# DeepRec-AI/DeepRec

Hardware: AMD Instinct MI355X
Metric: samples/sec (whole node) DLRM Criteo-TB-shaped synthetic (higher is better)
Workload: dtype bf16; 1 GPU; model=dlrm, global_batch=8192, seq_len=1, parallelism=single, hip_graph=True, optimizer=adamasync, embedding_dim=16, num_tables=26

## Files before the change

deeprec_amd/embedding/collection.py:

```python
from __future__ import annotations

from typing import List, Optional, Sequence

import torch

from deeprec_amd.embedding.options import EmbeddingVariableOption
from deeprec_amd.embedding.ragged import RaggedIds
from deeprec_amd.embedding.variable import get_global_step
from deeprec_amd.ops import functional as F
from deeprec_amd.ops.common import COMBINER_ID, KEY_BITS, DedupResult


def unique_and_probe(storage, keys, train: bool, graph_mode: bool = False,
                     allow_dedup: bool = True,
                     bump_step: bool = True) -> DedupResult:
    if graph_mode and train:
        return storage.dedup_lookup_capture(keys, bump_step=bump_step)
    prefers_dedup = getattr(storage, "prefers_dedup", None)
    if train and allow_dedup and prefers_dedup is not None \
            and prefers_dedup():
        return storage.dedup_lookup(keys, get_global_step())
    uniq, inverse, counts = torch.unique(
        keys, return_inverse=True, return_counts=True)
    slots = storage.lookup_or_create(uniq, counts, get_global_step(),
                                     train=train)
    if prefers_dedup is not None:
        storage.observe_uniq_ratio(uniq.numel(), keys.numel())
    return DedupResult(uniq, inverse.to(torch.int32), counts, slots, None,
                       None)


def prep_backward(storage, inverse, counts, rank=None):
    m = counts.numel()
    c32 = counts.to(torch.int32)
    bounds = torch.zeros(m + 1, dtype=torch.int32, device=inverse.device)
    bounds[1:] = c32.cumsum(0)
    if inverse.device.type != "cuda":
        order = torch.argsort(inverse.long()).to(torch.int32)
    elif rank is not None:
        order = storage.ext.csr_scatter(inverse, rank, bounds,
                                        storage.error_flag)
    else:
        order = storage.ext.csr_order(inverse, bounds, m)
    return order, bounds


def row_coeffs(comb, offsets, row_ids, weights):
    lengths = (offsets[1:] - offsets[:-1]).float()
    if weights is None:
        wsum = lengths
        wsq = lengths
    else:
        wsum = torch.zeros_like(lengths)
        wsum.index_add_(0, row_ids.long(), weights)
        wsq = torch.zeros_like(lengths)
        wsq.index_add_(0, row_ids.long(), weights * weights)
    denom = torch.where(comb == 2, wsq.sqrt(), wsum)
    coeff = torch.where(comb == 0, torch.ones_like(denom),
                        1.0 / denom.clamp(min=1e-12))
    return torch.where(lengths > 0, coeff, torch.zeros_like(coeff))


class EmbeddingCollection:
    def __init__(self, name: str, table_names: Sequence[str],
                 embedding_dim: int,
                 ev_option: Optional[EmbeddingVariableOption] = None,
                 combiners=None, device=None, value_dtype=torch.float32,
                 generator=None, trainable: bool = True):
        self.name = name
        self.table_names = list(table_names)
        self.n_tables = len(self.table_names)
        assert 0 < self.n_tables < (1 << (63 - KEY_BITS))
        self.dim = embedding_dim
        self.device = torch.device(device or "cpu")
        self.trainable = trainable
        self.ev_option = ev_option or EmbeddingVariableOption()
        self.combiners = list(combiners or ["mean"] * self.n_tables)
        assert len(self.combiners) == self.n_tables

        import copy
        opt = copy.deepcopy(self.ev_option)
        dvd = max(1, opt.init_option.default_value_dim)
        opt.init_option.default_value_dim = dvd * self.n_tables
        from deeprec_amd.embedding.options import StorageType
        fp8 = opt.storage_option.storage_type == StorageType.HBM_FP8
        if fp8:
            from deeprec_amd.ops.quant_backend import (QuantizedHbmStorage,
                                                       require_cuda_for_fp8)
            require_cuda_for_fp8(self.device, f"EmbeddingCollection {name!r}")
            self.trainable = trainable = False
            self.storage = QuantizedHbmStorage(embedding_dim, opt,
                                               value_dtype, self.device,
                                               generator)
        elif self.device.type == "cuda":
            from deeprec_amd.ops.hip_backend import HbmStorage
            self.storage = HbmStorage(embedding_dim, opt, value_dtype,
                                      self.device, generator)
        else:
            from deeprec_amd.ops.cpu_backend import CpuStorage
            self.storage = CpuStorage(embedding_dim, opt, value_dtype,
                                      self.device, generator)
        self.storage.key_bits = KEY_BITS
        self.storage.dvd_per_table = dvd
        self._combiner_ids = torch.tensor(
            [COMBINER_ID[c] for c in self.combiners], dtype=torch.int32,
            device=self.device)
        self._anchor = torch.zeros((), device=self.device,
                                   requires_grad=trainable)
        self._matrix_cache = {}
        self.graph_mode = False
        self._pending_grads: List = []
        self._recorded_ids: List[torch.Tensor] = []
        self._record_sparse_ids = False

    def composite(self, table: int, ids: torch.Tensor) -> torch.Tensor:
        return ids + (table << KEY_BITS)

    def decompose(self, keys: torch.Tensor):
        return keys >> KEY_BITS, keys & ((1 << KEY_BITS) - 1)

    def accumulate_grad(self, slots, keys, grad_unique):
        self._pending_grads.append((slots, keys, grad_unique))

    def consume_grads(self):
        out = self._pending_grads
        self._pending_grads = []
        return out

    def get_slab(self, name, width=None, init_value=0.0, dtype=torch.float32):
        return self.storage.get_slab(name, width or self.dim, init_value,
                                     dtype)

    def size(self):
        return self.storage.size()

    def total_count(self):
        return self.storage.total_count()

    def _concat_inputs(self, sp_list: Sequence[RaggedIds]):
        batch = sp_list[0].batch_size
        dev = self.device
        vals, offs, rows, weights = [], [], [], []
        base = 0
        any_weights = any(sp.weights is not None for sp in sp_list)
        for t, sp in enumerate(sp_list):
            assert sp.batch_size == batch, "collection: batch mismatch"
            vals.append(sp.values + (t << KEY_BITS))
            o = sp.offsets.to(torch.int64)
            offs.append((o[:-1] if t + 1 < len(sp_list) else o) + base)
            base += int(sp.values.numel())
            rows.append(sp.row_ids().to(torch.int64) + t * batch)
            if any_weights:
                weights.append(sp.weights.float() if sp.weights is not None
                               else torch.ones(sp.values.numel(), device=dev))
        values_cat = torch.cat(vals)
        offsets_cat = torch.cat(offs).to(torch.int32)
        row_ids_cat = torch.cat(rows).to(torch.int32)
        weights_cat = torch.cat(weights) if any_weights else None
        return batch, values_cat, offsets_cat, row_ids_cat, weights_cat

    def _row_coeffs(self, offsets_cat, row_ids_cat, weights_cat, batch):
        return row_coeffs(self._combiner_ids.repeat_interleave(batch),
                          offsets_cat, row_ids_cat, weights_cat)

    def lookup(self, sp_list: Sequence[RaggedIds], out_dtype=None,
               train: bool = True) -> torch.Tensor:
        assert len(sp_list) == self.n_tables
        batch, values_cat, offsets_cat, row_ids_cat, weights_cat = \
            self._concat_inputs(sp_list)
        train = train and self.trainable
        d = self._dedup_and_probe(values_cat, train)
        if not train:
            return self._forward(d.uniq, d.slots, d.inverse, offsets_cat,
                                 weights_cat, batch, out_dtype)
        order, bounds = self._prep_backward(d.inverse, d.counts, d.rank)
        row_coeff = self._row_coeffs(offsets_cat, row_ids_cat, weights_cat,
                                     batch)
        return _CollectionLookup.apply(
            self._anchor, self, d.uniq, d.slots, d.inverse, offsets_cat,
            row_ids_cat, order, bounds, row_coeff, weights_cat, batch,
            out_dtype, False)

    def _dedup_and_probe(self, values_cat, train) -> DedupResult:
        d = unique_and_probe(self.storage, values_cat, train,
                             self.graph_mode)
        if train and self._record_sparse_ids:
            self._recorded_ids.append(d.uniq.detach())
        return d

    def _prep_backward(self, inverse, counts, rank=None):
        return prep_backward(self.storage, inverse, counts, rank)

    def matrix_inputs(self, ids: torch.Tensor):
        batch, n = ids.shape
        assert n == self.n_tables
        cache = self._matrix_cache.get(batch)
        if cache is None:
            dev = self.device
            nb = n * batch
            cache = (
                torch.arange(nb + 1, dtype=torch.int32, device=dev),
                torch.arange(nb, dtype=torch.int32, device=dev),
                torch.ones(nb, device=dev),
                (torch.arange(n, dtype=torch.int64, device=dev)
                 << KEY_BITS).repeat_interleave(batch))
            self._matrix_cache[batch] = cache
        offsets, row_ids, row_coeff, tags = cache
        return ids.t().reshape(-1) + tags, offsets, row_ids, row_coeff

    def lookup_matrix(self, ids: torch.Tensor, out_dtype=None,
                      train: bool = True) -> torch.Tensor:
        batch = ids.shape[0]
        values_cat, offsets, row_ids, row_coeff = self.matrix_inputs(ids)
        train = train and self.trainable
        d = self._dedup_and_probe(values_cat, train)
        if not train:
            return self._forward(d.uniq, d.slots, d.inverse, offsets, None,
                                 batch, out_dtype)
        order, bounds = self._prep_backward(d.inverse, d.counts, d.rank)
        return _CollectionLookup.apply(
            self._anchor, self, d.uniq, d.slots, d.inverse, offsets,
            row_ids, order, bounds, row_coeff, None, batch, out_dtype, True)

    def _forward(self, uniq, slots, inverse, offsets_cat, weights_cat, batch,
                 out_dtype, emb_override=None):
        if self.device.type == "cuda" and hasattr(self.storage, "ext"):
            if emb_override is not None:
                return self.storage.ext.group_pooled_fwd_direct(
                    emb_override.contiguous(), uniq, inverse, offsets_cat,
                    weights_cat if weights_cat is not None
                    else torch.Tensor(),
                    self._combiner_ids, batch, self.n_tables,
                    out_dtype or torch.float32)
            return self.storage.group_pooled_lookup(
                uniq, slots, inverse, offsets_cat, weights_cat,
                self._combiner_ids, batch, self.n_tables, out_dtype)
        emb = (emb_override if emb_override is not None
               else self.storage.gather(uniq, slots))
        outs = []
        row_ids_all = None
        nb = offsets_cat.numel() - 1
        lengths = (offsets_cat[1:] - offsets_cat[:-1]).long()
        row_ids_cat = torch.repeat_interleave(
            torch.arange(nb, dtype=torch.int64,
                         device=offsets_cat.device), lengths)
        for t in range(self.n_tables):
            lo, hi = t * batch, (t + 1) * batch
            jmask = (row_ids_cat >= lo) & (row_ids_cat < hi)
            sub_off = (offsets_cat[lo:hi + 1] - offsets_cat[lo]).to(
                torch.int32)
            out_t = F.pooled_forward(
                emb, inverse[jmask], sub_off,
                (row_ids_cat[jmask] - lo).to(torch.int32),
                self.combiners[t],
                weights_cat[jmask] if weights_cat is not None else None,
                out_dtype)
            outs.append(out_t)
        return torch.cat(outs, dim=1)

    def _backward(self, grad_out, order, bounds, inverse, row_ids_cat,
                  weights_cat, row_coeff, m, batch, identity_rows=False):
        if self.device.type == "cuda":
            return self.storage.ext.group_pooled_bwd_seg(
                grad_out.contiguous(), order, inverse, row_ids_cat,
                weights_cat if weights_cat is not None else torch.Tensor(),
                row_coeff, m, batch, self.n_tables, self.dim,
                identity_rows, 0)
        g = grad_out.float().reshape(batch, self.n_tables, self.dim)
        grad_unique = torch.zeros(m, self.dim)
        order_l = order.long()
        j_sorted = order_l
        counts = (bounds[1:] - bounds[:-1]).long()
        u_of_k = torch.repeat_interleave(
            torch.arange(m, dtype=torch.int64), counts)
        rid = row_ids_cat.long()[j_sorted]
        t_idx = rid // batch
        b_idx = rid % batch
        contrib = g[b_idx, t_idx, :] * row_coeff[rid].unsqueeze(1)
        if weights_cat is not None:
            contrib = contrib * weights_cat[j_sorted].unsqueeze(1)
        grad_unique.index_add_(0, u_of_k, contrib)
        return grad_unique

    def export(self, include_filtered: bool = False):
        return self.storage.export(include_filtered)

    def restore(self, keys, values, freqs=None, versions=None):
        self.storage.import_(keys.to(self.device), values, freqs, versions)

    def export_tables(self, include_filtered: bool = False):
        keys, values, freqs, versions = self.storage.export()
        tid, raw = self.decompose(keys)
        out = {}
        for t, name in enumerate(self.table_names):
            mask = tid == t
            out[name] = (raw[mask], values[mask], freqs[mask],
                         versions[mask])
        return out

    def restore_table(self, table: int, keys, values, freqs=None,
                      versions=None):
        self.storage.import_(self.composite(table, keys.to(self.device)),
                             values, freqs, versions)

    def shrink(self, step: Optional[int] = None) -> int:
        return self.storage.shrink(
            step if step is not None else get_global_step())

    def start_sparse_recording(self):
        self._record_sparse_ids = True

    def consume_recorded_ids(self) -> torch.Tensor:
        if not self._recorded_ids:
            return torch.empty(0, dtype=torch.int64, device=self.device)
        ids = torch.unique(torch.cat(self._recorded_ids))
        self._recorded_ids = []
        return ids

    def get_frequency(self, table: int, keys):
        return self.storage.frequencies(
            self.composite(table, keys.to(self.device)))

    def get_version(self, table: int, keys):
        return self.storage.versions(
            self.composite(table, keys.to(self.device)))

    def __repr__(self):
        return (f"EmbeddingCollection(name={self.name!r}, "
                f"tables={self.n_tables}, dim={self.dim}, "
                f"device={self.device})")


class _CollectionLookup(torch.autograd.Function):
    @staticmethod
    def forward(ctx, anchor, coll, uniq, slots, inverse, offsets_cat,
                row_ids_cat, order, bounds, row_coeff, weights_cat, batch,
                out_dtype, identity_rows=False):
        out = coll._forward(uniq, slots, inverse, offsets_cat, weights_cat,
                            batch, out_dtype)
        ctx.coll = coll
        ctx.batch = batch
        ctx.identity_rows = identity_rows
        ctx.save_for_backward(uniq, slots, order, bounds, inverse,
                              row_ids_cat, row_coeff)
        ctx.weights_cat = weights_cat
        return out

    @staticmethod
    def backward(ctx, grad_out):
        uniq, slots, order, bounds, inverse, row_ids_cat, row_coeff = \
            ctx.saved_tensors
        coll = ctx.coll
        grad_unique = coll._backward(grad_out, order, bounds, inverse,
                                     row_ids_cat, ctx.weights_cat,
                                     row_coeff, uniq.numel(), ctx.batch,
                                     ctx.identity_rows)
        coll.accumulate_grad(slots, uniq, grad_unique)
        return (torch.zeros_like(coll._anchor),) + (None,) * 13
```

deeprec_amd/embedding/lookup.py:

```python
from __future__ import annotations

import os
from typing import List, Sequence

import torch

from deeprec_amd.embedding.collection import (prep_backward, row_coeffs,
                                              unique_and_probe)
from deeprec_amd.embedding.ragged import RaggedIds
from deeprec_amd.embedding.variable import (EmbeddingVariable,
                                            get_global_step)
from deeprec_amd.ops import functional as F
from deeprec_amd.ops.common import COMBINER_ID, PAD_KEY


class _PooledLookup(torch.autograd.Function):
    @staticmethod
    def forward(ctx, anchor, ev, uniq, slots, inverse, offsets, row_ids,
                counts, combiner, weights, out_dtype):
        out = ev.storage.pooled_lookup(
            uniq, slots, inverse, offsets, row_ids, combiner, weights,
            out_dtype) if hasattr(ev.storage, "pooled_lookup") else None
        if out is None:
            emb = ev.storage.gather(uniq, slots)
            out = F.pooled_forward(emb, inverse, offsets, row_ids, combiner,
                                   weights, out_dtype)
        ctx.ev = ev
        ctx.combiner = combiner
        ctx.save_for_backward(uniq, slots, inverse, offsets, row_ids, counts)
        ctx.weights = weights
        return out

    @staticmethod
    def backward(ctx, grad_out):
        uniq, slots, inverse, offsets, row_ids, counts = ctx.saved_tensors
        ev = ctx.ev
        if (grad_out.device.type == "cuda"
                and hasattr(ev.storage, "ext") and counts.numel()):
            grad_unique = _chunked_ev_backward(
                ev, grad_out, inverse, offsets, row_ids, counts,
                ctx.combiner, ctx.weights)
        elif hasattr(ev.storage, "pooled_grad"):
            grad_unique = ev.storage.pooled_grad(
                grad_out, inverse, offsets, row_ids, uniq.numel(),
                ctx.combiner, ctx.weights)
        else:
            grad_unique = F.pooled_backward(
                grad_out, inverse, offsets, row_ids, uniq.numel(),
                ctx.combiner, ctx.weights)
        ev.accumulate_grad(slots, uniq, grad_unique)
        return (torch.zeros_like(ctx.ev._anchor),) + (None,) * 10


def _chunked_ev_backward(ev, grad_out, inverse, offsets, row_ids, counts,
                         combiner, weights):
    st = ev.storage
    m = counts.numel()
    weights = weights.float() if weights is not None else None
    order, _ = prep_backward(st, inverse, counts)
    comb = torch.full((1,), COMBINER_ID[combiner], dtype=torch.int32,
                      device=grad_out.device)
    row_coeff = row_coeffs(comb, offsets, row_ids, weights)
    return st.ext.group_pooled_bwd_seg(
        grad_out.contiguous(), order, inverse.to(torch.int32),
        row_ids.to(torch.int32),
        weights if weights is not None else torch.Tensor(),
        row_coeff, m, offsets.numel() - 1, 1, ev.dim, False, 0)


def _drop_positions(sp_ids: RaggedIds, keep: torch.Tensor) -> RaggedIds:
    row_ids = sp_ids.row_ids()[keep]
    values = sp_ids.values[keep]
    weights = sp_ids.weights[keep] if sp_ids.weights is not None else None
    lengths = torch.zeros(sp_ids.batch_size, dtype=torch.int64,
                          device=values.device)
    lengths.index_add_(0, row_ids.long(),
                       torch.ones_like(row_ids, dtype=torch.int64))
    offsets = torch.zeros(sp_ids.batch_size + 1, dtype=sp_ids.offsets.dtype,
                          device=values.device)
    offsets[1:] = lengths.cumsum(0)
    return RaggedIds(values, offsets, weights)


def embedding_lookup_sparse(ev: EmbeddingVariable, sp_ids: RaggedIds,
                            combiner: str = "mean",
                            out_dtype=None,
                            train: bool = True) -> torch.Tensor:
    from deeprec_amd.parallel.sharded_embedding import (
        ShardedEmbeddingVariable, sharded_embedding_lookup_sparse)
    if isinstance(ev, ShardedEmbeddingVariable):
        return sharded_embedding_lookup_sparse(ev, sp_ids, combiner,
                                               out_dtype, train)
    inv = getattr(ev, "invalid_key", None)
    if inv is not None and bool((sp_ids.values == inv).any()):
        sp_ids = _drop_positions(sp_ids, sp_ids.values != inv)
    graph_mode = bool(getattr(ev, "graph_mode", False)) and ev.trainable
    uniq, inverse, counts, slots, _rank, _m = unique_and_probe(
        ev.storage, sp_ids.values, train, graph_mode,
        allow_dedup=ev.trainable
        and not os.environ.get("DEEPREC_AMD_DISABLE_DEDUP"),
        bump_step=not (graph_mode and train)
        or ev.first_lookup_of_step())
    if train and ev._record_sparse_ids:
        ev._recorded_ids.append(uniq.detach())
    row_ids = sp_ids.row_ids()
    if not (train and ev.trainable):
        emb = ev.storage.gather(uniq, slots)
        return F.pooled_forward(emb, inverse, offsets=sp_ids.offsets,
                                row_ids=row_ids, combiner=combiner,
                                weights=sp_ids.weights, out_dtype=out_dtype)
    return _PooledLookup.apply(ev._anchor, ev, uniq, slots,
                               inverse.to(torch.int32),
                               sp_ids.offsets.to(torch.int32),
                               row_ids, counts, combiner, sp_ids.weights,
                               out_dtype)


def safe_embedding_lookup_sparse(ev, sp_ids: RaggedIds, combiner="mean",
                                 out_dtype=None, train=True):
    if bool((sp_ids.values < 0).any()):
        sp_ids = _drop_positions(sp_ids, sp_ids.values >= 0)
    return embedding_lookup_sparse(ev, sp_ids, combiner, out_dtype, train)


class _PaddedSeqLookup(torch.autograd.Function):

    @staticmethod
    def forward(ctx, anchor, ev, uniq, slots, inverse, order, out_dtype):
        out = ev.storage.seq_gather_pad(uniq, slots, inverse, out_dtype)
        ctx.ev = ev
        ctx.save_for_backward(uniq, slots, inverse, order)
        return out

    @staticmethod
    def backward(ctx, grad_out):
        uniq, slots, inverse, order = ctx.saved_tensors
        ev = ctx.ev
        if grad_out.dtype not in (torch.float32, torch.bfloat16):
            grad_out = grad_out.float()
        none = torch.Tensor()
        grad_unique = ev.storage.ext.group_pooled_bwd_seg(
            grad_out.contiguous(), order, inverse, none, none, none,
            uniq.numel(), inverse.numel(), 1, ev.dim, True, 0)
        ev.accumulate_grad(slots, uniq, grad_unique)
        return (torch.zeros_like(ev._anchor),) + (None,) * 6


def masked_padded_lookup(ev, ids: torch.Tensor, pad_id: int, out_dtype=None,
                         train: bool = True) -> torch.Tensor:
    flat = ids.reshape(-1)
    mask = flat != pad_id
    rows = embedding_lookup(ev, flat[mask], out_dtype=out_dtype, train=train)
    emb = torch.zeros(flat.numel(), ev.dim, device=flat.device,
                      dtype=rows.dtype)
    emb = emb.index_put((mask.nonzero().squeeze(1),), rows)
    return emb.reshape(*ids.shape, ev.dim)


def _static_padded_lookup(ev, ids, pad_id, out_dtype, train):
    st = ev.storage
    flat = ids.reshape(-1).to(torch.int64)
    n = flat.numel()
    is_pad = flat == pad_id
    keys = torch.where(is_pad, torch.full_like(flat, PAD_KEY), flat)
    if not (train and ev.trainable):
        slots = st.lookup(keys)
        inverse = torch.where(
            is_pad, torch.full((n,), -1, dtype=torch.int32,
                               device=flat.device),
            torch.arange(n, dtype=torch.int32, device=flat.device))
        out = st.seq_gather_pad(keys, slots, inverse, out_dtype)
        return out.reshape(*ids.shape, ev.dim)
    if ev.graph_mode:
        d = st.dedup_lookup_capture(
            keys, pad=True, bump_step=ev.first_lookup_of_step())
    else:
        d = st.dedup_lookup(keys, get_global_step(), pad=True)
    if ev._record_sparse_ids:
        if d.m_dev is not None:
            raise RuntimeError(
                "sparse-id recording needs the exact unique keys; "
                "graph_mode pads them")
        ev._recorded_ids.append(d.uniq.detach())
    m = d.counts.numel()
    bounds = torch.zeros(m + 1, dtype=torch.int32, device=flat.device)
    bounds[1:] = d.counts.cumsum(0)
    order = st.ext.csr_scatter_pad(d.inverse, d.rank, bounds, st.error_flag)
    out = _PaddedSeqLookup.apply(ev._anchor, ev, d.uniq, d.slots, d.inverse,
                                 order, out_dtype)
    return out.reshape(*ids.shape, ev.dim)


def embedding_lookup(ev: EmbeddingVariable, ids: torch.Tensor,
                     out_dtype=None, train: bool = True,
                     pad_id=None) -> torch.Tensor:
    if pad_id is not None:
        st = getattr(ev, "storage", None)
        if (isinstance(ev, EmbeddingVariable) and ev.device.type == "cuda"
                and hasattr(st, "ext") and not hasattr(st, "apply_split")):
            return _static_padded_lookup(ev, ids, pad_id, out_dtype, train)
        return masked_padded_lookup(ev, ids, pad_id, out_dtype, train)
    flat = ids.reshape(-1)
    n = flat.numel()
    offsets = torch.arange(n + 1, dtype=torch.int32, device=flat.device)
    out = embedding_lookup_sparse(
        ev, RaggedIds(flat, offsets), combiner="sum",
        out_dtype=out_dtype, train=train)
    return out.reshape(*ids.shape, ev.dim)


def group_embedding_lookup_sparse(evs: Sequence[EmbeddingVariable],
                                  sp_ids_list: Sequence[RaggedIds],
                                  combiners=None, out_dtype=None,
                                  train: bool = True) -> List[torch.Tensor]:
    if combiners is None:
        combiners = ["mean"] * len(evs)
    if len(evs) != len(sp_ids_list) or len(evs) != len(combiners):
        raise ValueError("group_embedding_lookup_sparse: length mismatch")
    return [embedding_lookup_sparse(ev, sp, c, out_dtype, train)
            for ev, sp, c in zip(evs, sp_ids_list, combiners)]
```

deeprec_amd/models/common.py:

```python
from __future__ import annotations

from typing import List, Optional, Sequence

import torch
import torch.nn as nn

from deeprec_amd.data.synthetic import NUM_SPARSE
from deeprec_amd.embedding import EmbeddingVariableOption
from deeprec_amd.embedding.collection import EmbeddingCollection


def make_mlp(sizes: Sequence[int], in_dim: int, device,
             bf16: bool, final_activation: bool = True) -> nn.Sequential:
    if bf16 and torch.device(device).type == "cuda":
        from deeprec_amd.ops.fused_mlp import fused_mlp
        return fused_mlp(list(sizes), in_dim, final_activation)
    layers: List[nn.Module] = []
    d = in_dim
    for i, h in enumerate(sizes):
        layers.append(nn.Linear(d, h))
        if final_activation or i + 1 < len(sizes):
            layers.append(nn.ReLU(inplace=True))
        d = h
    return nn.Sequential(*layers)


class Dice(nn.Module):

    def __init__(self, dim: int, eps: float = 1e-8):
        super().__init__()
        self.bn = nn.BatchNorm1d(dim, eps=eps, affine=False)
        self.alpha = nn.Parameter(torch.zeros(dim))

    def forward(self, x):
        shape = x.shape
        p = torch.sigmoid(self.bn(x.reshape(-1, shape[-1]).float()))
        p = p.reshape(shape).to(x.dtype)
        return x * p + self.alpha.to(x.dtype) * x * (1 - p)


class RecModelBase(nn.Module):

    def __init__(self, embedding_dim: int = 16, device="cpu",
                 bf16: bool = True, num_sparse: int = NUM_SPARSE,
                 ev_option: Optional[EmbeddingVariableOption] = None,
                 name: str = "model", sharded: bool = False,
                 combiners: Optional[List[str]] = None):
        super().__init__()
        self.device_ = torch.device(device)
        self.embedding_dim = embedding_dim
        self.num_sparse = num_sparse
        self.bf16 = bf16 and self.device_.type == "cuda"
        cls = EmbeddingCollection
        if sharded:
            from deeprec_amd.parallel.sharded_collection import (
                ShardedEmbeddingCollection)
            cls = ShardedEmbeddingCollection
        self.collection = cls(
            f"{name}/sparse", [f"C{i + 1}" for i in range(num_sparse)],
            embedding_dim, ev_option=ev_option,
            combiners=combiners or ["mean"] * num_sparse,
            device=self.device_)

    @property
    def compute_dtype(self):
        return torch.bfloat16 if self.bf16 else torch.float32

    def embedding_variables(self):
        return [self.collection]

    def sparse_feats(self, sparse_ids, train=True) -> torch.Tensor:
        if isinstance(sparse_ids, torch.Tensor):
            cat = self.collection.lookup_matrix(
                sparse_ids, out_dtype=self.compute_dtype, train=train)
        else:
            cat = self.collection.lookup(
                sparse_ids, out_dtype=self.compute_dtype, train=train)
        return cat.view(-1, self.num_sparse, self.embedding_dim)

    def amp(self):
        import contextlib
        if self.bf16:
            return torch.autocast(device_type="cuda", dtype=torch.bfloat16)
        return contextlib.nullcontext()

    def loss_fn(self, logits: torch.Tensor, labels: torch.Tensor):
        return nn.functional.binary_cross_entropy_with_logits(
            logits.float(), labels.float())
```

deeprec_amd/models/dlrm.py:

```python
from __future__ import annotations

from typing import List, Optional

import torch
import torch.nn as nn

from deeprec_amd.data.synthetic import NUM_SPARSE
from deeprec_amd.embedding import (
    EmbeddingVariable, EmbeddingVariableOption,
    group_embedding_lookup_sparse,
)


def _mlp(sizes, in_dim, final_activation=True):
    layers: List[nn.Module] = []
    d = in_dim
    for i, h in enumerate(sizes):
        layers.append(nn.Linear(d, h))
        if final_activation or i + 1 < len(sizes):
            layers.append(nn.ReLU(inplace=True))
        d = h
    return nn.Sequential(*layers)


class DLRM(nn.Module):
    def __init__(self, embedding_dim: int = 16,
                 mlp_bot=(512, 256, 64, 16), mlp_top=(512, 256),
                 interaction_op: str = "dot", bf16: bool = True,
                 device="cpu", ev_option: Optional[EmbeddingVariableOption] = None,
                 num_sparse: int = NUM_SPARSE, name_prefix: str = "dlrm",
                 sharded: bool = False, use_collection: bool = True):
        super().__init__()
        assert mlp_bot[-1] == embedding_dim, \
            "bottom MLP output must match embedding dim (dot interaction)"
        self.embedding_dim = embedding_dim
        self.interaction_op = interaction_op
        self.bf16 = bf16
        self.device_ = torch.device(device)
        self.num_sparse = num_sparse

        self.dense_in = 16
        use_fused = bf16 and torch.device(device).type == "cuda"
        self._fused = use_fused
        n_f = num_sparse + 1
        n_pairs = n_f * (n_f - 1) // 2
        self.n_pairs_pad = (n_pairs + 15) & ~15
        top_in = (embedding_dim + self.n_pairs_pad
                  if interaction_op == "dot" else n_f * embedding_dim)
        if use_fused:
            from deeprec_amd.ops.fused_mlp import fused_mlp
            self.mlp_bot = fused_mlp(mlp_bot, self.dense_in)
            self.mlp_top = fused_mlp(list(mlp_top) + [1], top_in,
                                     final_activation=False)
        else:
            self.mlp_bot = _mlp(mlp_bot, self.dense_in)
            self.mlp_top = _mlp(list(mlp_top) + [1], top_in,
                                final_activation=False)
        self.to(self.device_)

        self.collection = None
        if sharded:
            from deeprec_amd.parallel.sharded_collection import (
                ShardedEmbeddingCollection)
            self.collection = ShardedEmbeddingCollection(
                f"{name_prefix}/sparse",
                [f"C{i+1}" for i in range(num_sparse)], embedding_dim,
                ev_option=ev_option, combiners=["mean"] * num_sparse,
                device=self.device_,
                comm_dtype=torch.bfloat16 if self.bf16 else None)
            self.evs = []
        elif use_collection:
            from deeprec_amd.embedding.collection import EmbeddingCollection
            self.collection = EmbeddingCollection(
                f"{name_prefix}/sparse",
                [f"C{i+1}" for i in range(num_sparse)], embedding_dim,
                ev_option=ev_option, combiners=["mean"] * num_sparse,
                device=self.device_)
            self.evs = []
        else:
            self.evs = [
                EmbeddingVariable(f"{name_prefix}/C{i+1}", embedding_dim,
                                  ev_option=ev_option, device=self.device_)
                for i in range(num_sparse)]

    def embedding_variables(self):
        return [self.collection] if self.collection is not None else self.evs

    def _interact(self, feats: torch.Tensor) -> torch.Tensor:
        from deeprec_amd.ops.fused_mlp import dot_interaction
        return dot_interaction(feats, self.n_pairs_pad)

    def forward(self, dense: torch.Tensor, sparse_ids,
                train: bool = True) -> torch.Tensor:
        compute_dtype = torch.bfloat16 if (
            self.bf16 and dense.device.type == "cuda") else torch.float32
        if self.collection is not None:
            if isinstance(sparse_ids, torch.Tensor):
                emb_cat = self.collection.lookup_matrix(
                    sparse_ids, out_dtype=compute_dtype, train=train)
            else:
                emb_cat = self.collection.lookup(sparse_ids,
                                                 out_dtype=compute_dtype,
                                                 train=train)
            emb_feats = emb_cat.view(-1, self.num_sparse, self.embedding_dim)
        else:
            emb_list = group_embedding_lookup_sparse(
                self.evs, sparse_ids, combiners=["mean"] * len(self.evs),
                out_dtype=compute_dtype, train=train)
            emb_feats = torch.stack(list(emb_list), dim=1)
        import contextlib
        amp = (torch.autocast(device_type="cuda", dtype=torch.bfloat16)
               if compute_dtype == torch.bfloat16 else contextlib.nullcontext())
        from deeprec_amd.ops.fused_mlp import prep_dense
        dense = prep_dense(dense, self.dense_in, fused=self._fused)
        with amp:
            bot = self.mlp_bot(dense)
            if self.interaction_op == "dot":
                from deeprec_amd.ops.fused_mlp import dot_interaction_cat
                top_in = dot_interaction_cat(bot, emb_feats,
                                             self.n_pairs_pad)
            else:
                feats = torch.cat(
                    [bot.unsqueeze(1), emb_feats.to(bot.dtype)], dim=1)
                top_in = feats.flatten(1)
            logits = self.mlp_top(top_in)
        return logits.squeeze(1).float()

    def loss_fn(self, logits: torch.Tensor, labels: torch.Tensor):
        return nn.functional.binary_cross_entropy_with_logits(logits, labels)
```

deeprec_amd/ops/build_ext.py:

```python
from __future__ import annotations

import hashlib
import importlib.machinery
import importlib.util
import os
import subprocess
import sys
import sysconfig

_EXT_NAME = "deeprec_amd_hip"
_HERE = os.path.dirname(os.path.abspath(__file__))
_EXT_DIR = os.path.normpath(os.path.join(_HERE, "..", "_ext"))
_SOURCES = [os.path.join(_HERE, "hip", "ev_kernels.hip"),
            os.path.join(_HERE, "hip", "dense_kernels.hip"),
            os.path.join(_HERE, "hip", "gru_kernels.hip"),
            os.path.join(_HERE, "hip", "attention_kernels.hip"),
            os.path.join(_HERE, "hip", "fp8_kernels.hip"),
            os.path.join(_HERE, "hip", "quant_ev_kernels.hip")]
_HIPCC = os.environ.get("HIPCC", "/opt/rocm/bin/hipcc")
_ARCH = os.environ.get("PYTORCH_ROCM_ARCH", "gfx950")

_cached = None


def _torch_paths():
    import torch
    root = os.path.dirname(torch.__file__)
    return (
        [os.path.join(root, "include"),
         os.path.join(root, "include", "torch", "csrc", "api", "include"),
         "/opt/rocm/include",
         sysconfig.get_paths()["include"]],
        os.path.join(root, "lib"),
    )


def _so_path() -> str:
    return os.path.join(_EXT_DIR, f"{_EXT_NAME}.so")


def _headers():
    hip_dir = os.path.join(_HERE, "hip")
    return sorted(os.path.join(hip_dir, f) for f in os.listdir(hip_dir)
                  if f.endswith((".h", ".hpp")))


def _sources_digest() -> str:
    h = hashlib.sha256()
    for s in _SOURCES + _headers():
        with open(s, "rb") as f:
            h.update(f.read())
    return h.hexdigest()[:16]


def build_extension(verbose: bool = False, force: bool = False):
    global _cached
    os.makedirs(_EXT_DIR, exist_ok=True)
    so = _so_path()
    stamp = os.path.join(_EXT_DIR, "source.sha")
    digest = _sources_digest()
    if (not force and os.path.exists(so) and os.path.exists(stamp)
            and open(stamp).read().strip() == digest):
        return load_extension()

    includes, libdir = _torch_paths()
    objs = []
    common_defs = [
        f"-DTORCH_EXTENSION_NAME={_EXT_NAME}",
        "-DTORCH_API_INCLUDE_EXTENSION_H",
        "-D__HIP_PLATFORM_AMD__=1", "-DUSE_ROCM=1", "-DHIPBLAS_V2",
        "-DCUDA_HAS_FP16=1", "-D__HIP_NO_HALF_OPERATORS__=1",
        "-D__HIP_NO_HALF_CONVERSIONS__=1",
        "-DHIP_ENABLE_WARP_SYNC_BUILTINS=1",
    ]
    for src in _SOURCES:
        obj = os.path.join(
            _EXT_DIR, os.path.basename(src).replace(".hip", ".o"))
        cmd = ([_HIPCC, "-c", src, "-o", obj, "-O3", "-std=c++17", "-fPIC",
                f"--offload-arch={_ARCH}", "-fno-gpu-rdc"]
               + common_defs + [f"-isystem{p}" for p in includes])
        if verbose:
            print(" ".join(cmd))
        subprocess.run(cmd, check=True)
        objs.append(obj)
    link = ([_HIPCC, "-shared", "-o", so] + objs +
            [f"-L{libdir}", "-lc10", "-lc10_hip", "-ltorch_cpu",
             "-ltorch_hip", "-ltorch", "-ltorch_python",
             "-L/opt/rocm/lib", "-lamdhip64",
             f"-Wl,-rpath,{libdir}"])
    if verbose:
        print(" ".join(link))
    subprocess.run(link, check=True)
    with open(stamp, "w") as f:
        f.write(digest)
    _cached = None
    return load_extension()


def load_extension():
    global _cached
    if _cached is not None:
        return _cached
    import torch
    so = _so_path()
    if not os.path.exists(so):
        return build_extension()
    loader = importlib.machinery.ExtensionFileLoader(_EXT_NAME, so)
    spec = importlib.util.spec_from_loader(_EXT_NAME, loader)
    mod = importlib.util.module_from_spec(spec)
    loader.exec_module(mod)
    sys.modules[_EXT_NAME] = mod
    _cached = mod
    return mod


def require_extension():
    try:
        return load_extension()
    except Exception as e:
        raise RuntimeError(
            "deeprec_amd HIP extension is not built/loadable. Run "
            "`python __graft_entry__.py` (build) first. Native kernels are "
            f"required on GPU — no eager fallback. Cause: {e}") from e
```

deeprec_amd/ops/hip/ev_kernels.hip:

```cpp

#include "hip_common.h"

#define DEV_INLINE __device__ __forceinline__

static constexpr int64_t EMPTY_KEY = INT64_MIN;
static constexpr int64_t PAD_KEY = INT64_MAX;
static constexpr int kBlock = 256;

namespace {

DEV_INLINE uint64_t mix_hash(uint64_t k) {
  k += 0x9E3779B97F4A7C15ull;
  k = (k ^ (k >> 30)) * 0xBF58476D1CE4E5B9ull;
  k = (k ^ (k >> 27)) * 0x94D049BB133111EBull;
  return k ^ (k >> 31);
}

DEV_INLINE float bf2f(__hip_bfloat16 v) { return __bfloat162float(v); }
DEV_INLINE __hip_bfloat16 f2bf(float v) { return __float2bfloat16(v); }


DEV_INLINE int64_t ht_find(const int64_t* __restrict__ ht_keys,
                           int64_t cap_mask, int64_t key) {
  uint64_t h = mix_hash((uint64_t)key) & (uint64_t)cap_mask;
  for (int64_t probe = 0; probe <= cap_mask; ++probe) {
    int64_t idx = (int64_t)((h + probe) & (uint64_t)cap_mask);
    int64_t cur = ht_keys[idx];
    if (cur == key) return idx;
    if (cur == EMPTY_KEY) return -1;
  }
  return -1;
}

DEV_INLINE int64_t ht_find_or_claim(int64_t* __restrict__ ht_keys,
                                    int64_t cap_mask, int64_t key,
                                    int32_t* __restrict__ entry_counter) {
  uint64_t h = mix_hash((uint64_t)key) & (uint64_t)cap_mask;
  for (int64_t probe = 0; probe <= cap_mask; ++probe) {
    int64_t idx = (int64_t)((h + probe) & (uint64_t)cap_mask);
    int64_t cur = ht_keys[idx];
    if (cur != key) {
      if (cur != EMPTY_KEY) continue;
      int64_t prev = (int64_t)atomicCAS(
          (unsigned long long*)&ht_keys[idx],
          (unsigned long long)EMPTY_KEY, (unsigned long long)key);
      if (prev != EMPTY_KEY && prev != key) continue;
      if (prev == EMPTY_KEY) atomicAdd(entry_counter, 1);
    }
    return idx;
  }
  return -1;
}

DEV_INLINE int64_t default_row(int64_t key, int key_bits,
                               int default_value_dim) {
  if (key_bits > 0) {
    int64_t mask = ((int64_t)1 << key_bits) - 1;
    return (key >> key_bits) * default_value_dim +
           (int64_t)((uint64_t)(key & mask) % (uint64_t)default_value_dim);
  }
  return (int64_t)((uint64_t)key % (uint64_t)default_value_dim);
}

DEV_INLINE int32_t ht_admit(
    int64_t key, int64_t idx, int32_t* __restrict__ ht_slot,
    int32_t* __restrict__ slot_counter, int max_slots,
    float* __restrict__ values, const float* __restrict__ default_values,
    int dim, int default_value_dim, int key_bits, int init_limit,
    int32_t* __restrict__ error_flag) {
  int32_t slot = atomicAdd(slot_counter, 1);
  if (slot >= max_slots) {
    atomicExch(error_flag, 1);
    return -1;
  }
  ht_slot[idx] = slot;
  if (slot < init_limit) {
    const float* src =
        default_values + default_row(key, key_bits, default_value_dim) * dim;
    float* dst = values + (int64_t)slot * dim;
    for (int d = 0; d < dim; ++d) dst[d] = src[d];
  }
  return slot;
}

__global__ void k_lookup_insert(
    const int64_t* __restrict__ keys, const int32_t* __restrict__ counts,
    int n, int64_t* __restrict__ ht_keys, int32_t* __restrict__ ht_slot,
    int32_t* __restrict__ ht_freq, int64_t* __restrict__ ht_version,
    int64_t cap_mask, int32_t* __restrict__ slot_counter,
    int32_t* __restrict__ entry_counter, int max_slots,
    float* __restrict__ values, const float* __restrict__ default_values,
    int dim, int default_value_dim, int key_bits, int init_limit,
    int filter_freq, int64_t step, int train,
    int32_t* __restrict__ out_slots, int32_t* __restrict__ error_flag) {
  int64_t i = blockIdx.x * (int64_t)blockDim.x + threadIdx.x;
  int64_t gstride = gridDim.x * (int64_t)blockDim.x;
  for (; i < n; i += gstride) {
    const int64_t key = keys[i];
    int32_t slot = -1;
    if (!train) {
      int64_t idx = ht_find(ht_keys, cap_mask, key);
      if (idx >= 0) slot = ht_slot[idx];
    } else {
      int64_t idx = ht_find_or_claim(ht_keys, cap_mask, key, entry_counter);
      if (idx < 0) {
        atomicExch(error_flag, 2);
      } else {
        int32_t freq = ht_freq[idx] + (counts ? counts[i] : 1);
        ht_freq[idx] = freq;
        ht_version[idx] = step;
        slot = ht_slot[idx];
        if (slot < 0 && freq >= filter_freq)
          slot = ht_admit(key, idx, ht_slot, slot_counter, max_slots, values,
                          default_values, dim, default_value_dim, key_bits,
                          init_limit, error_flag);
      }
    }
    out_slots[i] = slot;
  }
}

__global__ void k_insert_bulk(
    const int64_t* __restrict__ keys, const int32_t* __restrict__ slots,
    const int32_t* __restrict__ freqs, const int64_t* __restrict__ versions,
    int n, int64_t* __restrict__ ht_keys, int32_t* __restrict__ ht_slot,
    int32_t* __restrict__ ht_freq, int64_t* __restrict__ ht_version,
    int64_t cap_mask, int32_t* __restrict__ entry_counter,
    int32_t* __restrict__ error_flag) {
  int64_t i = blockIdx.x * (int64_t)blockDim.x + threadIdx.x;
  int64_t gstride = gridDim.x * (int64_t)blockDim.x;
  for (; i < n; i += gstride) {
    int64_t idx = ht_find_or_claim(ht_keys, cap_mask, keys[i], entry_counter);
    if (idx < 0) {
      atomicExch(error_flag, 2);
      continue;
    }
    ht_slot[idx] = slots[i];
    if (freqs) ht_freq[idx] = freqs[i];
    if (versions) ht_version[idx] = versions[i];
  }
}


template <bool SKIP_PAD>
__global__ void k_dedup_pass_a(
    const int64_t* __restrict__ keys, int nnz, int64_t* __restrict__ ht_keys,
    int32_t* __restrict__ ht_epoch, int32_t* __restrict__ ht_compact,
    int64_t cap_mask, const int32_t* __restrict__ epoch_dev, int epoch_val,
    int32_t* __restrict__ entry_counter, int32_t* __restrict__ m_counter,
    int64_t* __restrict__ uniq_keys, int64_t* __restrict__ compact_entry,
    int64_t* __restrict__ occ_entry, int32_t* __restrict__ error_flag) {
  const int epoch = epoch_dev ? *epoch_dev : epoch_val;
  int64_t j = blockIdx.x * (int64_t)blockDim.x + threadIdx.x;
  int64_t stride = gridDim.x * (int64_t)blockDim.x;
  for (; j < nnz; j += stride) {
    const int64_t key = keys[j];
    if constexpr (SKIP_PAD) {
      if (key == PAD_KEY) {
        occ_entry[j] = -1;
        continue;
      }
    }
    int64_t idx = ht_find_or_claim(ht_keys, cap_mask, key, entry_counter);
    if (idx < 0) {
      atomicExch(error_flag, 2);
      continue;
    }
    if (ht_epoch[idx] != epoch) {
      int old = atomicExch(&ht_epoch[idx], epoch);
      if (old != epoch) {
        int c = atomicAdd(m_counter, 1);
        ht_compact[idx] = c;
        uniq_keys[c] = key;
        compact_entry[c] = idx;
      }
    }
    occ_entry[j] = idx;
  }
}

__global__ void k_bump_epoch(int32_t* __restrict__ epoch_dev,
                             int64_t* __restrict__ step_dev) {
  if (threadIdx.x == 0 && blockIdx.x == 0) {
    epoch_dev[0] += 1;
    step_dev[0] += 1;
  }
}

__global__ void k_dedup_pass_b(
    const int64_t* __restrict__ compact_entry,
    const int64_t* __restrict__ uniq_keys, int n,
    const int32_t* __restrict__ m_dev, int32_t* __restrict__ ht_slot,
    int32_t* __restrict__ ht_freq, int64_t* __restrict__ ht_version,
    const int32_t* __restrict__ batch_counts,
    const int64_t* __restrict__ step_dev, int64_t step_val,
    int32_t* __restrict__ slot_counter, int max_slots,
    float* __restrict__ values, const float* __restrict__ default_values,
    int dim, int default_value_dim, int key_bits, int init_limit,
    int filter_freq, int32_t* __restrict__ out_slots,
    int32_t* __restrict__ error_flag) {
  const int m = m_dev ? *m_dev : n;
  const int64_t step = step_dev ? *step_dev : step_val;
  int64_t c = blockIdx.x * (int64_t)blockDim.x + threadIdx.x;
  int64_t gstride = gridDim.x * (int64_t)blockDim.x;
  for (; c < n; c += gstride) {
    if (m_dev && (c >= m || uniq_keys[c] == PAD_KEY)) {
      out_slots[c] = -1;
      continue;
    }
    int64_t idx = compact_entry[c];
    int32_t freq = ht_freq[idx] + batch_counts[c];
    ht_freq[idx] = freq;
    ht_version[idx] = step;
    int32_t slot = ht_slot[idx];
    if (slot < 0 && freq >= filter_freq)
      slot = ht_admit(uniq_keys[c], idx, ht_slot, slot_counter, max_slots,
                      values, default_values, dim, default_value_dim,
                      key_bits, init_limit, error_flag);
    out_slots[c] = slot;
  }
}

__global__ void k_zero_f32(float* __restrict__ p, int64_t n) {
  int64_t i = (blockIdx.x * (int64_t)blockDim.x + threadIdx.x) * 4;
  int64_t stride = gridDim.x * (int64_t)blockDim.x * 4;
  for (; i + 3 < n; i += stride)
    *reinterpret_cast<float4*>(p + i) = make_float4(0.f, 0.f, 0.f, 0.f);
  if (blockIdx.x == 0 && threadIdx.x == 0)
    for (int64_t j = n & ~3LL; j < n; ++j) p[j] = 0.0f;
}


__global__ void k_bump_epoch_only(int32_t* __restrict__ epoch_dev) {
  if (threadIdx.x == 0 && blockIdx.x == 0) epoch_dev[0] += 1;
}

__global__ void k_route_fill(int64_t* __restrict__ send_keys,
                             int32_t* __restrict__ send_cnt,
                             int32_t* __restrict__ peer_cursor, int total,
                             int world) {
  int64_t i = blockIdx.x * (int64_t)blockDim.x + threadIdx.x;
  int64_t stride = gridDim.x * (int64_t)blockDim.x;
  for (; i < total; i += stride) {
    send_keys[i] = PAD_KEY;
    send_cnt[i] = 0;
    if (i < world) peer_cursor[i] = 0;
  }
}

static constexpr int kMaxWorld = 64;

__global__ void k_route_pad(
    const int64_t* __restrict__ uniq_keys, const int32_t* __restrict__ counts,
    const int32_t* __restrict__ m_dev, int n_cap, int world, int cap,
    int key_bits, int64_t* __restrict__ send_keys,
    int32_t* __restrict__ send_cnt, int32_t* __restrict__ route_pos,
    int32_t* __restrict__ peer_cursor, int32_t* __restrict__ error_flag) {
  const int m = min(*m_dev, n_cap);
  const int64_t key_mask =
      key_bits > 0 ? (((int64_t)1 << key_bits) - 1) : ~(int64_t)0;
  __shared__ int32_t lcnt[kMaxWorld];
  __shared__ int32_t lbase[kMaxWorld];
  for (int64_t base = (int64_t)blockIdx.x * blockDim.x; base < m;
       base += (int64_t)gridDim.x * blockDim.x) {
    int64_t u = base + threadIdx.x;
    for (int o = threadIdx.x; o < world; o += blockDim.x) lcnt[o] = 0;
    __syncthreads();
    int owner = -1, my = 0;
    int64_t key = 0;
    if (u < m) {
      key = uniq_keys[u];
      owner = (int)((uint64_t)(key & key_mask) % (uint64_t)world);
      my = atomicAdd(&lcnt[owner], 1);
    }
    __syncthreads();
    for (int o = threadIdx.x; o < world; o += blockDim.x)
      lbase[o] = lcnt[o] ? atomicAdd(&peer_cursor[o], lcnt[o]) : 0;
    __syncthreads();
    if (u < m) {
      int pos = lbase[owner] + my;
      if (pos >= cap) {
        atomicExch(error_flag, 4);
        route_pos[u] = owner * cap;
      } else {
        int64_t o = (int64_t)owner * cap + pos;
        send_keys[o] = key;
        send_cnt[o] = counts[u];
        route_pos[u] = (int32_t)o;
      }
    }
    __syncthreads();
  }
}


__global__ void k_slots_gather_pad(const int32_t* __restrict__ inverse,
                                   const int32_t* __restrict__ slots,
                                   int nnz, int32_t* __restrict__ out) {
  int64_t j = blockIdx.x * (int64_t)blockDim.x + threadIdx.x;
  int64_t stride = gridDim.x * (int64_t)blockDim.x;
  for (; j < nnz; j += stride) {
    int c = inverse[j];
    out[j] = c < 0 ? -1 : slots[c];
  }
}

__global__ void k_cnt_sum_pad(const int32_t* __restrict__ inverse,
                              const int32_t* __restrict__ cnt, int nnz,
                              int32_t* __restrict__ cnt_sum) {
  int64_t j = blockIdx.x * (int64_t)blockDim.x + threadIdx.x;
  int64_t stride = gridDim.x * (int64_t)blockDim.x;
  for (; j < nnz; j += stride) {
    int c = inverse[j];
    if (c >= 0) atomicAdd(&cnt_sum[c], cnt[j]);
  }
}

__global__ void k_rows_segsum_pad(const float* __restrict__ grad,
                                  const int32_t* __restrict__ inverse,
                                  int nnz, int dim,
                                  float* __restrict__ grad2) {
  int64_t t = blockIdx.x * (int64_t)blockDim.x + threadIdx.x;
  int64_t total = (int64_t)nnz * dim;
  int64_t stride = gridDim.x * (int64_t)blockDim.x;
  for (; t < total; t += stride) {
    int j = (int)(t / dim);
    int c = inverse[j];
    if (c < 0) continue;
    int d = (int)(t % dim);
    atomicAdd(&grad2[(int64_t)c * dim + d], grad[t]);
  }
}

__global__ void k_compose_i32(const int32_t* __restrict__ inv_in,
                              const int32_t* __restrict__ lut, int nnz,
                              int32_t* __restrict__ inv_out) {
  int64_t j = blockIdx.x * (int64_t)blockDim.x + threadIdx.x;
  int64_t stride = gridDim.x * (int64_t)blockDim.x;
  for (; j < nnz; j += stride) inv_out[j] = lut[inv_in[j]];
}

__global__ void k_rows_to_padded(const float* __restrict__ src,
                                 const int32_t* __restrict__ route_pos,
                                 const int32_t* __restrict__ m_dev,
                                 int n_cap, int dim,
                                 float* __restrict__ dst) {
  const int m = min(*m_dev, n_cap);
  int64_t t = blockIdx.x * (int64_t)blockDim.x + threadIdx.x;
  int64_t total = (int64_t)m * dim;
  int64_t stride = gridDim.x * (int64_t)blockDim.x;
  for (; t < total; t += stride) {
    int u = (int)(t / dim);
    int d = (int)(t % dim);
    dst[(int64_t)route_pos[u] * dim + d] = src[t];
  }
}

struct WaveGroup {
  uint64_t mask;
  int leader;
  int pos;
};

DEV_INLINE WaveGroup wave_group_by(uint64_t v, bool valid) {
  WaveGroup g{0ull, 0, 0};
  const int lane = __lane_id();
  uint64_t mask = __ballot(valid);
  int leader = lane;
  for (int b = 0; b < 64; b += 8) {
#pragma unroll
    for (int i = 0; i < 8; ++i) {
      const bool bit = (v >> (b + i)) & 1ull;
      const uint64_t with = __ballot(bit);
      mask &= bit ? with : ~with;
    }
    leader = valid ? __ffsll((unsigned long long)mask) - 1 : lane;
    const uint64_t lv = __shfl(v, leader);
    if (!__ballot(valid && lv != v)) break;
  }
  if (valid) {
    g.mask = mask;
    g.leader = leader;
    g.pos = __popcll(mask & ((1ull << lane) - 1ull));
  }
  return g;
}

DEV_INLINE int64_t wave_slice_begin() {
  const int wave = __builtin_amdgcn_readfirstlane((int)(threadIdx.x >> 6));
  return (blockIdx.x * (int64_t)(blockDim.x >> 6) + wave) * 64;
}
DEV_INLINE int64_t wave_slice_stride() {
  return gridDim.x * (int64_t)(blockDim.x >> 6) * 64;
}

__global__ void k_dedup_pass_c(
    const int64_t* __restrict__ keys, const int64_t* __restrict__ occ_entry,
    int nnz, const int32_t* __restrict__ ht_compact,
    int32_t* __restrict__ inverse, int32_t* __restrict__ counts,
    int32_t* __restrict__ rank) {
  const int lane = __lane_id();
  const int64_t stride = wave_slice_stride();
  for (int64_t j0 = wave_slice_begin(); j0 < nnz; j0 += stride) {
    const int64_t j = j0 + lane;
    const bool in_range = j < nnz;
    const bool valid = in_range && !(keys && keys[j] == PAD_KEY);
    const int64_t entry = valid ? occ_entry[j] : 0;
    const WaveGroup g = wave_group_by((uint64_t)entry, valid);
    int c = -1, base = 0;
    if (valid && lane == g.leader) {
      c = ht_compact[entry];
      base = atomicAdd(&counts[c], __popcll(g.mask));
    }
    c = __shfl(c, g.leader);
    base = __shfl(base, g.leader);
    if (in_range) {
      inverse[j] = valid ? c : -1;
      rank[j] = valid ? base + g.pos : 0;
    }
  }
}

__global__ void k_csr_scatter(const int32_t* __restrict__ inverse,
                              const int32_t* __restrict__ rank, int nnz,
                              const int32_t* __restrict__ bounds,
                              int32_t* __restrict__ order,
                              int32_t* __restrict__ error_flag) {
  int64_t j = blockIdx.x * (int64_t)blockDim.x + threadIdx.x;
  int64_t stride = gridDim.x * (int64_t)blockDim.x;
  for (; j < nnz; j += stride) {
    int64_t o = (int64_t)bounds[inverse[j]] + rank[j];
    if (o < 0 || o >= nnz) {
      atomicExch(error_flag, 3);
      continue;
    }
    order[o] = (int32_t)j;
  }
}

__global__ void k_fill_i32(int32_t* __restrict__ p, int64_t n, int32_t v) {
  int64_t i = blockIdx.x * (int64_t)blockDim.x + threadIdx.x;
  int64_t stride = gridDim.x * (int64_t)blockDim.x;
  for (; i < n; i += stride) p[i] = v;
}

__global__ void k_csr_scatter_pad(const int32_t* __restrict__ inverse,
                                  const int32_t* __restrict__ rank, int nnz,
                                  const int32_t* __restrict__ bounds, int m,
                                  int32_t* __restrict__ order,
                                  int32_t* __restrict__ error_flag) {
  int64_t j = blockIdx.x * (int64_t)blockDim.x + threadIdx.x;
  int64_t stride = gridDim.x * (int64_t)blockDim.x;
  for (; j < nnz; j += stride) {
    const int c = inverse[j];
    if (c < 0) continue;
    if (c >= m) {
      atomicExch(error_flag, 3);
      continue;
    }
    int64_t o = (int64_t)bounds[c] + rank[j];
    if (o < 0 || o >= nnz) {
      atomicExch(error_flag, 3);
      continue;
    }
    order[o] = (int32_t)j;
  }
}

__global__ void k_csr_order(const int32_t* __restrict__ inverse, int nnz,
                            const int32_t* __restrict__ bounds,
                            int32_t* __restrict__ cursor,
                            int32_t* __restrict__ order) {
  int64_t j = blockIdx.x * (int64_t)blockDim.x + threadIdx.x;
  int64_t stride = gridDim.x * (int64_t)blockDim.x;
  for (; j < nnz; j += stride) {
    int c = inverse[j];
    int pos = atomicAdd(&cursor[c], 1);
    order[bounds[c] + pos] = (int32_t)j;
  }
}

__global__ void k_gather_host_rows(const float* __restrict__ host_src,
                                   const int64_t* __restrict__ rows,
                                   int64_t m, int dim,
                                   float* __restrict__ out) {
  int64_t t = blockIdx.x * (int64_t)blockDim.x + threadIdx.x;
  int64_t total = m * dim;
  int64_t stride = gridDim.x * (int64_t)blockDim.x;
  for (; t < total; t += stride)
    out[t] = host_src[rows[t / dim] * dim + t % dim];
}

__global__ void k_scatter_host_rows(const float* __restrict__ src,
                                    const int64_t* __restrict__ rows,
                                    int64_t m, int dim,
                                    float* __restrict__ host_dst) {
  int64_t t = blockIdx.x * (int64_t)blockDim.x + threadIdx.x;
  int64_t total = m * dim;
  int64_t stride = gridDim.x * (int64_t)blockDim.x;
  for (; t < total; t += stride)
    host_dst[rows[t / dim] * dim + t % dim] = src[t];
}

__global__ void k_lookup(
    const int64_t* __restrict__ keys, int n,
    const int64_t* __restrict__ ht_keys, const int32_t* __restrict__ ht_slot,
    int64_t cap_mask, int32_t* __restrict__ out_slots,
    int64_t* __restrict__ out_entry) {
  int64_t i = blockIdx.x * (int64_t)blockDim.x + threadIdx.x;
  int64_t gstride = gridDim.x * (int64_t)blockDim.x;
  for (; i < n; i += gstride) {
    int64_t idx = ht_find(ht_keys, cap_mask, keys[i]);
    out_slots[i] = idx >= 0 ? ht_slot[idx] : -1;
    if (out_entry) out_entry[i] = idx;
  }
}

__global__ void k_export_scan(
    const int64_t* __restrict__ ht_keys, const int32_t* __restrict__ ht_slot,
    const int32_t* __restrict__ ht_freq,
    const int64_t* __restrict__ ht_version, int64_t capacity,
    int32_t* __restrict__ cursor, int64_t* __restrict__ out_keys,
    int32_t* __restrict__ out_slots, int32_t* __restrict__ out_freqs,
    int64_t* __restrict__ out_versions, int out_cap) {
  int64_t i = blockIdx.x * (int64_t)blockDim.x + threadIdx.x;
  int64_t stride = gridDim.x * (int64_t)blockDim.x;
  for (; i < capacity; i += stride) {
    int64_t k = ht_keys[i];
    if (k == EMPTY_KEY) continue;
    int32_t pos = atomicAdd(cursor, 1);
    if (pos >= out_cap) continue;
    out_keys[pos] = k;
    out_slots[pos] = ht_slot[i];
    out_freqs[pos] = ht_freq[i];
    out_versions[pos] = ht_version[i];
  }
}


template <typename OutT>
__global__ void k_gather(
    const float* __restrict__ values, const float* __restrict__ default_values,
    const int64_t* __restrict__ keys, const int32_t* __restrict__ slots,
    int m, int dim, int default_value_dim, float no_permission_value,
    int use_no_permission, OutT* __restrict__ out) {
  int64_t t = blockIdx.x * (int64_t)blockDim.x + threadIdx.x;
  int64_t total = (int64_t)m * dim;
  int64_t stride = gridDim.x * (int64_t)blockDim.x;
  for (; t < total; t += stride) {
    int i = (int)(t / dim);
    int d = (int)(t % dim);
    int32_t s = slots[i];
    float v;
    if (s >= 0) {
      v = values[(int64_t)s * dim + d];
    } else if (use_no_permission) {
      v = no_permission_value;
    } else {
      int64_t row = (int64_t)((uint64_t)keys[i] % (uint64_t)default_value_dim);
      v = default_values[row * dim + d];
    }
    if constexpr (std::is_same_v<OutT, __hip_bfloat16>) out[t] = f2bf(v);
    else out[t] = v;
  }
}

template <typename OutT, int VEC>
__global__ void k_seq_gather_pad(
    const float* __restrict__ values, const float* __restrict__ default_values,
    const int64_t* __restrict__ keys, const int32_t* __restrict__ slots,
    const int32_t* __restrict__ inverse, int nnz, int n_uniq, int dim,
    int default_value_dim, float no_permission_value, int use_no_permission,
    OutT* __restrict__ out) {
  const int cpr = dim / VEC;
  int64_t t = blockIdx.x * (int64_t)blockDim.x + threadIdx.x;
  const int64_t total = (int64_t)nnz * cpr;
  const int64_t stride = gridDim.x * (int64_t)blockDim.x;
  for (; t < total; t += stride) {
    const int j = (int)(t / cpr);
    const int d0 = (int)(t % cpr) * VEC;
    const int u = inverse[j];
    float v[VEC];
#pragma unroll
    for (int i = 0; i < VEC; ++i) v[i] = 0.0f;
    if ((unsigned)u < (unsigned)n_uniq) {
      const int32_t s = slots[u];
      const float* src = nullptr;
      if (s >= 0) {
        src = values + (int64_t)s * dim + d0;
      } else if (!use_no_permission) {
        int64_t row =
            (int64_t)((uint64_t)keys[u] % (uint64_t)default_value_dim);
        src = default_values + row * dim + d0;
      }
      if (src) {
        if constexpr (VEC % 4 == 0) {
#pragma unroll
          for (int i = 0; i < VEC; i += 4) {
            const float4 q = *reinterpret_cast<const float4*>(src + i);
            v[i] = q.x; v[i + 1] = q.y; v[i + 2] = q.z; v[i + 3] = q.w;
          }
        } else {
#pragma unroll
          for (int i = 0; i < VEC; ++i) v[i] = src[i];
        }
      } else {
#pragma unroll
        for (int i = 0; i < VEC; ++i) v[i] = no_permission_value;
      }
    }
    OutT* dst = out + (int64_t)j * dim + d0;
    if constexpr (std::is_same_v<OutT, __hip_bfloat16>) {
      if constexpr (VEC == 1) {
        dst[0] = f2bf(v[0]);
      } else {
        uint32_t w[VEC / 2];
#pragma unroll
        for (int i = 0; i < VEC / 2; ++i) {
          const __hip_bfloat16 lo = f2bf(v[2 * i]), hi = f2bf(v[2 * i + 1]);
          w[i] = (uint32_t)(*reinterpret_cast<const uint16_t*>(&lo)) |
                 ((uint32_t)(*reinterpret_cast<const uint16_t*>(&hi)) << 16);
        }
        if constexpr (VEC == 8)
          *reinterpret_cast<uint4*>(dst) = make_uint4(w[0], w[1], w[2], w[3]);
        else
          *reinterpret_cast<uint2*>(dst) = make_uint2(w[0], w[1]);
      }
    } else {
      if constexpr (VEC == 4)
        *reinterpret_cast<float4*>(dst) = make_float4(v[0], v[1], v[2], v[3]);
      else
        dst[0] = v[0];
    }
  }
}

DEV_INLINE float row_coeff(int combiner, int len, const float* wsum) {
  if (combiner == 0 || len == 0) return 1.0f;
  float denom = wsum ? *wsum : (float)len;
  if (combiner == 2) denom = sqrtf(wsum ? *wsum : (float)len);
  return denom > 1e-12f ? 1.0f / denom : 0.0f;
}

template <typename OutT>
__global__ void k_pooled_fwd(
    const float* __restrict__ values, const float* __restrict__ default_values,
    const int64_t* __restrict__ keys, const int32_t* __restrict__ slots,
    const int32_t* __restrict__ inverse, const int32_t* __restrict__ offsets,
    const float* __restrict__ weights, int batch, int dim,
    int default_value_dim, float no_permission_value, int use_no_permission,
    int combiner, OutT* __restrict__ out) {
  int64_t t = blockIdx.x * (int64_t)blockDim.x + threadIdx.x;
  int64_t total = (int64_t)batch * dim;
  int64_t stride = gridDim.x * (int64_t)blockDim.x;
  for (; t < total; t += stride) {
    int b = (int)(t / dim);
    int d = (int)(t % dim);
    int beg = offsets[b], end = offsets[b + 1];
    float acc = 0.0f, wacc = 0.0f;
    for (int j = beg; j < end; ++j) {
      int u = inverse[j];
      int32_t s = slots[u];
      float v;
      if (s >= 0) {
        v = values[(int64_t)s * dim + d];
      } else if (use_no_permission) {
        v = no_permission_value;
      } else {
        int64_t row =
            (int64_t)((uint64_t)keys[u] % (uint64_t)default_value_dim);
        v = default_values[row * dim + d];
      }
      float w = weights ? weights[j] : 1.0f;
      acc += w * v;
      wacc += (combiner == 2) ? w * w : w;
    }
    float coeff = 1.0f;
    int len = end - beg;
    if (combiner != 0 && len > 0) {
      float denom = (combiner == 2) ? sqrtf(wacc) : wacc;
      coeff = denom > 1e-12f ? 1.0f / denom : 0.0f;
    }
    float r = acc * coeff;
    if constexpr (std::is_same_v<OutT, __hip_bfloat16>) out[t] = f2bf(r);
    else out[t] = r;
  }
}

template <typename GradT>
__global__ void k_pooled_bwd(
    const GradT* __restrict__ grad_out, const int32_t* __restrict__ inverse,
    const int32_t* __restrict__ offsets, const float* __restrict__ weights,
    int batch, int dim, int combiner, float* __restrict__ grad_unique) {
  int64_t t = blockIdx.x * (int64_t)blockDim.x + threadIdx.x;
  int64_t total = (int64_t)batch * dim;
  int64_t stride = gridDim.x * (int64_t)blockDim.x;
  for (; t < total; t += stride) {
    int b = (int)(t / dim);
    int d = (int)(t % dim);
    int beg = offsets[b], end = offsets[b + 1];
    int len = end - beg;
    if (len == 0) continue;
    float g;
    if constexpr (std::is_same_v<GradT, __hip_bfloat16>) g = bf2f(grad_out[t]);
    else g = grad_out[t];
    float coeff = 1.0f;
    if (combiner != 0) {
      float wacc = 0.0f;
      if (weights) {
        for (int j = beg; j < end; ++j)
          wacc += (combiner == 2) ? weights[j] * weights[j] : weights[j];
      } else {
        wacc = (float)len;
      }
      float denom = (combiner == 2) ? sqrtf(wacc) : wacc;
      coeff = denom > 1e-12f ? 1.0f / denom : 0.0f;
    }
    float gc = g * coeff;
    for (int j = beg; j < end; ++j) {
      float w = weights ? weights[j] : 1.0f;
      atomicAdd(&grad_unique[(int64_t)inverse[j] * dim + d], w * gc);
    }
  }
}


template <typename OutT>
__global__ void k_group_pooled_fwd(
    const float* __restrict__ values, const float* __restrict__ default_values,
    const int64_t* __restrict__ keys, const int32_t* __restrict__ slots,
    const int32_t* __restrict__ inverse, const int32_t* __restrict__ offsets,
    const float* __restrict__ weights,
    const int32_t* __restrict__ combiner_ids, int batch, int n_tables,
    int dim, int default_value_dim, int key_bits, float no_permission_value,
    int use_no_permission, const float* __restrict__ direct,
    OutT* __restrict__ out) {
  int64_t t = blockIdx.x * (int64_t)blockDim.x + threadIdx.x;
  int64_t total = (int64_t)batch * n_tables * dim;
  int64_t stride = gridDim.x * (int64_t)blockDim.x;
  const int64_t key_mask = ((int64_t)1 << key_bits) - 1;
  for (; t < total; t += stride) {
    int d = (int)(t % dim);
    int64_t rid = t / dim;
    int table = (int)(rid / batch);
    int b = (int)(rid % batch);
    int beg = offsets[rid], end = offsets[rid + 1];
    int combiner = combiner_ids[table];
    float acc = 0.0f, wacc = 0.0f;
    for (int j = beg; j < end; ++j) {
      int u = inverse[j];
      float v;
      if (direct) {
        v = direct[(int64_t)u * dim + d];
      } else {
        int32_t s = slots[u];
        if (s >= 0) {
          v = values[(int64_t)s * dim + d];
        } else if (use_no_permission) {
          v = no_permission_value;
        } else {
          int64_t k = keys[u];
          int64_t row = (int64_t)(table)*default_value_dim +
                        (int64_t)((uint64_t)(k & key_mask) %
                                  (uint64_t)default_value_dim);
          v = default_values[row * dim + d];
        }
      }
      float w = weights ? weights[j] : 1.0f;
      acc += w * v;
      wacc += (combiner == 2) ? w * w : w;
    }
    float coeff = 1.0f;
    if (combiner != 0 && end > beg) {
      float denom = (combiner == 2) ? sqrtf(wacc) : wacc;
      coeff = denom > 1e-12f ? 1.0f / denom : 0.0f;
    }
    float r = acc * coeff;
    int64_t oidx = ((int64_t)b * n_tables + table) * dim + d;
    if constexpr (std::is_same_v<OutT, __hip_bfloat16>) out[oidx] = f2bf(r);
    else out[oidx] = r;
  }
}

template <typename GradT, int LANES, int R, bool IDENTITY>
__global__ void k_group_pooled_bwd_seg(
    const GradT* __restrict__ grad_out, const int32_t* __restrict__ order,
    const int32_t* __restrict__ inverse, const int32_t* __restrict__ row_ids,
    const float* __restrict__ weights, const float* __restrict__ row_coeff,
    int nnz, int m_rows, int batch, int n_tables, int dim,
    float* __restrict__ grad_unique) {
  constexpr int kGroups = kBlock / LANES;
  const int l = threadIdx.x % LANES;
  const int64_t step = gridDim.x * (int64_t)kGroups * R;
  const int n_rows = batch * n_tables;
  auto u_at = [&](int64_t k) -> int {
    if (k < 0 || k >= nnz) return -2;
    int j = order[k];
    if ((unsigned)j >= (unsigned)nnz) return -1;
    int u = inverse[j];
    return (unsigned)u < (unsigned)m_rows ? u : -1;
  };
  for (int64_t k0 = (blockIdx.x * (int64_t)kGroups + threadIdx.x / LANES) * R;
       k0 < nnz; k0 += step) {
    int u[R], grow[R];
    float cf[R];
#pragma unroll
    for (int r = 0; r < R; ++r) {
      u[r] = -2;
      grow[r] = 0;
      cf[r] = 1.0f;
      const int64_t k = k0 + r;
      if (k < nnz) {
        const int j = order[k];
        if ((unsigned)j >= (unsigned)nnz) { u[r] = -1; continue; }
        const int rid = IDENTITY ? j : row_ids[j];
        const int uu = inverse[j];
        if ((unsigned)uu >= (unsigned)m_rows ||
            (unsigned)rid >= (unsigned)n_rows) { u[r] = -1; continue; }
        u[r] = uu;
        grow[r] = (rid % batch) * n_tables + rid / batch;
        if constexpr (!IDENTITY)
          cf[r] = (weights ? weights[j] : 1.0f) * row_coeff[rid];
      }
    }
    const int u_prev = u_at(k0 - 1);
    const int u_next = u_at(k0 + R);
    for (int d = l; d < dim; d += LANES) {
      float g[R];
#pragma unroll
      for (int r = 0; r < R; ++r) {
        g[r] = 0.0f;
        if (u[r] >= 0) {
          const int64_t gidx = (int64_t)grow[r] * dim + d;
          if constexpr (std::is_same_v<GradT, __hip_bfloat16>)
            g[r] = bf2f(grad_out[gidx]);
          else
            g[r] = grad_out[gidx];
        }
      }
      float acc = 0.0f;
      bool cut = u[0] >= 0 && u_prev == u[0];
#pragma unroll
      for (int r = 0; r < R; ++r) {
        if (u[r] < 0) continue;
        if constexpr (IDENTITY) acc += g[r];
        else acc += cf[r] * g[r];
        const int un = (r + 1 < R) ? u[r + 1] : u_next;
        if (un == u[r] && r + 1 < R) continue;
        float* dst = &grad_unique[(int64_t)u[r] * dim + d];
        if (cut || un == u[r]) atomicAdd(dst, acc);
        else *dst = acc;
        acc = 0.0f;
        cut = false;
      }
    }
  }
}


#define APPLY_PROLOG                                              \
  int64_t t = blockIdx.x * (int64_t)blockDim.x + threadIdx.x;     \
  int64_t total = (int64_t)m * dim;                               \
  int64_t stride = gridDim.x * (int64_t)blockDim.x;               \
  for (; t < total; t += stride) {                                \
    int i = (int)(t / dim);                                       \
    int d = (int)(t % dim);                                       \
    int32_t s = slots[i];                                         \
    if (s < 0) continue;                                          \
    int64_t o = (int64_t)s * dim + d;                             \
    float g = grad[t];

#define APPLY_EPILOG }

__global__ void k_apply_sgd(float* __restrict__ w,
                            const int32_t* __restrict__ slots,
                            const float* __restrict__ grad, int m, int dim,
                            float lr) {
  APPLY_PROLOG
  w[o] -= lr * g;
  APPLY_EPILOG
}

__global__ void k_apply_adagrad(float* __restrict__ w,
                                float* __restrict__ accum,
                                const int32_t* __restrict__ slots,
                                const float* __restrict__ grad, int m,
                                int dim, float lr, float epsilon) {
  APPLY_PROLOG
  float a = accum[o] + g * g;
  accum[o] = a;
  w[o] -= lr * g / (sqrtf(a) + epsilon);
  APPLY_EPILOG
}

__global__ void k_apply_adagrad_decay(
    float* __restrict__ w, float* __restrict__ accum,
    float* __restrict__ period_slab, const int32_t* __restrict__ slots,
    const float* __restrict__ grad, int m, int dim, float lr, float epsilon,
    float cur_period, float decay_rate, float baseline) {
  APPLY_PROLOG
  float prev_period = period_slab[s];
  float dp = cur_period - prev_period;
  if (dp < 0.0f) dp = 0.0f;
  float decay = powf(decay_rate, dp);
  float a = accum[o] * decay;
  if (a < baseline) a = baseline;
  a += g * g;
  accum[o] = a;
  w[o] -= lr * g / (sqrtf(a) + epsilon);
  APPLY_EPILOG
}

__global__ void k_commit_period(float* __restrict__ period_slab,
                                const int32_t* __restrict__ slots, int m,
                                float cur_period) {
  int64_t i = blockIdx.x * (int64_t)blockDim.x + threadIdx.x;
  int64_t gstride = gridDim.x * (int64_t)blockDim.x;
  for (; i < m; i += gstride) {
    int32_t sl = slots[i];
    if (sl >= 0) period_slab[sl] = cur_period;
  }
}

__global__ void k_apply_adam(float* __restrict__ w, float* __restrict__ mom,
                             float* __restrict__ vel,
                             const int32_t* __restrict__ slots,
                             const float* __restrict__ grad, int m, int dim,
                             float lr_t, float beta1, float beta2,
                             float epsilon) {
  APPLY_PROLOG
  float mn = beta1 * mom[o] + (1.0f - beta1) * g;
  float vn = beta2 * vel[o] + (1.0f - beta2) * g * g;
  mom[o] = mn;
  vel[o] = vn;
  w[o] -= lr_t * mn / (sqrtf(vn) + epsilon);
  APPLY_EPILOG
}

__global__ void k_apply_adam_dev(float* __restrict__ w,
                                 float* __restrict__ mom,
                                 float* __restrict__ vel,
                                 const int32_t* __restrict__ slots,
                                 const float* __restrict__ grad, int m,
                                 int dim, float lr, float beta1, float beta2,
                                 float epsilon,
                                 const float* __restrict__ powers) {
  const float lr_t =
      lr * sqrtf(1.0f - powers[1]) / (1.0f - powers[0]);
  APPLY_PROLOG
  float mn = beta1 * mom[o] + (1.0f - beta1) * g;
  float vn = beta2 * vel[o] + (1.0f - beta2) * g * g;
  mom[o] = mn;
  vel[o] = vn;
  w[o] -= lr_t * mn / (sqrtf(vn) + epsilon);
  APPLY_EPILOG
}

__global__ void k_update_powers(float* __restrict__ powers, float beta1,
                                float beta2) {
  if (threadIdx.x == 0 && blockIdx.x == 0) {
    powers[0] *= beta1;
    powers[1] *= beta2;
  }
}

__global__ void k_apply_adamw(float* __restrict__ w, float* __restrict__ mom,
                              float* __restrict__ vel,
                              const int32_t* __restrict__ slots,
                              const float* __restrict__ grad, int m, int dim,
                              float lr_t, float lr, float beta1, float beta2,
                              float epsilon, float weight_decay) {
  APPLY_PROLOG
  float mn = beta1 * mom[o] + (1.0f - beta1) * g;
  float vn = beta2 * vel[o] + (1.0f - beta2) * g * g;
  mom[o] = mn;
  vel[o] = vn;
  float wv = w[o];
  w[o] = wv - lr_t * mn / (sqrtf(vn) + epsilon) - lr * weight_decay * wv;
  APPLY_EPILOG
}

__global__ void k_apply_rmsprop(float* __restrict__ w, float* __restrict__ vel,
                                const int32_t* __restrict__ slots,
                                const float* __restrict__ grad, int m,
                                int dim, float lr, float beta2,
                                float epsilon) {
  APPLY_PROLOG
  float vn = beta2 * vel[o] + (1.0f - beta2) * g * g;
  vel[o] = vn;
  w[o] -= lr * g / (sqrtf(vn) + epsilon);
  APPLY_EPILOG
}

__global__ void k_apply_ftrl(float* __restrict__ w, float* __restrict__ n,
                             float* __restrict__ z,
                             const int32_t* __restrict__ slots,
                             const float* __restrict__ grad, int m, int dim,
                             float lr, float l1, float l2, float lr_power,
                             float l2_shrinkage) {
  APPLY_PROLOG
  float wv = w[o];
  float n_old = n[o];
  float n_new = n_old + g * g;
  float sigma = (powf(n_new, -lr_power) - powf(n_old, -lr_power)) / lr;
  float gs = g + 2.0f * l2_shrinkage * wv;
  float z_new = z[o] + gs - sigma * wv;
  n[o] = n_new;
  z[o] = z_new;
  float quad = powf(n_new, -lr_power) / lr + 2.0f * l2;
  float w_new = 0.0f;
  if (fabsf(z_new) > l1)
    w_new = ((z_new > 0.0f ? l1 : -l1) - z_new) / quad;
  w[o] = w_new;
  APPLY_EPILOG
}

}


#define CHECK_DEV(t) TORCH_CHECK((t).is_cuda(), #t " must be on GPU")

static inline void zero_fill(void* p, int64_t n, hipStream_t stream) {
  if (n <= 0) return;
  k_zero_f32<<<n_blocks((n + 3) / 4), kBlock, 0, stream>>>(
      static_cast<float*>(p), n);
}

torch::Tensor ht_lookup_insert(
    torch::Tensor keys, torch::Tensor counts, torch::Tensor ht_keys,
    torch::Tensor ht_slot, torch::Tensor ht_freq, torch::Tensor ht_version,
    torch::Tensor slot_counter, torch::Tensor entry_counter,
    torch::Tensor values, torch::Tensor default_values, int64_t max_slots,
    int64_t dvd_per_table, int64_t key_bits, int64_t init_limit,
    int64_t filter_freq, int64_t step, bool train,
    torch::Tensor error_flag) {
  CHECK_DEV(keys);
  int n = keys.numel();
  auto out = torch::empty({n}, keys.options().dtype(torch::kInt32));
  if (n == 0) return out;
  auto stream = current_hip_stream();
  int dim = values.size(1);
  k_lookup_insert<<<n_blocks(n), kBlock, 0, stream>>>(
      keys.data_ptr<int64_t>(),
      counts.defined() && counts.numel() ? counts.data_ptr<int32_t>()
                                         : nullptr,
      n, ht_keys.data_ptr<int64_t>(), ht_slot.data_ptr<int32_t>(),
      ht_freq.data_ptr<int32_t>(), ht_version.data_ptr<int64_t>(),
      ht_keys.numel() - 1, slot_counter.data_ptr<int32_t>(),
      entry_counter.data_ptr<int32_t>(), (int)max_slots,
      values.data_ptr<float>(), default_values.data_ptr<float>(), dim,
      (int)dvd_per_table, (int)key_bits, (int)init_limit, (int)filter_freq,
      step, train ? 1 : 0, out.data_ptr<int32_t>(),
      error_flag.data_ptr<int32_t>());
  return out;
}

template <typename T>
static inline const T* opt_ptr(const c10::optional<torch::Tensor>& t) {
  return t.has_value() ? t->data_ptr<T>() : nullptr;
}

template <bool SKIP_PAD>
static torch::Tensor dedup_a_impl(
    torch::Tensor keys, torch::Tensor ht_keys, torch::Tensor ht_epoch,
    torch::Tensor ht_compact, c10::optional<torch::Tensor> epoch_dev,
    int64_t epoch, torch::Tensor entry_counter, torch::Tensor m_counter,
    torch::Tensor uniq_keys, torch::Tensor compact_entry,
    torch::Tensor occ_entry, torch::Tensor error_flag) {
  int64_t nnz = keys.numel();
  if (nnz == 0) return m_counter;
  auto stream = current_hip_stream();
  k_dedup_pass_a<SKIP_PAD><<<n_blocks(nnz), kBlock, 0, stream>>>(
      keys.data_ptr<int64_t>(), (int)nnz, ht_keys.data_ptr<int64_t>(),
      ht_epoch.data_ptr<int32_t>(), ht_compact.data_ptr<int32_t>(),
      ht_keys.numel() - 1, opt_ptr<int32_t>(epoch_dev), (int)epoch,
      entry_counter.data_ptr<int32_t>(), m_counter.data_ptr<int32_t>(),
      uniq_keys.data_ptr<int64_t>(), compact_entry.data_ptr<int64_t>(),
      occ_entry.data_ptr<int64_t>(), error_flag.data_ptr<int32_t>());
  return m_counter;
}

torch::Tensor ht_dedup_a(torch::Tensor keys, torch::Tensor ht_keys,
                         torch::Tensor ht_epoch, torch::Tensor ht_compact,
                         c10::optional<torch::Tensor> epoch_dev,
                         int64_t epoch, torch::Tensor entry_counter,
                         torch::Tensor m_counter, torch::Tensor uniq_keys,
                         torch::Tensor compact_entry,
                         torch::Tensor occ_entry, torch::Tensor error_flag) {
  return dedup_a_impl<false>(keys, ht_keys, ht_epoch, ht_compact, epoch_dev,
                             epoch, entry_counter, m_counter, uniq_keys,
                             compact_entry, occ_entry, error_flag);
}

torch::Tensor ht_dedup_a_pad(torch::Tensor keys, torch::Tensor ht_keys,
                             torch::Tensor ht_epoch, torch::Tensor ht_compact,
                             c10::optional<torch::Tensor> epoch_dev,
                             int64_t epoch, torch::Tensor entry_counter,
                             torch::Tensor m_counter, torch::Tensor uniq_keys,
                             torch::Tensor compact_entry,
                             torch::Tensor occ_entry,
                             torch::Tensor error_flag) {
  return dedup_a_impl<true>(keys, ht_keys, ht_epoch, ht_compact, epoch_dev,
                            epoch, entry_counter, m_counter, uniq_keys,
                            compact_entry, occ_entry, error_flag);
}

torch::Tensor ht_dedup_b(torch::Tensor compact_entry, torch::Tensor uniq_keys,
                         c10::optional<torch::Tensor> m_dev,
                         torch::Tensor ht_slot, torch::Tensor ht_freq,
                         torch::Tensor ht_version,
                         torch::Tensor batch_counts,
                         c10::optional<torch::Tensor> step_dev, int64_t step,
                         torch::Tensor slot_counter, int64_t max_slots,
                         torch::Tensor values, torch::Tensor default_values,
                         int64_t dvd_per_table, int64_t key_bits,
                         int64_t init_limit, int64_t filter_freq,
                         torch::Tensor error_flag) {
  int n = uniq_keys.numel();
  auto slots = torch::empty({n}, ht_slot.options());
  if (n == 0) return slots;
  auto stream = current_hip_stream();
  k_dedup_pass_b<<<n_blocks(n), kBlock, 0, stream>>>(
      compact_entry.data_ptr<int64_t>(), uniq_keys.data_ptr<int64_t>(), n,
      opt_ptr<int32_t>(m_dev), ht_slot.data_ptr<int32_t>(),
      ht_freq.data_ptr<int32_t>(), ht_version.data_ptr<int64_t>(),
      batch_counts.data_ptr<int32_t>(), opt_ptr<int64_t>(step_dev), step,
      slot_counter.data_ptr<int32_t>(), (int)max_slots,
      values.data_ptr<float>(), default_values.data_ptr<float>(),
      values.size(1), (int)dvd_per_table, (int)key_bits, (int)init_limit,
      (int)filter_freq, slots.data_ptr<int32_t>(),
      error_flag.data_ptr<int32_t>());
  return slots;
}

void bump_epoch(torch::Tensor epoch_dev, torch::Tensor step_dev) {
  k_bump_epoch<<<1, 64, 0, current_hip_stream()>>>(
      epoch_dev.data_ptr<int32_t>(), step_dev.data_ptr<int64_t>());
}

void bump_epoch_only(torch::Tensor epoch_dev) {
  k_bump_epoch_only<<<1, 64, 0, current_hip_stream()>>>(
      epoch_dev.data_ptr<int32_t>());
}

std::tuple<torch::Tensor, torch::Tensor, torch::Tensor> route_pad(
    torch::Tensor uniq_keys, torch::Tensor counts, torch::Tensor m_dev,
    int64_t world, int64_t cap, int64_t key_bits,
    torch::Tensor error_flag) {
  int n_cap = uniq_keys.numel();
  int total = (int)(world * cap);
  auto opts_i32 = counts.options();
  auto send_keys = torch::empty({(int64_t)total}, uniq_keys.options());
  auto send_cnt = torch::empty({(int64_t)total}, opts_i32);
  auto route_pos = torch::empty({(int64_t)n_cap}, opts_i32);
  auto cursor = torch::empty({world}, opts_i32);
  auto stream = current_hip_stream();
  k_route_fill<<<n_blocks(total), kBlock, 0, stream>>>(
      send_keys.data_ptr<int64_t>(), send_cnt.data_ptr<int32_t>(),
      cursor.data_ptr<int32_t>(), total, (int)world);
  k_route_pad<<<n_blocks(n_cap), kBlock, 0, stream>>>(
      uniq_keys.data_ptr<int64_t>(), counts.data_ptr<int32_t>(),
      m_dev.data_ptr<int32_t>(), n_cap, (int)world, (int)cap, (int)key_bits,
      send_keys.data_ptr<int64_t>(), send_cnt.data_ptr<int32_t>(),
      route_pos.data_ptr<int32_t>(), cursor.data_ptr<int32_t>(),
      error_flag.data_ptr<int32_t>());
  return {send_keys, send_cnt, route_pos};
}

torch::Tensor slots_gather_pad(torch::Tensor inverse, torch::Tensor slots) {
  int64_t nnz = inverse.numel();
  auto out = torch::empty({nnz}, slots.options());
  if (nnz == 0) return out;
  k_slots_gather_pad<<<n_blocks(nnz), kBlock, 0, current_hip_stream()>>>(
      inverse.data_ptr<int32_t>(), slots.data_ptr<int32_t>(), (int)nnz,
      out.data_ptr<int32_t>());
  return out;
}

torch::Tensor cnt_sum_pad(torch::Tensor inverse, torch::Tensor cnt,
                          int64_t m_cap) {
  int64_t nnz = inverse.numel();
  auto out = torch::empty({m_cap}, cnt.options());
  auto stream = current_hip_stream();
  zero_fill(out.data_ptr<int32_t>(), m_cap, stream);
  if (nnz)
    k_cnt_sum_pad<<<n_blocks(nnz), kBlock, 0, stream>>>(
        inverse.data_ptr<int32_t>(), cnt.data_ptr<int32_t>(), (int)nnz,
        out.data_ptr<int32_t>());
  return out;
}

torch::Tensor rows_segsum_pad(torch::Tensor grad, torch::Tensor inverse,
                              int64_t m_cap) {
  int64_t nnz = inverse.numel();
  int dim = grad.size(1);
  auto out = torch::empty({m_cap, (int64_t)dim}, grad.options());
  auto stream = current_hip_stream();
  zero_fill(out.data_ptr<float>(), m_cap * dim, stream);
  if (nnz)
    k_rows_segsum_pad<<<n_blocks(nnz * dim), kBlock, 0, stream>>>(
        grad.data_ptr<float>(), inverse.data_ptr<int32_t>(), (int)nnz, dim,
        out.data_ptr<float>());
  return out;
}

torch::Tensor gather_host_rows(torch::Tensor host_src, torch::Tensor rows) {
  TORCH_CHECK(host_src.is_pinned(), "cold slab must be pinned host memory");
  TORCH_CHECK(rows.is_cuda() && rows.scalar_type() == torch::kInt64);
  int64_t m = rows.numel();
  int dim = host_src.size(1);
  auto out = torch::empty({m, (int64_t)dim},
                          rows.options().dtype(torch::kFloat32));
  if (m == 0) return out;
  k_gather_host_rows<<<n_blocks(m * dim), kBlock, 0, current_hip_stream()>>>(
      host_src.data_ptr<float>(), rows.data_ptr<int64_t>(), m, dim,
      out.data_ptr<float>());
  return out;
}

void scatter_host_rows(torch::Tensor src, torch::Tensor rows,
                       torch::Tensor host_dst) {
  TORCH_CHECK(host_dst.is_pinned(), "cold slab must be pinned host memory");
  TORCH_CHECK(rows.is_cuda() && src.is_cuda());
  int64_t m = rows.numel();
  int dim = host_dst.size(1);
  if (m == 0) return;
  k_scatter_host_rows<<<n_blocks(m * dim), kBlock, 0, current_hip_stream()>>>(
      src.data_ptr<float>(), rows.data_ptr<int64_t>(), m, dim,
      host_dst.data_ptr<float>());
}

torch::Tensor compose_i32(torch::Tensor inv_in, torch::Tensor lut) {
  int64_t nnz = inv_in.numel();
  auto out = torch::empty({nnz}, inv_in.options());
  if (nnz == 0) return out;
  k_compose_i32<<<n_blocks(nnz), kBlock, 0, current_hip_stream()>>>(
      inv_in.data_ptr<int32_t>(), lut.data_ptr<int32_t>(), (int)nnz,
      out.data_ptr<int32_t>());
  return out;
}

torch::Tensor rows_to_padded(torch::Tensor src, torch::Tensor route_pos,
                             torch::Tensor m_dev, int64_t out_rows) {
  int n_cap = route_pos.numel();
  int dim = src.size(1);
  auto dst = torch::empty({out_rows, (int64_t)dim}, src.options());
  auto stream = current_hip_stream();
  zero_fill(dst.data_ptr<float>(), out_rows * dim, stream);
  k_rows_to_padded<<<n_blocks((int64_t)n_cap * dim), kBlock, 0, stream>>>(
      src.data_ptr<float>(), route_pos.data_ptr<int32_t>(),
      m_dev.data_ptr<int32_t>(), n_cap, dim, dst.data_ptr<float>());
  return dst;
}

std::tuple<torch::Tensor, torch::Tensor, torch::Tensor> ht_dedup_c(
    c10::optional<torch::Tensor> keys, torch::Tensor occ_entry,
    torch::Tensor ht_compact, int64_t m) {
  int64_t nnz = occ_entry.numel();
  auto inverse = torch::empty({nnz}, ht_compact.options());
  auto rank = torch::empty({nnz}, ht_compact.options());
  auto counts = torch::empty({m}, ht_compact.options());
  if (nnz == 0) return {inverse, counts, rank};
  auto stream = current_hip_stream();
  zero_fill(counts.data_ptr<int32_t>(), m, stream);
  k_dedup_pass_c<<<n_blocks(nnz), kBlock, 0, stream>>>(
      opt_ptr<int64_t>(keys), occ_entry.data_ptr<int64_t>(), (int)nnz,
      ht_compact.data_ptr<int32_t>(), inverse.data_ptr<int32_t>(),
      counts.data_ptr<int32_t>(), rank.data_ptr<int32_t>());
  return {inverse, counts, rank};
}

torch::Tensor csr_scatter(torch::Tensor inverse, torch::Tensor rank,
                          torch::Tensor bounds, torch::Tensor error_flag) {
  int64_t nnz = inverse.numel();
  auto order = torch::empty({nnz}, inverse.options());
  if (nnz == 0) return order;
  k_csr_scatter<<<n_blocks(nnz), kBlock, 0, current_hip_stream()>>>(
      inverse.data_ptr<int32_t>(), rank.data_ptr<int32_t>(), (int)nnz,
      bounds.data_ptr<int32_t>(), order.data_ptr<int32_t>(),
      error_flag.data_ptr<int32_t>());
  return order;
}

torch::Tensor csr_scatter_pad(torch::Tensor inverse, torch::Tensor rank,
                              torch::Tensor bounds,
                              torch::Tensor error_flag) {
  int64_t nnz = inverse.numel();
  auto order = torch::empty({nnz}, inverse.options());
  if (nnz == 0) return order;
  TORCH_CHECK(rank.numel() == nnz, "csr_scatter_pad: rank size mismatch");
  TORCH_CHECK(bounds.numel() >= 1, "csr_scatter_pad: bounds is empty");
  auto stream = current_hip_stream();
  k_fill_i32<<<n_blocks(nnz), kBlock, 0, stream>>>(
      order.data_ptr<int32_t>(), nnz, -1);
  k_csr_scatter_pad<<<n_blocks(nnz), kBlock, 0, stream>>>(
      inverse.data_ptr<int32_t>(), rank.data_ptr<int32_t>(), (int)nnz,
      bounds.data_ptr<int32_t>(), (int)(bounds.numel() - 1),
      order.data_ptr<int32_t>(), error_flag.data_ptr<int32_t>());
  return order;
}

template <typename OutT, int VEC>
static void launch_seq_gather_pad(
    torch::Tensor& values, torch::Tensor& default_values, torch::Tensor& keys,
    torch::Tensor& slots, torch::Tensor& inverse, int dim,
    double no_permission_value, bool use_no_permission, OutT* out,
    hipStream_t stream) {
  int64_t nnz = inverse.numel();
  k_seq_gather_pad<OutT, VEC>
      <<<n_blocks(nnz * (dim / VEC)), kBlock, 0, stream>>>(
          values.data_ptr<float>(), default_values.data_ptr<float>(),
          keys.data_ptr<int64_t>(), slots.data_ptr<int32_t>(),
          inverse.data_ptr<int32_t>(), (int)nnz, (int)slots.numel(), dim,
          (int)default_values.size(0), (float)no_permission_value,
          use_no_permission ? 1 : 0, out);
}

torch::Tensor seq_gather_pad(torch::Tensor values,
                             torch::Tensor default_values, torch::Tensor keys,
                             torch::Tensor slots, torch::Tensor inverse,
                             double no_permission_value,
                             bool use_no_permission,
                             torch::ScalarType out_dtype) {
  CHECK_DEV(inverse);
  TORCH_CHECK(keys.numel() == slots.numel(),
              "seq_gather_pad: keys/slots size mismatch");
  TORCH_CHECK(out_dtype == torch::kFloat32 || out_dtype == torch::kBFloat16,
              "seq_gather_pad: out dtype must be float32 or bfloat16");
  int64_t nnz = inverse.numel();
  int dim = values.size(1);
  auto out = torch::empty({nnz, dim}, values.options().dtype(out_dtype));
  if (nnz * dim == 0) return out;
  auto stream = current_hip_stream();
  if (out_dtype == torch::kBFloat16) {
    auto* op = reinterpret_cast<__hip_bfloat16*>(out.data_ptr<at::BFloat16>());
    if (dim % 8 == 0)
      launch_seq_gather_pad<__hip_bfloat16, 8>(
          values, default_values, keys, slots, inverse, dim,
          no_permission_value, use_no_permission, op, stream);
    else if (dim % 4 == 0)
      launch_seq_gather_pad<__hip_bfloat16, 4>(
          values, default_values, keys, slots, inverse, dim,
          no_permission_value, use_no_permission, op, stream);
    else
      launch_seq_gather_pad<__hip_bfloat16, 1>(
          values, default_values, keys, slots, inverse, dim,
          no_permission_value, use_no_permission, op, stream);
  } else {
    auto* op = out.data_ptr<float>();
    if (dim % 4 == 0)
      launch_seq_gather_pad<float, 4>(
          values, default_values, keys, slots, inverse, dim,
          no_permission_value, use_no_permission, op, stream);
    else
      launch_seq_gather_pad<float, 1>(
          values, default_values, keys, slots, inverse, dim,
          no_permission_value, use_no_permission, op, stream);
  }
  return out;
}

torch::Tensor csr_order(torch::Tensor inverse, torch::Tensor bounds,
                        int64_t m) {
  int64_t nnz = inverse.numel();
  auto order = torch::empty({nnz}, inverse.options());
  auto cursor = torch::zeros({m}, inverse.options());
  if (nnz == 0) return order;
  auto stream = current_hip_stream();
  k_csr_order<<<n_blocks(nnz), kBlock, 0, stream>>>(
      inverse.data_ptr<int32_t>(), (int)nnz, bounds.data_ptr<int32_t>(),
      cursor.data_ptr<int32_t>(), order.data_ptr<int32_t>());
  return order;
}

void ht_insert_bulk(torch::Tensor keys, torch::Tensor slots,
                    torch::Tensor freqs, torch::Tensor versions,
                    torch::Tensor ht_keys, torch::Tensor ht_slot,
                    torch::Tensor ht_freq, torch::Tensor ht_version,
                    torch::Tensor entry_counter, torch::Tensor error_flag) {
  int n = keys.numel();
  if (n == 0) return;
  auto stream = current_hip_stream();
  k_insert_bulk<<<n_blocks(n), kBlock, 0, stream>>>(
      keys.data_ptr<int64_t>(), slots.data_ptr<int32_t>(),
      freqs.defined() && freqs.numel() ? freqs.data_ptr<int32_t>() : nullptr,
      versions.defined() && versions.numel() ? versions.data_ptr<int64_t>()
                                             : nullptr,
      n, ht_keys.data_ptr<int64_t>(), ht_slot.data_ptr<int32_t>(),
      ht_freq.data_ptr<int32_t>(), ht_version.data_ptr<int64_t>(),
      ht_keys.numel() - 1, entry_counter.data_ptr<int32_t>(),
      error_flag.data_ptr<int32_t>());
}

std::tuple<torch::Tensor, torch::Tensor> ht_lookup(torch::Tensor keys,
                                                   torch::Tensor ht_keys,
                                                   torch::Tensor ht_slot,
                                                   bool want_entry) {
  int n = keys.numel();
  auto slots = torch::empty({n}, keys.options().dtype(torch::kInt32));
  auto entry = want_entry
                   ? torch::empty({n}, keys.options().dtype(torch::kInt64))
                   : torch::Tensor();
  if (n == 0) return {slots, entry};
  auto stream = current_hip_stream();
  k_lookup<<<n_blocks(n), kBlock, 0, stream>>>(
      keys.data_ptr<int64_t>(), n, ht_keys.data_ptr<int64_t>(),
      ht_slot.data_ptr<int32_t>(), ht_keys.numel() - 1,
      slots.data_ptr<int32_t>(),
      want_entry ? entry.data_ptr<int64_t>() : nullptr);
  return {slots, entry};
}

std::tuple<torch::Tensor, torch::Tensor, torch::Tensor, torch::Tensor>
ht_export(torch::Tensor ht_keys, torch::Tensor ht_slot, torch::Tensor ht_freq,
          torch::Tensor ht_version, int64_t n_entries) {
  auto opts_i64 = ht_keys.options();
  auto opts_i32 = ht_slot.options();
  auto out_keys = torch::empty({n_entries}, opts_i64);
  auto out_slots = torch::empty({n_entries}, opts_i32);
  auto out_freqs = torch::empty({n_entries}, opts_i32);
  auto out_versions = torch::empty({n_entries}, opts_i64);
  auto cursor = torch::zeros({1}, opts_i32);
  if (n_entries > 0) {
    auto stream = current_hip_stream();
    k_export_scan<<<n_blocks(ht_keys.numel()), kBlock, 0, stream>>>(
        ht_keys.data_ptr<int64_t>(), ht_slot.data_ptr<int32_t>(),
        ht_freq.data_ptr<int32_t>(), ht_version.data_ptr<int64_t>(),
        ht_keys.numel(), cursor.data_ptr<int32_t>(),
        out_keys.data_ptr<int64_t>(), out_slots.data_ptr<int32_t>(),
        out_freqs.data_ptr<int32_t>(), out_versions.data_ptr<int64_t>(),
        (int)n_entries);
  }
  return {out_keys, out_slots, out_freqs, out_versions};
}

torch::Tensor ev_gather(torch::Tensor values, torch::Tensor default_values,
                        torch::Tensor keys, torch::Tensor slots,
                        double no_permission_value, bool use_no_permission,
                        torch::ScalarType out_dtype) {
  int m = keys.numel();
  int dim = values.size(1);
  auto out = torch::empty({m, dim}, values.options().dtype(out_dtype));
  if (m == 0) return out;
  auto stream = current_hip_stream();
  int64_t total = (int64_t)m * dim;
  if (out_dtype == torch::kBFloat16) {
    k_gather<__hip_bfloat16><<<n_blocks(total), kBlock, 0, stream>>>(
        values.data_ptr<float>(), default_values.data_ptr<float>(),
        keys.data_ptr<int64_t>(), slots.data_ptr<int32_t>(), m, dim,
        default_values.size(0), (float)no_permission_value,
        use_no_permission ? 1 : 0,
        reinterpret_cast<__hip_bfloat16*>(out.data_ptr<at::BFloat16>()));
  } else {
    k_gather<float><<<n_blocks(total), kBlock, 0, stream>>>(
        values.data_ptr<float>(), default_values.data_ptr<float>(),
        keys.data_ptr<int64_t>(), slots.data_ptr<int32_t>(), m, dim,
        default_values.size(0), (float)no_permission_value,
        use_no_permission ? 1 : 0, out.data_ptr<float>());
  }
  return out;
}

torch::Tensor pooled_fwd(torch::Tensor values, torch::Tensor default_values,
                         torch::Tensor keys, torch::Tensor slots,
                         torch::Tensor inverse, torch::Tensor offsets,
                         torch::Tensor weights, int64_t combiner,
                         double no_permission_value, bool use_no_permission,
                         torch::ScalarType out_dtype) {
  int batch = offsets.numel() - 1;
  int dim = values.size(1);
  auto out = torch::empty({batch, dim}, values.options().dtype(out_dtype));
  if (batch == 0) return out;
  auto stream = current_hip_stream();
  int64_t total = (int64_t)batch * dim;
  const float* wptr =
      weights.defined() && weights.numel() ? weights.data_ptr<float>()
                                           : nullptr;
  if (out_dtype == torch::kBFloat16) {
    k_pooled_fwd<__hip_bfloat16><<<n_blocks(total), kBlock, 0, stream>>>(
        values.data_ptr<float>(), default_values.data_ptr<float>(),
        keys.data_ptr<int64_t>(), slots.data_ptr<int32_t>(),
        inverse.data_ptr<int32_t>(), offsets.data_ptr<int32_t>(), wptr, batch,
        dim, default_values.size(0), (float)no_permission_value,
        use_no_permission ? 1 : 0, (int)combiner,
        reinterpret_cast<__hip_bfloat16*>(out.data_ptr<at::BFloat16>()));
  } else {
    k_pooled_fwd<float><<<n_blocks(total), kBlock, 0, stream>>>(
        values.data_ptr<float>(), default_values.data_ptr<float>(),
        keys.data_ptr<int64_t>(), slots.data_ptr<int32_t>(),
        inverse.data_ptr<int32_t>(), offsets.data_ptr<int32_t>(), wptr, batch,
        dim, default_values.size(0), (float)no_permission_value,
        use_no_permission ? 1 : 0, (int)combiner, out.data_ptr<float>());
  }
  return out;
}

torch::Tensor pooled_bwd(torch::Tensor grad_out, torch::Tensor inverse,
                         torch::Tensor offsets, torch::Tensor weights,
                         int64_t m, int64_t combiner) {
  int batch = offsets.numel() - 1;
  int dim = grad_out.size(1);
  auto grad_unique = torch::zeros(
      {m, dim}, grad_out.options().dtype(torch::kFloat32));
  if (batch == 0 || m == 0) return grad_unique;
  auto stream = current_hip_stream();
  int64_t total = (int64_t)batch * dim;
  const float* wptr =
      weights.defined() && weights.numel() ? weights.data_ptr<float>()
                                           : nullptr;
  if (grad_out.scalar_type() == torch::kBFloat16) {
    k_pooled_bwd<__hip_bfloat16><<<n_blocks(total), kBlock, 0, stream>>>(
        reinterpret_cast<const __hip_bfloat16*>(
            grad_out.data_ptr<at::BFloat16>()),
        inverse.data_ptr<int32_t>(), offsets.data_ptr<int32_t>(), wptr, batch,
        dim, (int)combiner, grad_unique.data_ptr<float>());
  } else {
    k_pooled_bwd<float><<<n_blocks(total), kBlock, 0, stream>>>(
        grad_out.data_ptr<float>(), inverse.data_ptr<int32_t>(),
        offsets.data_ptr<int32_t>(), wptr, batch, dim, (int)combiner,
        grad_unique.data_ptr<float>());
  }
  return grad_unique;
}

torch::Tensor group_pooled_fwd(
    torch::Tensor values, torch::Tensor default_values, torch::Tensor keys,
    torch::Tensor slots, torch::Tensor inverse, torch::Tensor offsets,
    torch::Tensor weights, torch::Tensor combiner_ids, int64_t batch,
    int64_t n_tables, int64_t key_bits, double no_permission_value,
    bool use_no_permission, torch::ScalarType out_dtype) {
  int dim = values.size(1);
  auto out = torch::empty({batch, n_tables * dim},
                          values.options().dtype(out_dtype));
  int64_t total = batch * n_tables * dim;
  if (total == 0) return out;
  auto stream = current_hip_stream();
  const float* wptr =
      weights.defined() && weights.numel() ? weights.data_ptr<float>()
                                           : nullptr;
  if (out_dtype == torch::kBFloat16) {
    k_group_pooled_fwd<__hip_bfloat16>
        <<<n_blocks(total), kBlock, 0, stream>>>(
            values.data_ptr<float>(), default_values.data_ptr<float>(),
            keys.data_ptr<int64_t>(), slots.data_ptr<int32_t>(),
            inverse.data_ptr<int32_t>(), offsets.data_ptr<int32_t>(), wptr,
            combiner_ids.data_ptr<int32_t>(), (int)batch, (int)n_tables, dim,
            default_values.size(0) / (int)n_tables, (int)key_bits,
            (float)no_permission_value, use_no_permission ? 1 : 0, nullptr,
            reinterpret_cast<__hip_bfloat16*>(out.data_ptr<at::BFloat16>()));
  } else {
    k_group_pooled_fwd<float><<<n_blocks(total), kBlock, 0, stream>>>(
        values.data_ptr<float>(), default_values.data_ptr<float>(),
        keys.data_ptr<int64_t>(), slots.data_ptr<int32_t>(),
        inverse.data_ptr<int32_t>(), offsets.data_ptr<int32_t>(), wptr,
        combiner_ids.data_ptr<int32_t>(), (int)batch, (int)n_tables, dim,
        default_values.size(0) / (int)n_tables, (int)key_bits,
        (float)no_permission_value, use_no_permission ? 1 : 0, nullptr,
        out.data_ptr<float>());
  }
  return out;
}

torch::Tensor group_pooled_fwd_direct(
    torch::Tensor emb_rows, torch::Tensor keys, torch::Tensor inverse,
    torch::Tensor offsets, torch::Tensor weights, torch::Tensor combiner_ids,
    int64_t batch, int64_t n_tables, torch::ScalarType out_dtype) {
  int dim = emb_rows.size(1);
  auto out = torch::empty({batch, n_tables * dim},
                          emb_rows.options().dtype(out_dtype));
  int64_t total = batch * n_tables * dim;
  if (total == 0) return out;
  auto stream = current_hip_stream();
  const float* wptr =
      weights.defined() && weights.numel() ? weights.data_ptr<float>()
                                           : nullptr;
  if (out_dtype == torch::kBFloat16) {
    k_group_pooled_fwd<__hip_bfloat16>
        <<<n_blocks(total), kBlock, 0, stream>>>(
            nullptr, nullptr, keys.data_ptr<int64_t>(), nullptr,
            inverse.data_ptr<int32_t>(), offsets.data_ptr<int32_t>(), wptr,
            combiner_ids.data_ptr<int32_t>(), (int)batch, (int)n_tables, dim,
            1, 0, 0.0f, 0, emb_rows.data_ptr<float>(),
            reinterpret_cast<__hip_bfloat16*>(out.data_ptr<at::BFloat16>()));
  } else {
    k_group_pooled_fwd<float><<<n_blocks(total), kBlock, 0, stream>>>(
        nullptr, nullptr, keys.data_ptr<int64_t>(), nullptr,
        inverse.data_ptr<int32_t>(), offsets.data_ptr<int32_t>(), wptr,
        combiner_ids.data_ptr<int32_t>(), (int)batch, (int)n_tables, dim, 1,
        0, 0.0f, 0, emb_rows.data_ptr<float>(), out.data_ptr<float>());
  }
  return out;
}

static constexpr int kSegR = 8;

template <typename T, int LANES, int R>
static void launch_bwd_seg(const T* gp, torch::Tensor& order,
                           torch::Tensor& inverse, torch::Tensor& row_ids,
                           const float* wptr, torch::Tensor& row_coeff,
                           int64_t m, int64_t batch, int64_t n_tables,
                           int64_t dim, bool identity_rows,
                           torch::Tensor& out, hipStream_t stream) {
  int64_t nnz = order.numel();
  int64_t groups = (nnz + R - 1) / R;
  int grid = n_blocks(groups * LANES);
  if (identity_rows) {
    k_group_pooled_bwd_seg<T, LANES, R, true><<<grid, kBlock, 0, stream>>>(
        gp, order.data_ptr<int32_t>(), inverse.data_ptr<int32_t>(), nullptr,
        nullptr, nullptr, (int)nnz, (int)m, (int)batch, (int)n_tables,
        (int)dim, out.data_ptr<float>());
  } else {
    k_group_pooled_bwd_seg<T, LANES, R, false><<<grid, kBlock, 0, stream>>>(
        gp, order.data_ptr<int32_t>(), inverse.data_ptr<int32_t>(),
        row_ids.data_ptr<int32_t>(), wptr, row_coeff.data_ptr<float>(),
        (int)nnz, (int)m, (int)batch, (int)n_tables, (int)dim,
        out.data_ptr<float>());
  }
}

template <typename T, int LANES>
static void launch_bwd_seg_r(int64_t r, const T* gp, torch::Tensor& order,
                             torch::Tensor& inverse, torch::Tensor& row_ids,
                             const float* wptr, torch::Tensor& row_coeff,
                             int64_t m, int64_t batch, int64_t n_tables,
                             int64_t dim, bool identity_rows,
                             torch::Tensor& out, hipStream_t stream) {
#define SEG_CASE(RR)                                                       \
  case RR:                                                                 \
    launch_bwd_seg<T, LANES, RR>(gp, order, inverse, row_ids, wptr,        \
                                 row_coeff, m, batch, n_tables, dim,       \
                                 identity_rows, out, stream);              \
    break;
  switch (r) {
    SEG_CASE(4)
    SEG_CASE(8)
    SEG_CASE(16)
    SEG_CASE(32)
    default:
      TORCH_CHECK(false, "group_pooled_bwd_seg: r must be 4, 8, 16 or 32");
  }
#undef SEG_CASE
}

torch::Tensor group_pooled_bwd_seg(
    torch::Tensor grad_out, torch::Tensor order, torch::Tensor inverse,
    torch::Tensor row_ids, torch::Tensor weights, torch::Tensor row_coeff,
    int64_t m, int64_t batch, int64_t n_tables, int64_t dim,
    bool identity_rows, int64_t r) {
  auto grad_unique = torch::empty(
      {m, dim}, grad_out.options().dtype(torch::kFloat32));
  if (m * dim == 0) return grad_unique;
  TORCH_CHECK(inverse.numel() == order.numel(),
              "group_pooled_bwd_seg: inverse/order size mismatch");
  TORCH_CHECK(grad_out.numel() == batch * n_tables * dim,
              "group_pooled_bwd_seg: grad_out is not [batch, n_tables*dim]");
  if (!identity_rows)
    TORCH_CHECK(row_ids.numel() == order.numel() &&
                    row_coeff.numel() == batch * n_tables,
                "group_pooled_bwd_seg: row_ids/row_coeff size mismatch");
  auto stream = current_hip_stream();
  zero_fill(grad_unique.data_ptr<float>(), m * dim, stream);
  if (order.numel() == 0) return grad_unique;
  const float* wptr =
      weights.defined() && weights.numel() ? weights.data_ptr<float>()
                                           : nullptr;
  if (wptr)
    TORCH_CHECK(weights.numel() == order.numel(),
                "group_pooled_bwd_seg: weights size mismatch");
  if (r <= 0) r = kSegR;
  if (grad_out.scalar_type() == torch::kBFloat16) {
    auto* gp = reinterpret_cast<const __hip_bfloat16*>(
        grad_out.data_ptr<at::BFloat16>());
    if (dim >= 16)
      launch_bwd_seg_r<__hip_bfloat16, 16>(
          r, gp, order, inverse, row_ids, wptr, row_coeff, m, batch,
          n_tables, dim, identity_rows, grad_unique, stream);
    else
      launch_bwd_seg_r<__hip_bfloat16, 8>(
          r, gp, order, inverse, row_ids, wptr, row_coeff, m, batch,
          n_tables, dim, identity_rows, grad_unique, stream);
  } else {
    auto* gp = grad_out.data_ptr<float>();
    if (dim >= 16)
      launch_bwd_seg_r<float, 16>(
          r, gp, order, inverse, row_ids, wptr, row_coeff, m, batch,
          n_tables, dim, identity_rows, grad_unique, stream);
    else
      launch_bwd_seg_r<float, 8>(
          r, gp, order, inverse, row_ids, wptr, row_coeff, m, batch,
          n_tables, dim, identity_rows, grad_unique, stream);
  }
  return grad_unique;
}


void apply_sgd(torch::Tensor w, torch::Tensor slots, torch::Tensor grad,
               double lr) {
  int m = slots.numel();
  if (m == 0) return;
  int dim = w.size(1);
  auto stream = current_hip_stream();
  k_apply_sgd<<<n_blocks((int64_t)m * dim), kBlock, 0, stream>>>(
      w.data_ptr<float>(), slots.data_ptr<int32_t>(), grad.data_ptr<float>(),
      m, dim, (float)lr);
}

void apply_adagrad(torch::Tensor w, torch::Tensor accum, torch::Tensor slots,
                   torch::Tensor grad, double lr, double epsilon) {
  int m = slots.numel();
  if (m == 0) return;
  int dim = w.size(1);
  auto stream = current_hip_stream();
  k_apply_adagrad<<<n_blocks((int64_t)m * dim), kBlock, 0, stream>>>(
      w.data_ptr<float>(), accum.data_ptr<float>(), slots.data_ptr<int32_t>(),
      grad.data_ptr<float>(), m, dim, (float)lr, (float)epsilon);
}

void apply_adagrad_decay(torch::Tensor w, torch::Tensor accum,
                         torch::Tensor period_slab, torch::Tensor slots,
                         torch::Tensor grad, double lr, double epsilon,
                         double cur_period, double decay_rate,
                         double baseline) {
  int m = slots.numel();
  if (m == 0) return;
  int dim = w.size(1);
  auto stream = current_hip_stream();
  k_apply_adagrad_decay<<<n_blocks((int64_t)m * dim), kBlock, 0, stream>>>(
      w.data_ptr<float>(), accum.data_ptr<float>(),
      period_slab.data_ptr<float>(), slots.data_ptr<int32_t>(),
      grad.data_ptr<float>(), m, dim, (float)lr, (float)epsilon,
      (float)cur_period, (float)decay_rate, (float)baseline);
  k_commit_period<<<n_blocks(m), kBlock, 0, stream>>>(
      period_slab.data_ptr<float>(), slots.data_ptr<int32_t>(), m,
      (float)cur_period);
}

void apply_adam(torch::Tensor w, torch::Tensor mom, torch::Tensor vel,
                torch::Tensor slots, torch::Tensor grad, double lr_t,
                double beta1, double beta2, double epsilon) {
  int m = slots.numel();
  if (m == 0) return;
  int dim = w.size(1);
  auto stream = current_hip_stream();
  k_apply_adam<<<n_blocks((int64_t)m * dim), kBlock, 0, stream>>>(
      w.data_ptr<float>(), mom.data_ptr<float>(), vel.data_ptr<float>(),
      slots.data_ptr<int32_t>(), grad.data_ptr<float>(), m, dim, (float)lr_t,
      (float)beta1, (float)beta2, (float)epsilon);
}

void apply_adam_dev(torch::Tensor w, torch::Tensor mom, torch::Tensor vel,
                    torch::Tensor slots, torch::Tensor grad, double lr,
                    double beta1, double beta2, double epsilon,
                    torch::Tensor powers) {
  int m = slots.numel();
  if (m == 0) return;
  int dim = w.size(1);
  auto stream = current_hip_stream();
  k_apply_adam_dev<<<n_blocks((int64_t)m * dim), kBlock, 0, stream>>>(
      w.data_ptr<float>(), mom.data_ptr<float>(), vel.data_ptr<float>(),
      slots.data_ptr<int32_t>(), grad.data_ptr<float>(), m, dim, (float)lr,
      (float)beta1, (float)beta2, (float)epsilon,
      powers.data_ptr<float>());
}

void update_powers(torch::Tensor powers, double beta1, double beta2) {
  auto stream = current_hip_stream();
  k_update_powers<<<1, 64, 0, stream>>>(powers.data_ptr<float>(),
                                        (float)beta1, (float)beta2);
}

void apply_adamw(torch::Tensor w, torch::Tensor mom, torch::Tensor vel,
                 torch::Tensor slots, torch::Tensor grad, double lr_t,
                 double lr, double beta1, double beta2, double epsilon,
                 double weight_decay) {
  int m = slots.numel();
  if (m == 0) return;
  int dim = w.size(1);
  auto stream = current_hip_stream();
  k_apply_adamw<<<n_blocks((int64_t)m * dim), kBlock, 0, stream>>>(
      w.data_ptr<float>(), mom.data_ptr<float>(), vel.data_ptr<float>(),
      slots.data_ptr<int32_t>(), grad.data_ptr<float>(), m, dim, (float)lr_t,
      (float)lr, (float)beta1, (float)beta2, (float)epsilon,
      (float)weight_decay);
}

void apply_rmsprop(torch::Tensor w, torch::Tensor vel, torch::Tensor slots,
                   torch::Tensor grad, double lr, double beta2,
                   double epsilon) {
  int m = slots.numel();
  if (m == 0) return;
  int dim = w.size(1);
  auto stream = current_hip_stream();
  k_apply_rmsprop<<<n_blocks((int64_t)m * dim), kBlock, 0, stream>>>(
      w.data_ptr<float>(), vel.data_ptr<float>(), slots.data_ptr<int32_t>(),
      grad.data_ptr<float>(), m, dim, (float)lr, (float)beta2,
      (float)epsilon);
}

void apply_ftrl(torch::Tensor w, torch::Tensor n, torch::Tensor z,
                torch::Tensor slots, torch::Tensor grad, double lr, double l1,
                double l2, double lr_power, double l2_shrinkage) {
  int m = slots.numel();
  if (m == 0) return;
  int dim = w.size(1);
  auto stream = current_hip_stream();
  k_apply_ftrl<<<n_blocks((int64_t)m * dim), kBlock, 0, stream>>>(
      w.data_ptr<float>(), n.data_ptr<float>(), z.data_ptr<float>(),
      slots.data_ptr<int32_t>(), grad.data_ptr<float>(), m, dim, (float)lr,
      (float)l1, (float)l2, (float)lr_power, (float)l2_shrinkage);
}

void register_dense(pybind11::module_& mod);
void register_gru(pybind11::module_& mod);
void register_attention(pybind11::module_& mod);
void register_fp8(pybind11::module_& mod);
void register_quant_ev(pybind11::module_& mod);

PYBIND11_MODULE(TORCH_EXTENSION_NAME, mod) {
  register_dense(mod);
  register_gru(mod);
  register_attention(mod);
  register_fp8(mod);
  register_quant_ev(mod);
  mod.def("ht_lookup_insert", &ht_lookup_insert);
  mod.def("ht_dedup_a", &ht_dedup_a);
  mod.def("ht_dedup_a_pad", &ht_dedup_a_pad);
  mod.def("ht_dedup_b", &ht_dedup_b);
  mod.def("bump_epoch", &bump_epoch);
  mod.def("bump_epoch_only", &bump_epoch_only);
  mod.def("route_pad", &route_pad);
  mod.def("rows_to_padded", &rows_to_padded);
  mod.def("slots_gather_pad", &slots_gather_pad);
  mod.def("cnt_sum_pad", &cnt_sum_pad);
  mod.def("rows_segsum_pad", &rows_segsum_pad);
  mod.def("compose_i32", &compose_i32);
  mod.def("gather_host_rows", &gather_host_rows);
  mod.def("scatter_host_rows", &scatter_host_rows);
  mod.def("ht_dedup_c", &ht_dedup_c);
  mod.def("csr_order", &csr_order);
  mod.def("csr_scatter", &csr_scatter);
  mod.def("csr_scatter_pad", &csr_scatter_pad);
  mod.def("seq_gather_pad", &seq_gather_pad);
  mod.def("ht_insert_bulk", &ht_insert_bulk);
  mod.def("ht_lookup", &ht_lookup);
  mod.def("ht_export", &ht_export);
  mod.def("ev_gather", &ev_gather);
  mod.def("pooled_fwd", &pooled_fwd);
  mod.def("pooled_bwd", &pooled_bwd);
  mod.def("group_pooled_fwd", &group_pooled_fwd);
  mod.def("group_pooled_fwd_direct", &group_pooled_fwd_direct);
  mod.def("group_pooled_bwd_seg", &group_pooled_bwd_seg);
  mod.attr("BWD_SEG_R") = (int64_t)kSegR;
  mod.def("apply_sgd", &apply_sgd);
  mod.def("apply_adagrad", &apply_adagrad);
  mod.def("apply_adagrad_decay", &apply_adagrad_decay);
  mod.def("apply_adam", &apply_adam);
  mod.def("apply_adamw", &apply_adamw);
  mod.def("apply_adam_dev", &apply_adam_dev);
  mod.def("update_powers", &update_powers);
  mod.def("apply_rmsprop", &apply_rmsprop);
  mod.def("apply_ftrl", &apply_ftrl);
  mod.attr("EMPTY_KEY") = EMPTY_KEY;
  mod.attr("PAD_KEY") = INT64_MAX;
}
```

deeprec_amd/ops/hip_backend.py:

```python
from __future__ import annotations

import math
import torch

from deeprec_amd.embedding.options import (
    CBFFilter,
    CounterFilter,
    EmbeddingVariableOption,
    GlobalStepEvict,
    L2WeightEvict,
)
from deeprec_amd.ops.build_ext import require_extension
from deeprec_amd.ops.common import COMBINER_ID, KEY_BITS, DedupResult

_LOAD_FACTOR = 0.6


def _pow2(n: int) -> int:
    return 1 << max(10, (n - 1).bit_length())


class HbmStorage:

    def __init__(self, dim: int, ev_option: EmbeddingVariableOption,
                 value_dtype=torch.float32, device=None, generator=None):
        assert value_dtype == torch.float32, \
            "master values are fp32; bf16 is produced by the fused gather"
        self.ext = require_extension()
        self.dim = dim
        self.device = torch.device(device or "cuda")
        self.value_dtype = value_dtype
        self.ev_option = ev_option

        io = ev_option.init_option
        self.default_value_dim = max(1, io.default_value_dim)
        dv = torch.empty(self.default_value_dim, dim, dtype=torch.float32)
        if io.initializer is None:
            dv.normal_(0.0, 1.0 / math.sqrt(dim), generator=generator)
        elif callable(io.initializer):
            io.initializer(dv)
        else:
            dv.fill_(float(io.initializer))
        self.default_values = dv.to(self.device)

        fo = ev_option.filter_option
        self.filter_freq = 0
        if isinstance(fo, (CounterFilter, CBFFilter)):
            self.filter_freq = fo.filter_freq

        self.key_bits = 0
        self.dvd_per_table = self.default_value_dim

        cap = _pow2(ev_option.init_capacity)
        self._alloc_table(cap)
        self._alloc_slabs(max(1024, cap // 2))
        self.slabs = {}
        self._slab_init = {}
        self.slot_counter = torch.zeros(1, dtype=torch.int32,
                                        device=self.device)
        self.entry_counter = torch.zeros(1, dtype=torch.int32,
                                         device=self.device)
        self.error_flag = torch.zeros(1, dtype=torch.int32,
                                      device=self.device)
        self._entries_hint = 0
        self._slots_hint = 0
        self._uniq_ratio = None

    def _alloc_table(self, capacity: int):
        self.capacity = capacity
        self.ht_keys = torch.full((capacity,), -(2 ** 63), dtype=torch.int64,
                                  device=self.device)
        self.ht_slot = torch.full((capacity,), -1, dtype=torch.int32,
                                  device=self.device)
        self.ht_freq = torch.zeros(capacity, dtype=torch.int32,
                                   device=self.device)
        self.ht_version = torch.full((capacity,), -1, dtype=torch.int64,
                                     device=self.device)
        self.ht_epoch = torch.zeros(capacity, dtype=torch.int32,
                                    device=self.device)
        self.ht_compact = torch.zeros(capacity, dtype=torch.int32,
                                      device=self.device)
        self._epoch = getattr(self, "_epoch", 0)

    def _alloc_slabs(self, max_slots: int):
        self.values = torch.empty(max_slots, self.dim, dtype=torch.float32,
                                  device=self.device)

    @property
    def max_slots(self) -> int:
        return self.values.shape[0]

    def _init_limit(self) -> int:
        return self.max_slots

    def _sync_counters(self):
        c = torch.stack([self.slot_counter, self.entry_counter]).cpu()
        self._slots_hint = int(c[0])
        self._entries_hint = int(c[1])

    def _ensure_capacity(self, incoming: int):
        if (self._entries_hint + incoming > self.capacity * _LOAD_FACTOR or
                self._slots_hint + incoming > self.max_slots):
            self._sync_counters()
            if self._entries_hint + incoming > self.capacity * _LOAD_FACTOR:
                self._rehash(_pow2(
                    int((self._entries_hint + incoming) / _LOAD_FACTOR) + 1))
            if self._slots_hint + incoming > self.max_slots:
                self._grow_slots(self._slots_hint + incoming)
        self._entries_hint += incoming
        self._slots_hint += incoming

    def _grow_slots(self, need: int):
        new_cap = self.max_slots
        while new_cap < need:
            new_cap *= 2
        nv = torch.empty(new_cap, self.dim, dtype=torch.float32,
                         device=self.device)
        nv[: self.max_slots] = self.values
        for name, t in list(self.slabs.items()):
            nt = torch.full((new_cap, t.shape[1]), self._slab_init[name],
                            dtype=t.dtype, device=self.device)
            nt[: t.shape[0]] = t
            self.slabs[name] = nt
        self.values = nv

    def _rehash(self, new_capacity: int):
        keys, slots, freqs, versions = self._export_entries()
        self._alloc_table(new_capacity)
        self.entry_counter.zero_()
        self.ext.ht_insert_bulk(keys, slots, freqs, versions, self.ht_keys,
                                self.ht_slot, self.ht_freq, self.ht_version,
                                self.entry_counter, self.error_flag)
        self._check_error()

    def _export_entries(self):
        n = int(self.entry_counter.cpu())
        keys, slots, freqs, versions = self.ext.ht_export(
            self.ht_keys, self.ht_slot, self.ht_freq, self.ht_version, n)
        if n and bool((keys == self.ext.PAD_KEY).any()):
            keep = keys != self.ext.PAD_KEY
            keys, slots = keys[keep], slots[keep]
            freqs, versions = freqs[keep], versions[keep]
        if n:
            order = torch.argsort(keys)
            keys, slots = keys[order], slots[order]
            freqs, versions = freqs[order], versions[order]
        return keys, slots, freqs, versions

    def _check_error(self):
        err = int(self.error_flag.cpu())
        if err != 0:
            raise RuntimeError(
                f"HBM hash table error {err} (1=slab overflow, "
                "2=table full, 3=CSR scatter out of bounds, "
                "4=padded all-to-all peer cap overflow — re-capture with "
                "a larger pad_cap) — engine invariant violated")

    def get_slab(self, name, width, init_value, dtype=torch.float32):
        if name not in self.slabs:
            self.slabs[name] = torch.full(
                (self.max_slots, width), init_value, dtype=dtype,
                device=self.device)
            self._slab_init[name] = init_value
        return self.slabs[name]

    def lookup_or_create(self, keys, counts, step, train=True):
        if train:
            self._ensure_capacity(keys.numel())
        counts_i32 = (counts.to(torch.int32)
                      if counts is not None else torch.Tensor())
        return self.ext.ht_lookup_insert(
            keys, counts_i32, self.ht_keys, self.ht_slot, self.ht_freq,
            self.ht_version, self.slot_counter, self.entry_counter,
            self.values, self.default_values, self.max_slots,
            self.dvd_per_table, self.key_bits, self._init_limit(),
            self.filter_freq, step, train, self.error_flag)

    def lookup(self, keys):
        slots, _ = self.ext.ht_lookup(keys, self.ht_keys, self.ht_slot, False)
        return slots

    def lookup_tier(self, keys) -> torch.Tensor:
        slots = self.lookup(keys).long()
        hot = getattr(self, "hot_rows", None)
        tier = torch.where(slots >= 0,
                           torch.zeros_like(slots),
                           torch.full_like(slots, -1))
        if hot is not None:
            tier = torch.where(slots >= hot, torch.ones_like(slots), tier)
            ssd_base = getattr(self, "ssd_base", None)
            if ssd_base is not None:
                tier = torch.where(slots >= ssd_base,
                                   torch.full_like(slots, 2), tier)
        return tier

    def enable_graph_mode(self, expected_entries: int, expected_slots: int):
        if self.capacity < _pow2(int(expected_entries / _LOAD_FACTOR) + 1):
            self._rehash(_pow2(int(expected_entries / _LOAD_FACTOR) + 1))
        if self.max_slots < expected_slots:
            self._grow_slots(expected_slots)
        self.graph_mode = True
        self._epoch_dev = torch.tensor([self._epoch], dtype=torch.int32,
                                       device=self.device)
        from deeprec_amd.embedding.variable import get_global_step
        self._step_dev = torch.tensor([get_global_step()],
                                      dtype=torch.int64, device=self.device)

    def _dedup_claim(self, keys: torch.Tensor, epoch_dev=None, pad=False):
        nnz = keys.numel()
        uniq_buf = torch.empty(nnz, dtype=torch.int64, device=self.device)
        centry_buf = torch.empty(nnz, dtype=torch.int64, device=self.device)
        occ_entry = torch.empty(nnz, dtype=torch.int64, device=self.device)
        m_counter = torch.zeros(1, dtype=torch.int32, device=self.device)
        pass_a = self.ext.ht_dedup_a_pad if pad else self.ext.ht_dedup_a
        pass_a(keys, self.ht_keys, self.ht_epoch, self.ht_compact,
               epoch_dev, self._epoch, self.entry_counter, m_counter,
               uniq_buf, centry_buf, occ_entry, self.error_flag)
        return uniq_buf, centry_buf, occ_entry, m_counter

    def _dedup_count(self, occ_entry: torch.Tensor, m: int, pad_keys=None):
        return self.ext.ht_dedup_c(pad_keys, occ_entry, self.ht_compact, m)

    def _dedup_admit(self, centry, uniq, counts, step=0, m_dev=None):
        return self.ext.ht_dedup_b(
            centry, uniq, m_dev, self.ht_slot, self.ht_freq,
            self.ht_version, counts,
            self._step_dev if m_dev is not None else None, step,
            self.slot_counter, self.max_slots, self.values,
            self.default_values, self.dvd_per_table, self.key_bits,
            self._init_limit(), self.filter_freq, self.error_flag)

    def dedup_lookup_capture(self, values_cat: torch.Tensor, pad=False,
                             bump_step=True) -> DedupResult:
        if bump_step:
            self.ext.bump_epoch(self._epoch_dev, self._step_dev)
        else:
            self.ext.bump_epoch_only(self._epoch_dev)
        uniq_buf, centry_buf, occ_entry, m_counter = self._dedup_claim(
            values_cat, self._epoch_dev, pad)
        inverse, counts, rank = self._dedup_count(
            occ_entry, values_cat.numel(),
            pad_keys=values_cat if pad else None)
        slots = self._dedup_admit(centry_buf, uniq_buf, counts,
                                  m_dev=m_counter)
        return DedupResult(uniq_buf, inverse, counts, slots, rank, m_counter)

    def dedup_only_capture(self, values_cat: torch.Tensor) -> DedupResult:
        self.ext.bump_epoch(self._epoch_dev, self._step_dev)
        uniq_buf, _centry, occ_entry, m_counter = self._dedup_claim(
            values_cat, self._epoch_dev)
        inverse, counts, rank = self._dedup_count(occ_entry,
                                                  values_cat.numel())
        return DedupResult(uniq_buf, inverse, counts, None, rank, m_counter)

    def dedup_lookup_capture_owner(self, recv_keys: torch.Tensor,
                                   recv_cnt: torch.Tensor) -> DedupResult:
        nnz = recv_keys.numel()
        self.ext.bump_epoch_only(self._epoch_dev)
        uniq_buf, centry_buf, occ_entry, m_counter = self._dedup_claim(
            recv_keys, self._epoch_dev)
        inverse, _counts_c, _rank = self._dedup_count(occ_entry, nnz,
                                                      pad_keys=recv_keys)
        cnt_sum = self.ext.cnt_sum_pad(inverse, recv_cnt, nnz)
        slots = self._dedup_admit(centry_buf, uniq_buf, cnt_sum,
                                  m_dev=m_counter)
        return DedupResult(uniq_buf, inverse, cnt_sum, slots, None,
                           m_counter)

    def prefers_dedup(self) -> bool:
        return self._uniq_ratio is None or self._uniq_ratio < 0.95

    def observe_uniq_ratio(self, m: int, nnz: int):
        r = m / max(nnz, 1)
        self._uniq_ratio = (r if self._uniq_ratio is None
                            else 0.7 * self._uniq_ratio + 0.3 * r)

    def dedup_lookup(self, values_cat: torch.Tensor, step: int,
                     pad=False) -> DedupResult:
        nnz = values_cat.numel()
        self._ensure_capacity(nnz)
        self._epoch += 1
        uniq_buf, centry_buf, occ_entry, m_counter = self._dedup_claim(
            values_cat, pad=pad)
        c = torch.cat([m_counter, self.entry_counter,
                       self.slot_counter]).cpu()
        m = int(c[0])
        self._entries_hint = int(c[1])
        self._slots_hint = int(c[2]) + m
        if not pad:
            self.observe_uniq_ratio(m, nnz)
        uniq = uniq_buf[:m]
        inverse, counts, rank = self._dedup_count(
            occ_entry, m, pad_keys=values_cat if pad else None)
        slots = self._dedup_admit(centry_buf[:m], uniq, counts, step=step)
        return DedupResult(uniq, inverse, counts, slots, rank, None)

    def _use_no_permission(self) -> bool:
        return (self.filter_freq > 0 and
                self.ev_option.init_option.default_value_no_permission
                is not None)

    def _no_permission_value(self) -> float:
        v = self.ev_option.init_option.default_value_no_permission
        return float(v) if v is not None else 0.0

    def gather(self, keys, slots, out_dtype=None):
        return self.ext.ev_gather(
            self.values, self.default_values, keys, slots,
            self._no_permission_value(), self._use_no_permission(),
            out_dtype or torch.float32)

    def seq_gather_pad(self, keys, slots, inverse, out_dtype=None):
        return self.ext.seq_gather_pad(
            self.values, self.default_values, keys, slots, inverse,
            self._no_permission_value(), self._use_no_permission(),
            out_dtype or torch.float32)

    def pooled_lookup(self, keys, slots, inverse, offsets, row_ids, combiner,
                      weights, out_dtype):
        return self.ext.pooled_fwd(
            self.values, self.default_values, keys, slots,
            inverse.to(torch.int32), offsets.to(torch.int32),
            weights.float() if weights is not None else torch.Tensor(),
            COMBINER_ID[combiner], self._no_permission_value(),
            self._use_no_permission(), out_dtype or torch.float32)

    def group_pooled_lookup(self, keys, slots, inverse, offsets, weights,
                            combiner_ids, batch, n_tables, out_dtype):
        return self.ext.group_pooled_fwd(
            self.values, self.default_values, keys, slots,
            inverse, offsets,
            weights if weights is not None else torch.Tensor(),
            combiner_ids, batch, n_tables, KEY_BITS,
            self._no_permission_value(),
            self._use_no_permission(),
            out_dtype or torch.float32)

    def pooled_grad(self, grad_out, inverse, offsets, row_ids, m, combiner,
                    weights):
        return self.ext.pooled_bwd(
            grad_out.contiguous(), inverse.to(torch.int32),
            offsets.to(torch.int32),
            weights.float() if weights is not None else torch.Tensor(),
            m, COMBINER_ID[combiner])

    def shrink(self, step: int) -> int:
        eo = self.ev_option.evict_option
        if eo is None:
            return 0
        keys, slots, freqs, versions = self._export_entries()
        if keys.numel() == 0:
            return 0
        if isinstance(eo, GlobalStepEvict) and eo.steps_to_live > 0:
            keep = versions >= (step - eo.steps_to_live)
        elif isinstance(eo, L2WeightEvict) and eo.l2_weight_threshold > 0:
            keep = torch.ones(keys.numel(), dtype=torch.bool,
                              device=self.device)
            has = slots >= 0
            norms = self._row_norms(slots[has].long())
            kk = keep[has].clone()
            kk &= norms >= eo.l2_weight_threshold
            keep[has] = kk
        else:
            return 0
        n_evicted = int((~keep).sum())
        if n_evicted == 0:
            return 0
        self._rebuild(keys[keep], slots[keep], freqs[keep], versions[keep])
        return n_evicted

    def _row_norms(self, slots):
        return self.values[slots].norm(dim=1)

    def _rebuild(self, keys, slots, freqs, versions):
        adm = slots >= 0
        old_slots = slots[adm].long()
        n_adm = int(adm.sum())
        new_slots = torch.full_like(slots, -1)
        new_slots[adm] = torch.arange(n_adm, dtype=torch.int32,
                                      device=self.device)
        self.values[:n_adm] = self.values[old_slots]
        for name, t in self.slabs.items():
            t[:n_adm] = t[old_slots]
        self._alloc_table(self.capacity)
        self.entry_counter.zero_()
        self.slot_counter.fill_(n_adm)
        self.ext.ht_insert_bulk(keys, new_slots, freqs, versions,
                                self.ht_keys, self.ht_slot, self.ht_freq,
                                self.ht_version, self.entry_counter,
                                self.error_flag)
        self._check_error()
        self._sync_counters()

    def export(self, include_filtered: bool = False):
        keys, slots, freqs, versions = self._export_entries()
        adm = slots >= 0
        out = (keys[adm], self.values[slots[adm].long()].clone(),
               freqs[adm].to(torch.int64), versions[adm])
        if include_filtered:
            out = out + (keys[~adm], freqs[~adm].to(torch.int64))
        return out

    def export_slabs(self, names):
        keys, slots, freqs, versions = self._export_entries()
        adm = slots >= 0
        s = slots[adm].long()
        return [self.slabs[nm][s].clone() for nm in names]

    def import_(self, keys, values, freqs=None, versions=None,
                slab_rows=None):
        m = keys.numel()
        if m == 0:
            return
        keys = keys.to(self.device)
        values = values.to(self.device, torch.float32)
        slots = self._import_entries(keys, freqs, versions)
        self.values[slots.long()] = values
        if slab_rows is not None:
            for name, rows in slab_rows.items():
                self.get_slab(name, rows.shape[1], 0.0)[slots.long()] = \
                    rows.to(self.device)
        self._check_error()
        self._sync_counters()

    def _import_entries(self, keys, freqs, versions):
        m = keys.numel()
        existing = self.lookup(keys)
        is_new = existing < 0
        n_new = int(is_new.sum())
        self._ensure_capacity(m)
        self._sync_counters()
        base = self._slots_hint
        slots = existing.clone()
        slots[is_new] = base + torch.arange(n_new, dtype=torch.int32,
                                            device=self.device)
        self.slot_counter.fill_(base + n_new)
        self._slots_hint = base + n_new
        self.ext.ht_insert_bulk(
            keys, slots,
            freqs.to(self.device, torch.int32) if freqs is not None
            else torch.Tensor(),
            versions.to(self.device, torch.int64) if versions is not None
            else torch.Tensor(),
            self.ht_keys, self.ht_slot, self.ht_freq, self.ht_version,
            self.entry_counter, self.error_flag)
        return slots

    def import_filtered(self, keys, freqs):
        m = keys.numel()
        if m == 0:
            return
        keys = keys.to(self.device)
        self._ensure_capacity(m)
        slots = torch.full((m,), -1, dtype=torch.int32, device=self.device)
        self.ext.ht_insert_bulk(
            keys, slots, freqs.to(self.device, torch.int32),
            torch.Tensor(), self.ht_keys, self.ht_slot, self.ht_freq,
            self.ht_version, self.entry_counter, self.error_flag)
        self._check_error()
        self._sync_counters()

    def memory_usage(self) -> dict:
        table = sum(t.numel() * t.element_size()
                    for t in (self.ht_keys, self.ht_slot, self.ht_freq,
                              self.ht_version, self.ht_epoch,
                              self.ht_compact))
        values = self.values.numel() * self.values.element_size()
        slabs = sum(t.numel() * t.element_size()
                    for t in self.slabs.values())
        return {"table_bytes": table, "values_bytes": values,
                "slab_bytes": slabs,
                "total_bytes": table + values + slabs}

    def size(self) -> int:
        _, slots, _, _ = self._export_entries()
        return int((slots >= 0).sum())

    def total_count(self) -> int:
        return int(self.entry_counter.cpu())

    def frequencies(self, keys):
        keys = keys.to(self.device)
        slots, entry = self.ext.ht_lookup(keys, self.ht_keys, self.ht_slot,
                                          True)
        out = torch.zeros(keys.numel(), dtype=torch.int64, device=self.device)
        found = entry >= 0
        out[found] = self.ht_freq[entry[found]].to(torch.int64)
        return out

    def versions(self, keys):
        keys = keys.to(self.device)
        slots, entry = self.ext.ht_lookup(keys, self.ht_keys, self.ht_slot,
                                          True)
        out = torch.full((keys.numel(),), -1, dtype=torch.int64,
                         device=self.device)
        found = entry >= 0
        out[found] = self.ht_version[entry[found]]
        return out



def sparse_apply(name: str, storage: HbmStorage, slots, grad, hyper: dict):
    if getattr(storage, "inference_only", False):
        raise RuntimeError(
            f"{type(storage).__name__} is inference-only: its rows are "
            "quantized and cannot take a sparse optimizer apply")
    ext = storage.ext
    grad = grad.float().contiguous()
    slots = slots.to(torch.int32)
    w = storage.values
    d = storage.dim
    if name == "sgd":
        ext.apply_sgd(w, slots, grad, hyper["lr"])
    elif name == "adagrad":
        accum = storage.get_slab("adagrad_accum", d,
                                 hyper.get("initial_accumulator", 0.1))
        ext.apply_adagrad(w, accum, slots, grad, hyper["lr"],
                          hyper.get("epsilon", 0.0))
    elif name == "adagrad_decay":
        accum = storage.get_slab("adagrad_accum", d,
                                 hyper.get("initial_accumulator", 0.1))
        period = storage.get_slab("adagrad_decay_period", 1, 0.0)
        cur_period = float(hyper["global_step"]
                           // max(1, hyper["accumulator_decay_step"]))
        ext.apply_adagrad_decay(
            w, accum, period, slots, grad, hyper["lr"],
            hyper.get("epsilon", 0.0), cur_period,
            hyper["accumulator_decay_rate"], hyper["accumulator_baseline"])
    elif name in ("adam", "adamw"):
        import math as _m
        mom = storage.get_slab("adam_m", d, 0.0)
        vel = storage.get_slab("adam_v", d, 0.0)
        b1, b2 = hyper["beta1"], hyper["beta2"]
        t = hyper["step_t"]
        lr_t = hyper["lr"] * _m.sqrt(1 - b2 ** t) / (1 - b1 ** t)
        if name == "adam":
            ext.apply_adam(w, mom, vel, slots, grad, lr_t, b1, b2,
                           hyper["epsilon"])
        else:
            ext.apply_adamw(w, mom, vel, slots, grad, lr_t, hyper["lr"],
                            b1, b2, hyper["epsilon"], hyper["weight_decay"])
    elif name == "adam_async":
        import math as _m
        b1, b2 = hyper["beta1"], hyper["beta2"]
        if hyper.get("powers_dev") is not None:
            mom = storage.get_slab("adam_m", d, 0.0)
            vel = storage.get_slab("adam_v", d, 0.0)
            ext.apply_adam_dev(w, mom, vel, slots, grad, hyper["lr"],
                               b1, b2, hyper["epsilon"],
                               hyper["powers_dev"])
        elif hyper.get("sparse_rmsprop"):
            vel = storage.get_slab("adam_v", d, 0.0)
            ext.apply_rmsprop(w, vel, slots, grad, hyper["lr"], b2,
                              hyper["epsilon"])
        else:
            mom = storage.get_slab("adam_m", d, 0.0)
            vel = storage.get_slab("adam_v", d, 0.0)
            lr_t = hyper["lr"] * _m.sqrt(1 - hyper["beta2_power"]) / \
                (1 - hyper["beta1_power"])
            ext.apply_adam(w, mom, vel, slots, grad, lr_t, b1, b2,
                           hyper["epsilon"])
    elif name == "ftrl":
        n = storage.get_slab("ftrl_accum", d, 0.1)
        z = storage.get_slab("ftrl_linear", d, 0.0)
        ext.apply_ftrl(w, n, z, slots, grad, hyper["lr"], hyper["l1"],
                       hyper["l2"], hyper["lr_power"],
                       hyper.get("l2_shrinkage", 0.0))
    else:
        raise ValueError(f"unknown sparse optimizer {name!r}")
```

deeprec_amd/parallel/sharded_collection.py:

```python
from __future__ import annotations

from typing import NamedTuple, Optional, Sequence

import torch

from deeprec_amd.embedding.collection import EmbeddingCollection
from deeprec_amd.embedding.options import EmbeddingVariableOption
from deeprec_amd.embedding.ragged import RaggedIds
from deeprec_amd.embedding.variable import get_global_step
from deeprec_amd.ops.common import KEY_BITS, PAD_KEY
from deeprec_amd.parallel import comm


class ShardedEmbeddingCollection:

    def __init__(self, name: str, table_names: Sequence[str],
                 embedding_dim: int,
                 ev_option: Optional[EmbeddingVariableOption] = None,
                 combiners=None, device=None, value_dtype=torch.float32,
                 generator=None, trainable: bool = True,
                 comm_dtype: Optional[torch.dtype] = None,
                 node_size: Optional[int] = None):
        self.world = comm.world_size()
        self.rank = comm.rank()
        self.comm_dtype = comm_dtype
        self.node_size = node_size
        self.local = EmbeddingCollection(
            f"{name}/part_{self.rank}", table_names, embedding_dim,
            ev_option, combiners, device, value_dtype, generator, trainable)
        self.name = name
        self.dim = embedding_dim
        self.n_tables = self.local.n_tables
        self._pad_cap = None
        self._observed_max_split = 0

    @property
    def device(self):
        return self.local.device

    @property
    def storage(self):
        return self.local.storage

    @property
    def trainable(self):
        return self.local.trainable

    @property
    def _anchor(self):
        return self.local._anchor

    @property
    def _pending_grads(self):
        return self.local._pending_grads

    def consume_grads(self):
        return self.local.consume_grads()

    def get_slab(self, *a, **kw):
        return self.local.get_slab(*a, **kw)

    def size(self):
        return self.local.size()

    def shrink(self, step=None):
        return self.local.shrink(step)

    def export_tables(self, include_filtered=False):
        return self.local.export_tables(include_filtered)

    def reshard(self, world: int, rank: int):
        old = self.local
        self.world = world
        self.rank = rank
        self.local = EmbeddingCollection(
            f"{self.name}/part_{rank}", list(old.table_names), self.dim,
            old.ev_option, list(old.combiners), old.device,
            trainable=old.trainable)

    def restore_table(self, table, keys, values, freqs=None, versions=None):
        mask = (keys % self.world) == self.rank
        self.local.restore_table(
            table, keys[mask], values[mask],
            None if freqs is None else freqs[mask],
            None if versions is None else versions[mask])

    def lookup_matrix(self, ids: torch.Tensor, out_dtype=None,
                      train: bool = True) -> torch.Tensor:
        values_cat, offsets, row_ids, row_coeff = \
            self.local.matrix_inputs(ids)
        return self._lookup_cat(values_cat, offsets, row_ids, row_coeff,
                                None, ids.shape[0], out_dtype, train)

    def lookup(self, sp_list: Sequence[RaggedIds], out_dtype=None,
               train: bool = True) -> torch.Tensor:
        coll = self.local
        batch, values_cat, offsets_cat, row_ids_cat, weights_cat = \
            coll._concat_inputs(sp_list)
        row_coeff = coll._row_coeffs(offsets_cat, row_ids_cat, weights_cat,
                                     batch)
        return self._lookup_cat(values_cat, offsets_cat, row_ids_cat,
                                row_coeff, weights_cat, batch, out_dtype,
                                train)

    def _lookup_cat(self, values_cat, offsets_cat, row_ids_cat, row_coeff,
                    weights_cat, batch, out_dtype, train):
        coll = self.local
        train = train and coll.trainable
        if train and self._pad_cap is not None:
            return _padded_sharded_lookup(
                self, values_cat, offsets_cat, row_ids_cat, row_coeff,
                weights_cat, batch, out_dtype)
        uniq, inverse, counts = torch.unique(
            values_cat, return_inverse=True, return_counts=True)
        inverse = inverse.to(torch.int32)
        if not train:
            emb = _exchange_lookup(self, uniq, counts, train=False)[0]
            return coll._forward(uniq, None, inverse, offsets_cat,
                                 weights_cat, batch, out_dtype,
                                 emb_override=emb)
        order, bounds = coll._prep_backward(inverse, counts)
        return _ShardedCollectionLookup.apply(
            coll._anchor, self, uniq, counts, inverse, offsets_cat,
            row_ids_cat, order, bounds, row_coeff, weights_cat, batch,
            out_dtype)

    def static_mode(self, pad_cap: int):
        self._pad_cap = int(pad_cap)

    def observed_max_split(self) -> int:
        return self._observed_max_split

    def enable_graph_mode(self, expected_entries: int, expected_slots: int,
                          pad_cap: int):
        self.local.storage.enable_graph_mode(expected_entries,
                                             expected_slots)
        self.local.graph_mode = True
        self.static_mode(pad_cap)


def _route_pad_cpu(uniq, counts, world, cap, key_bits):
    m = uniq.numel()
    raw = uniq & ((1 << key_bits) - 1)
    owner = (raw % world).to(torch.int64)
    send_splits = torch.bincount(owner, minlength=world)
    if m and int(send_splits.max()) > cap:
        raise ValueError(
            f"padded exchange overflow: peer split {int(send_splits.max())}"
            f" exceeds pad cap {cap}")
    order = torch.argsort(owner, stable=True)
    group_start = torch.zeros(world, dtype=torch.int64)
    group_start[1:] = send_splits.cumsum(0)[:-1]
    sorted_owner = owner[order]
    rank_in_group = torch.arange(m, dtype=torch.int64) \
        - group_start[sorted_owner]
    dest = sorted_owner * cap + rank_in_group
    send_keys = torch.full((world * cap,), PAD_KEY, dtype=torch.int64)
    send_cnt = torch.zeros(world * cap, dtype=torch.int32)
    send_keys[dest] = uniq[order]
    send_cnt[dest] = counts[order].to(torch.int32)
    route_pos = torch.empty(m, dtype=torch.int64)
    route_pos[order] = dest
    return send_keys, send_cnt, route_pos


class _PaddedExchange(NamedTuple):
    inverse: torch.Tensor
    order: torch.Tensor
    bounds: torch.Tensor
    route_pos: torch.Tensor
    m_dev: Optional[torch.Tensor]
    own_inv: torch.Tensor
    own_keys: torch.Tensor
    own_slots: torch.Tensor


def _padded_lookup_gpu(sev, values_cat):
    coll, st = sev.local, sev.local.storage
    w, cap = sev.world, sev._pad_cap
    splits = [cap] * w
    req = st.dedup_only_capture(values_cat)
    send_keys, send_cnt, route_pos = st.ext.route_pad(
        req.uniq, req.counts, req.m_dev, w, cap, KEY_BITS, st.error_flag)
    order, bounds = coll._prep_backward(req.inverse, req.counts, req.rank)
    recv_keys = comm.all_to_all_single(send_keys, splits, splits)
    recv_cnt = comm.all_to_all_single(send_cnt, splits, splits)
    own = st.dedup_lookup_capture_owner(recv_keys, recv_cnt)
    slots_elem = st.ext.slots_gather_pad(own.inverse, own.slots)
    reply = st.ext.ev_gather(
        st.values, st.default_values, recv_keys, slots_elem,
        st._no_permission_value(), st._use_no_permission(),
        sev.comm_dtype or torch.float32)
    emb_rows = comm.all_to_all_single(reply, splits, splits).float()
    ex = _PaddedExchange(req.inverse, order, bounds, route_pos, req.m_dev,
                         own.inverse, own.uniq, own.slots)
    return ex, emb_rows, recv_keys, st.ext.compose_i32(req.inverse,
                                                       route_pos)


def _padded_lookup_cpu(sev, values_cat):
    coll, st = sev.local, sev.local.storage
    w, cap = sev.world, sev._pad_cap
    splits = [cap] * w
    uniq, inv_t, counts = torch.unique(
        values_cat, return_inverse=True, return_counts=True)
    inverse = inv_t.to(torch.int32)
    order, bounds = coll._prep_backward(inverse, counts)
    send_keys, send_cnt, route_pos = _route_pad_cpu(uniq, counts, w, cap,
                                                    KEY_BITS)
    recv_keys = comm.all_to_all_single(send_keys, splits, splits)
    recv_cnt = comm.all_to_all_single(send_cnt, splits, splits)
    uniq2, inv2 = torch.unique(recv_keys, return_inverse=True)
    cnt2 = torch.zeros(uniq2.numel(), dtype=torch.int64)
    cnt2.index_add_(0, inv2, recv_cnt.long())
    n_own = int((uniq2 != PAD_KEY).sum())
    own_keys = uniq2[:n_own]
    own_slots = st.lookup_or_create(own_keys, cnt2[:n_own],
                                    get_global_step(), train=True)
    reply = torch.zeros(uniq2.numel(), coll.dim)
    reply[:n_own] = st.gather(own_keys, own_slots)
    reply = reply[inv2]
    if sev.comm_dtype is not None:
        lp = reply.to(sev.comm_dtype).contiguous()
        emb_rows = comm.all_to_all_single(
            lp.view(torch.int16), splits, splits) \
            .view(sev.comm_dtype).float()
    else:
        emb_rows = comm.all_to_all_single(reply.contiguous(), splits,
                                          splits)
    ex = _PaddedExchange(inverse, order, bounds, route_pos, None, inv2,
                         own_keys, own_slots)
    return ex, emb_rows, uniq2, route_pos[inverse.long()].to(torch.int32)


def _padded_sharded_lookup(sev, values_cat, offsets_cat, row_ids_cat,
                           row_coeff, weights_cat, batch, out_dtype):
    exchange = (_padded_lookup_gpu if sev.local.device.type == "cuda"
                else _padded_lookup_cpu)
    ex, emb_rows, keys, inverse_final = exchange(sev, values_cat)
    return _PaddedShardedLookup.apply(
        sev.local._anchor, sev, ex, emb_rows, keys, inverse_final,
        offsets_cat, row_ids_cat, row_coeff, weights_cat, batch, out_dtype)


class _PaddedShardedLookup(torch.autograd.Function):
    @staticmethod
    def forward(ctx, anchor, sev, ex, emb_rows, keys, inverse_final,
                offsets_cat, row_ids_cat, row_coeff, weights_cat, batch,
                out_dtype):
        out = sev.local._forward(keys, None, inverse_final, offsets_cat,
                                 weights_cat, batch, out_dtype,
                                 emb_override=emb_rows)
        ctx.sev = sev
        ctx.ex = ex
        ctx.batch = batch
        ctx.weights_cat = weights_cat
        ctx.save_for_backward(row_ids_cat, row_coeff)
        return out

    @staticmethod
    def backward(ctx, grad_out):
        sev, ex = ctx.sev, ctx.ex
        coll = sev.local
        st = coll.storage
        w, cap = sev.world, sev._pad_cap
        splits = [cap] * w
        row_ids_cat, row_coeff = ctx.saved_tensors
        grad_unique = coll._backward(grad_out, ex.order, ex.bounds,
                                     ex.inverse, row_ids_cat,
                                     ctx.weights_cat, row_coeff,
                                     ex.bounds.numel() - 1, ctx.batch)
        if coll.device.type == "cuda":
            grad_send = st.ext.rows_to_padded(grad_unique, ex.route_pos,
                                              ex.m_dev, w * cap)
            grad_recv = comm.all_to_all_single(grad_send, splits, splits)
            grad_own = st.ext.rows_segsum_pad(grad_recv, ex.own_inv, w * cap)
        else:
            grad_send = torch.zeros(w * cap, grad_unique.shape[1])
            grad_send[ex.route_pos] = grad_unique
            grad_recv = comm.all_to_all_single(grad_send, splits, splits)
            n_own = ex.own_keys.numel()
            grad_own = torch.zeros(n_own + 1, grad_recv.shape[1])
            grad_own.index_add_(0, ex.own_inv, grad_recv)
            grad_own = grad_own[:n_own]
        coll.accumulate_grad(ex.own_slots, ex.own_keys, grad_own)
        return (torch.zeros_like(coll._anchor),) + (None,) * 11


def _a2a(sev: ShardedEmbeddingCollection, tensor, in_sp, out_sp):
    if sev.node_size and sev.world > sev.node_size:
        from deeprec_amd.parallel.hierarchical import hierarchical_all_to_all
        out, oc = hierarchical_all_to_all(tensor, in_sp, sev.node_size)
        assert oc == list(out_sp)
        return out
    return comm.all_to_all_single(tensor, in_sp, out_sp)


def _exchange_lookup(sev: ShardedEmbeddingCollection, uniq, counts, train):
    coll = sev.local
    w = sev.world
    raw = uniq & ((1 << KEY_BITS) - 1)
    owner = (raw % w).to(torch.int64)
    order_o = torch.argsort(owner, stable=True)
    send_keys = uniq[order_o]
    send_counts = counts[order_o]
    send_splits = torch.bincount(owner, minlength=w)
    recv_splits = comm.exchange_counts(send_splits)
    in_sp, out_sp = send_splits.tolist(), recv_splits.tolist()
    sev._observed_max_split = max(sev._observed_max_split,
                                  max(in_sp), max(out_sp))
    recv_keys = _a2a(sev, send_keys, in_sp, out_sp)
    recv_counts = _a2a(sev, send_counts, in_sp, out_sp)
    uniq2, inv2 = torch.unique(recv_keys, return_inverse=True)
    counts2 = torch.zeros(uniq2.numel(), dtype=recv_counts.dtype,
                          device=uniq.device)
    counts2.index_add_(0, inv2, recv_counts)
    slots2 = coll.storage.lookup_or_create(uniq2, counts2, get_global_step(),
                                           train=train)
    emb2 = coll.storage.gather(uniq2, slots2)
    emb_out = emb2[inv2]
    if sev.comm_dtype is not None:
        lp = emb_out.to(sev.comm_dtype).contiguous()
        if torch.distributed.get_backend() == "gloo":
            emb_back = _a2a(sev, lp.view(torch.int16), out_sp,
                            in_sp).view(sev.comm_dtype).float()
        else:
            emb_back = _a2a(sev, lp, out_sp, in_sp).float()
    else:
        emb_back = _a2a(sev, emb_out.contiguous(), out_sp, in_sp)
    emb = torch.empty_like(emb_back)
    emb[order_o] = emb_back
    ctx = (order_o, inv2, slots2, uniq2, in_sp, out_sp)
    return emb, ctx


class _ShardedCollectionLookup(torch.autograd.Function):
    @staticmethod
    def forward(ctx, anchor, sev, uniq, counts, inverse, offsets_cat,
                row_ids_cat, order, bounds, row_coeff, weights_cat, batch,
                out_dtype):
        emb, ex_ctx = _exchange_lookup(sev, uniq, counts, train=True)
        out = sev.local._forward(uniq, None, inverse, offsets_cat,
                                 weights_cat, batch, out_dtype,
                                 emb_override=emb)
        ctx.sev = sev
        ctx.batch = batch
        ctx.weights_cat = weights_cat
        ctx.ex = ex_ctx
        ctx.save_for_backward(uniq, order, bounds, inverse, row_ids_cat,
                              row_coeff)
        return out

    @staticmethod
    def backward(ctx, grad_out):
        sev = ctx.sev
        coll = sev.local
        uniq, order, bounds, inverse, row_ids_cat, row_coeff = \
            ctx.saved_tensors
        order_o, inv2, slots2, uniq2, in_sp, out_sp = ctx.ex
        grad_unique = coll._backward(grad_out, order, bounds, inverse,
                                     row_ids_cat, ctx.weights_cat,
                                     row_coeff, uniq.numel(), ctx.batch)
        grad_send = grad_unique[order_o]
        grad_recv = _a2a(sev, grad_send.contiguous(), in_sp, out_sp)
        grad2 = torch.zeros(uniq2.numel(), grad_recv.shape[1],
                            device=grad_recv.device, dtype=grad_recv.dtype)
        grad2.index_add_(0, inv2.long(), grad_recv)
        coll.accumulate_grad(slots2, uniq2, grad2)
        return (torch.zeros_like(coll._anchor),) + (None,) * 12
```

deeprec_amd/parallel/sharded_embedding.py:

```python
from __future__ import annotations

from typing import Optional

import torch

from deeprec_amd.embedding.options import EmbeddingVariableOption
from deeprec_amd.embedding.ragged import RaggedIds
from deeprec_amd.embedding.variable import EmbeddingVariable
from deeprec_amd.ops import functional as F
from deeprec_amd.parallel import comm


class ShardedEmbeddingVariable:

    def __init__(self, name: str, embedding_dim: int,
                 ev_option: Optional[EmbeddingVariableOption] = None,
                 device=None, value_dtype=torch.float32):
        self.name = name
        self.dim = embedding_dim
        self.world = comm.world_size()
        self.rank = comm.rank()
        self.local_ev = EmbeddingVariable(
            f"{name}/part_{self.rank}", embedding_dim, value_dtype,
            ev_option, device)

    @property
    def local(self):
        return self.local_ev

    @property
    def device(self):
        return self.local_ev.device

    @property
    def storage(self):
        return self.local_ev.storage

    @property
    def trainable(self):
        return self.local_ev.trainable

    @property
    def _anchor(self):
        return self.local_ev._anchor

    @property
    def _pending_grads(self):
        return self.local_ev._pending_grads

    def consume_grads(self):
        return self.local_ev.consume_grads()

    def export(self, include_filtered=False):
        return self.local_ev.export(include_filtered)

    def restore(self, keys, values, freqs=None, versions=None):
        mine = (keys % self.world) == self.rank
        self.local_ev.restore(keys[mine], values[mine],
                              None if freqs is None else freqs[mine],
                              None if versions is None else versions[mine])

    def shrink(self, step=None):
        return self.local_ev.shrink(step)

    def size(self):
        return self.local_ev.size()

    def get_slab(self, name, width=None, init_value=0.0, dtype=torch.float32):
        return self.local_ev.get_slab(name, width, init_value, dtype)

    def reshard(self, world: int, rank: int):
        old = self.local_ev
        self.world = world
        self.rank = rank
        self.local_ev = EmbeddingVariable(
            f"{self.name}/part_{rank}", self.dim, old.value_dtype,
            old.ev_option, old.device, trainable=old.trainable)


class _ShardedPooledLookup(torch.autograd.Function):
    @staticmethod
    def forward(ctx, anchor, sev: ShardedEmbeddingVariable, uniq, counts,
                inverse, offsets, row_ids, combiner, weights, out_dtype):
        w = sev.world
        dev = uniq.device
        owner = (uniq % w).to(torch.int64)
        order = torch.argsort(owner, stable=True)
        send_keys = uniq[order]
        send_counts_payload = counts[order]
        send_splits = torch.bincount(owner, minlength=w)
        recv_splits = comm.exchange_counts(send_splits)
        in_sp = send_splits.tolist()
        out_sp = recv_splits.tolist()
        recv_keys = comm.all_to_all_single(send_keys, in_sp, out_sp)
        recv_counts = comm.all_to_all_single(send_counts_payload, in_sp, out_sp)
        uniq2, inv2 = torch.unique(recv_keys, return_inverse=True)
        counts2 = torch.zeros(uniq2.numel(), dtype=recv_counts.dtype,
                              device=dev)
        counts2.index_add_(0, inv2, recv_counts)
        slots2 = sev.local_ev.lookup_or_create(uniq2, counts2)
        emb2 = sev.local_ev.storage.gather(uniq2, slots2)
        emb_out = emb2[inv2]
        emb_back = comm.all_to_all_single(emb_out.contiguous(), out_sp, in_sp)
        emb_uniq = torch.empty_like(emb_back)
        emb_uniq[order] = emb_back
        out = F.pooled_forward(emb_uniq, inverse, offsets, row_ids, combiner,
                               weights, out_dtype)
        ctx.sev = sev
        ctx.combiner = combiner
        ctx.weights = weights
        ctx.splits = (in_sp, out_sp)
        ctx.save_for_backward(order, inv2, slots2, uniq2, inverse, offsets,
                              row_ids)
        return out

    @staticmethod
    def backward(ctx, grad_out):
        sev = ctx.sev
        in_sp, out_sp = ctx.splits
        order, inv2, slots2, uniq2, inverse, offsets, row_ids = \
            ctx.saved_tensors
        m = order.numel()
        grad_unique = F.pooled_backward(grad_out, inverse, offsets, row_ids,
                                        m, ctx.combiner, ctx.weights)
        grad_send = grad_unique[order]
        grad_recv = comm.all_to_all_single(grad_send.contiguous(),
                                           in_sp, out_sp)
        grad2 = torch.zeros(uniq2.numel(), grad_recv.shape[1],
                            device=grad_recv.device, dtype=grad_recv.dtype)
        grad2.index_add_(0, inv2, grad_recv)
        sev.local_ev.accumulate_grad(slots2, uniq2, grad2)
        return (torch.zeros_like(sev.local_ev._anchor),) + (None,) * 9


def _sharded_lookup_infer(sev: ShardedEmbeddingVariable, uniq, inverse,
                          offsets, row_ids, combiner, weights, out_dtype):
    w = sev.world
    owner = (uniq % w).to(torch.int64)
    order = torch.argsort(owner, stable=True)
    send_keys = uniq[order]
    send_splits = torch.bincount(owner, minlength=w)
    recv_splits = comm.exchange_counts(send_splits)
    in_sp, out_sp = send_splits.tolist(), recv_splits.tolist()
    recv_keys = comm.all_to_all_single(send_keys, in_sp, out_sp)
    uniq2, inv2 = torch.unique(recv_keys, return_inverse=True)
    slots2 = sev.local_ev.storage.lookup(uniq2)
    emb2 = sev.local_ev.storage.gather(uniq2, slots2)
    emb_out = emb2[inv2]
    emb_back = comm.all_to_all_single(emb_out.contiguous(), out_sp, in_sp)
    emb_uniq = torch.empty_like(emb_back)
    emb_uniq[order] = emb_back
    return F.pooled_forward(emb_uniq, inverse, offsets, row_ids, combiner,
                            weights, out_dtype)


def sharded_embedding_lookup_sparse(sev: ShardedEmbeddingVariable,
                                    sp_ids: RaggedIds, combiner="mean",
                                    out_dtype=None, train=True):
    uniq, inverse, counts = torch.unique(
        sp_ids.values, return_inverse=True, return_counts=True)
    row_ids = sp_ids.row_ids()
    if not (train and sev.trainable):
        return _sharded_lookup_infer(
            sev, uniq, inverse.to(torch.int32), sp_ids.offsets, row_ids,
            combiner, sp_ids.weights, out_dtype)
    return _ShardedPooledLookup.apply(
        sev._anchor, sev, uniq, counts, inverse.to(torch.int32),
        sp_ids.offsets, row_ids, combiner, sp_ids.weights, out_dtype)
```

Measured before the change: 15.57 million samples/sec.

## Fuse embedding dedup prologue, matrix key tagging, CSR bounds scan and BCE loss kernels

Several launch-reduction changes for the graph-captured DLRM training step. The id-matrix transpose and table tagging are folded into the hash dedup pass. Epoch bump, counter reset and counts zeroing become one begin kernel. The CSR bounds cumsum moves to a custom two-kernel scan, and BCE-with-logits mean gets dedicated forward and backward kernels. Anchor gradients now return None instead of zeros_like. Each change removes small kernels or copies per step, at the cost of more custom code paths, and the None anchor gradient may change how autograd treats the anchor.

```diff
diff --git a/deeprec_amd/embedding/collection.py b/deeprec_amd/embedding/collection.py
--- a/deeprec_amd/embedding/collection.py
+++ b/deeprec_amd/embedding/collection.py
@@ -33,11 +33,13 @@
 def prep_backward(storage, inverse, counts, rank=None):
     m = counts.numel()
     c32 = counts.to(torch.int32)
-    bounds = torch.zeros(m + 1, dtype=torch.int32, device=inverse.device)
-    bounds[1:] = c32.cumsum(0)
     if inverse.device.type != "cuda":
+        bounds = torch.zeros(m + 1, dtype=torch.int32, device=inverse.device)
+        bounds[1:] = c32.cumsum(0)
         order = torch.argsort(inverse.long()).to(torch.int32)
-    elif rank is not None:
+        return order, bounds
+    bounds = storage.ext.csr_bounds(c32.contiguous())
+    if rank is not None:
         order = storage.ext.csr_scatter(inverse, rank, bounds,
                                         storage.error_flag)
     else:
@@ -192,6 +194,10 @@
         return prep_backward(self.storage, inverse, counts, rank)
 
     def matrix_inputs(self, ids: torch.Tensor):
+        offsets, row_ids, row_coeff, tags = self._matrix_static(ids)
+        return ids.t().reshape(-1) + tags, offsets, row_ids, row_coeff
+
+    def _matrix_static(self, ids: torch.Tensor):
         batch, n = ids.shape
         assert n == self.n_tables
         cache = self._matrix_cache.get(batch)
@@ -205,15 +211,20 @@
                 (torch.arange(n, dtype=torch.int64, device=dev)
                  << KEY_BITS).repeat_interleave(batch))
             self._matrix_cache[batch] = cache
-        offsets, row_ids, row_coeff, tags = cache
-        return ids.t().reshape(-1) + tags, offsets, row_ids, row_coeff
+        return cache
 
     def lookup_matrix(self, ids: torch.Tensor, out_dtype=None,
                       train: bool = True) -> torch.Tensor:
         batch = ids.shape[0]
-        values_cat, offsets, row_ids, row_coeff = self.matrix_inputs(ids)
         train = train and self.trainable
-        d = self._dedup_and_probe(values_cat, train)
+        if (train and self.graph_mode and not self._record_sparse_ids
+                and ids.dtype == torch.int64 and ids.is_contiguous()
+                and hasattr(self.storage, "dedup_lookup_capture_matrix")):
+            offsets, row_ids, row_coeff, _ = self._matrix_static(ids)
+            d = self.storage.dedup_lookup_capture_matrix(ids)
+        else:
+            values_cat, offsets, row_ids, row_coeff = self.matrix_inputs(ids)
+            d = self._dedup_and_probe(values_cat, train)
         if not train:
             return self._forward(d.uniq, d.slots, d.inverse, offsets, None,
                                  batch, out_dtype)
@@ -356,4 +367,4 @@
                                      row_coeff, uniq.numel(), ctx.batch,
                                      ctx.identity_rows)
         coll.accumulate_grad(slots, uniq, grad_unique)
-        return (torch.zeros_like(coll._anchor),) + (None,) * 13
+        return (None,) * 14
diff --git a/deeprec_amd/embedding/lookup.py b/deeprec_amd/embedding/lookup.py
--- a/deeprec_amd/embedding/lookup.py
+++ b/deeprec_amd/embedding/lookup.py
@@ -49,7 +49,7 @@
                 grad_out, inverse, offsets, row_ids, uniq.numel(),
                 ctx.combiner, ctx.weights)
         ev.accumulate_grad(slots, uniq, grad_unique)
-        return (torch.zeros_like(ctx.ev._anchor),) + (None,) * 10
+        return (None,) * 11
 
 
 def _chunked_ev_backward(ev, grad_out, inverse, offsets, row_ids, counts,
@@ -143,7 +143,7 @@
             grad_out.contiguous(), order, inverse, none, none, none,
             uniq.numel(), inverse.numel(), 1, ev.dim, True, 0)
         ev.accumulate_grad(slots, uniq, grad_unique)
-        return (torch.zeros_like(ev._anchor),) + (None,) * 6
+        return (None,) * 7
 
 
 def masked_padded_lookup(ev, ids: torch.Tensor, pad_id: int, out_dtype=None,
diff --git a/deeprec_amd/models/common.py b/deeprec_amd/models/common.py
--- a/deeprec_amd/models/common.py
+++ b/deeprec_amd/models/common.py
@@ -85,5 +85,5 @@
         return contextlib.nullcontext()
 
     def loss_fn(self, logits: torch.Tensor, labels: torch.Tensor):
-        return nn.functional.binary_cross_entropy_with_logits(
-            logits.float(), labels.float())
+        from deeprec_amd.ops.fused_loss import bce_with_logits_mean
+        return bce_with_logits_mean(logits.float(), labels.float())
diff --git a/deeprec_amd/models/dlrm.py b/deeprec_amd/models/dlrm.py
--- a/deeprec_amd/models/dlrm.py
+++ b/deeprec_amd/models/dlrm.py
@@ -127,4 +127,5 @@
         return logits.squeeze(1).float()
 
     def loss_fn(self, logits: torch.Tensor, labels: torch.Tensor):
-        return nn.functional.binary_cross_entropy_with_logits(logits, labels)
+        from deeprec_amd.ops.fused_loss import bce_with_logits_mean
+        return bce_with_logits_mean(logits, labels)
diff --git a/deeprec_amd/ops/build_ext.py b/deeprec_amd/ops/build_ext.py
--- a/deeprec_amd/ops/build_ext.py
+++ b/deeprec_amd/ops/build_ext.py
@@ -16,7 +16,8 @@
             os.path.join(_HERE, "hip", "gru_kernels.hip"),
             os.path.join(_HERE, "hip", "attention_kernels.hip"),
             os.path.join(_HERE, "hip", "fp8_kernels.hip"),
-            os.path.join(_HERE, "hip", "quant_ev_kernels.hip")]
+            os.path.join(_HERE, "hip", "quant_ev_kernels.hip"),
+            os.path.join(_HERE, "hip", "loss_kernels.hip")]
 _HIPCC = os.environ.get("HIPCC", "/opt/rocm/bin/hipcc")
 _ARCH = os.environ.get("PYTORCH_ROCM_ARCH", "gfx950")
 
diff --git a/deeprec_amd/ops/fused_loss.py b/deeprec_amd/ops/fused_loss.py
--- /dev/null
+++ b/deeprec_amd/ops/fused_loss.py
@@ -0,0 +1,44 @@
+from __future__ import annotations
+
+import torch
+import torch.nn.functional as F
+
+from deeprec_amd.ops.build_ext import require_extension
+
+
+class _BceLogitsMean(torch.autograd.Function):
+    @staticmethod
+    def forward(ctx, logits, labels):
+        ctx.save_for_backward(logits, labels)
+        return require_extension().bce_logits_mean_fwd(logits, labels)
+
+    @staticmethod
+    def backward(ctx, grad_out):
+        logits, labels = ctx.saved_tensors
+        return require_extension().bce_logits_mean_bwd(
+            logits, labels, grad_out.contiguous()), None
+
+
+def _fused_ok(logits, labels) -> bool:
+    if logits.device.type != "cuda" or labels.device != logits.device:
+        return False
+    if logits.dtype != torch.float32 or labels.dtype != torch.float32:
+        return False
+    if logits.dim() != 1 or labels.shape != logits.shape:
+        return False
+    if not (logits.is_contiguous() and labels.is_contiguous()):
+        return False
+    if labels.requires_grad:
+        return False
+    return 1 <= logits.numel() <= require_extension().BCE_LOGITS_MEAN_MAX_B
+
+
+def bce_with_logits_mean(logits: torch.Tensor, labels: torch.Tensor,
+                         weight=None, pos_weight=None,
+                         reduction: str = "mean") -> torch.Tensor:
+    if (weight is None and pos_weight is None and reduction == "mean"
+            and _fused_ok(logits, labels)):
+        return _BceLogitsMean.apply(logits, labels)
+    return F.binary_cross_entropy_with_logits(
+        logits, labels, weight=weight, pos_weight=pos_weight,
+        reduction=reduction)
diff --git a/deeprec_amd/ops/hip/ev_kernels.hip b/deeprec_amd/ops/hip/ev_kernels.hip
--- a/deeprec_amd/ops/hip/ev_kernels.hip
+++ b/deeprec_amd/ops/hip/ev_kernels.hip
@@ -142,19 +142,27 @@
 }
 
 
-template <bool SKIP_PAD>
+template <bool SKIP_PAD, bool MATRIX = false>
 __global__ void k_dedup_pass_a(
     const int64_t* __restrict__ keys, int nnz, int64_t* __restrict__ ht_keys,
     int32_t* __restrict__ ht_epoch, int32_t* __restrict__ ht_compact,
     int64_t cap_mask, const int32_t* __restrict__ epoch_dev, int epoch_val,
     int32_t* __restrict__ entry_counter, int32_t* __restrict__ m_counter,
     int64_t* __restrict__ uniq_keys, int64_t* __restrict__ compact_entry,
-    int64_t* __restrict__ occ_entry, int32_t* __restrict__ error_flag) {
+    int64_t* __restrict__ occ_entry, int32_t* __restrict__ error_flag,
+    int batch = 0, int n_tables = 0, int key_bits = 0) {
   const int epoch = epoch_dev ? *epoch_dev : epoch_val;
   int64_t j = blockIdx.x * (int64_t)blockDim.x + threadIdx.x;
   int64_t stride = gridDim.x * (int64_t)blockDim.x;
   for (; j < nnz; j += stride) {
-    const int64_t key = keys[j];
+    int64_t key;
+    if constexpr (MATRIX) {
+      const int t = (int)j / batch;
+      const int b = (int)j - t * batch;
+      key = keys[(int64_t)b * n_tables + t] + ((int64_t)t << key_bits);
+    } else {
+      key = keys[j];
+    }
     if constexpr (SKIP_PAD) {
       if (key == PAD_KEY) {
         occ_entry[j] = -1;
@@ -185,6 +193,22 @@
     epoch_dev[0] += 1;
     step_dev[0] += 1;
   }
+}
+
+__global__ void k_dedup_begin(int32_t* __restrict__ epoch_dev,
+                              int64_t* __restrict__ step_dev,
+                              int32_t* __restrict__ m_counter,
+                              int32_t* __restrict__ counts, int64_t n) {
+  if (threadIdx.x == 0 && blockIdx.x == 0) {
+    epoch_dev[0] += 1;
+    if (step_dev) step_dev[0] += 1;
+    m_counter[0] = 0;
+    for (int64_t j = n & ~3LL; j < n; ++j) counts[j] = 0;
+  }
+  int64_t i = (blockIdx.x * (int64_t)blockDim.x + threadIdx.x) * 4;
+  int64_t stride = gridDim.x * (int64_t)blockDim.x * 4;
+  for (; i + 3 < n; i += stride)
+    *reinterpret_cast<int4*>(counts + i) = make_int4(0, 0, 0, 0);
 }
 
 __global__ void k_dedup_pass_b(
@@ -417,6 +441,79 @@
     if (in_range) {
       inverse[j] = valid ? c : -1;
       rank[j] = valid ? base + g.pos : 0;
+    }
+  }
+}
+
+constexpr int kScanPer = 4;
+constexpr int kScanTile = kBlock * kScanPer;
+constexpr int kScanMaxBlocks = 1024;
+
+DEV_INLINE int block_sum_i32(int v, int* __restrict__ red) {
+  red[threadIdx.x] = v;
+  __syncthreads();
+  for (int s = kBlock / 2; s > 0; s >>= 1) {
+    if ((int)threadIdx.x < s) red[threadIdx.x] += red[threadIdx.x + s];
+    __syncthreads();
+  }
+  const int total = red[0];
+  __syncthreads();
+  return total;
+}
+
+__global__ __launch_bounds__(kBlock) void k_tile_sums(
+    const int32_t* __restrict__ counts, int64_t m, int n_tiles,
+    int32_t* __restrict__ tile_sums) {
+  __shared__ int red[kBlock];
+  for (int t = blockIdx.x; t < n_tiles; t += gridDim.x) {
+    const int64_t i0 = (int64_t)t * kScanTile + threadIdx.x * kScanPer;
+    int v = 0;
+#pragma unroll
+    for (int k = 0; k < kScanPer; ++k)
+      if (i0 + k < m) v += counts[i0 + k];
+    const int total = block_sum_i32(v, red);
+    if (threadIdx.x == 0) tile_sums[t] = total;
+  }
+}
+
+__global__ __launch_bounds__(kBlock) void k_csr_bounds(
+    const int32_t* __restrict__ counts, int64_t m, int n_tiles,
+    const int32_t* __restrict__ tile_sums, int32_t* __restrict__ bounds) {
+  __shared__ int red[kBlock];
+  __shared__ int scan[2][kBlock];
+  if (blockIdx.x == 0 && threadIdx.x == 0) bounds[0] = 0;
+  int base = 0;
+  int summed = 0;
+  for (int t = blockIdx.x; t < n_tiles; t += gridDim.x) {
+    int part = 0;
+    for (int u = summed + threadIdx.x; u < t; u += kBlock)
+      part += tile_sums[u];
+    base += block_sum_i32(part, red);
+    summed = t;
+    const int64_t i0 = (int64_t)t * kScanTile + threadIdx.x * kScanPer;
+    int c[kScanPer];
+    int mine = 0;
+#pragma unroll
+    for (int k = 0; k < kScanPer; ++k) {
+      c[k] = i0 + k < m ? counts[i0 + k] : 0;
+      mine += c[k];
+    }
+    int cur = 0;
+    scan[0][threadIdx.x] = mine;
+    __syncthreads();
+    for (int d = 1; d < kBlock; d <<= 1) {
+      int v = scan[cur][threadIdx.x];
+      if ((int)threadIdx.x >= d) v += scan[cur][threadIdx.x - d];
+      scan[cur ^ 1][threadIdx.x] = v;
+      cur ^= 1;
+      __syncthreads();
+    }
+    int run = base + scan[cur][threadIdx.x] - mine;
+    __syncthreads();
+#pragma unroll
+    for (int k = 0; k < kScanPer; ++k) {
+      run += c[k];
+      if (i0 + k < m) bounds[i0 + k + 1] = run;
     }
   }
 }
@@ -1060,23 +1157,25 @@
   return t.has_value() ? t->data_ptr<T>() : nullptr;
 }
 
-template <bool SKIP_PAD>
+template <bool SKIP_PAD, bool MATRIX = false>
 static torch::Tensor dedup_a_impl(
     torch::Tensor keys, torch::Tensor ht_keys, torch::Tensor ht_epoch,
     torch::Tensor ht_compact, c10::optional<torch::Tensor> epoch_dev,
     int64_t epoch, torch::Tensor entry_counter, torch::Tensor m_counter,
     torch::Tensor uniq_keys, torch::Tensor compact_entry,
-    torch::Tensor occ_entry, torch::Tensor error_flag) {
+    torch::Tensor occ_entry, torch::Tensor error_flag, int batch = 0,
+    int n_tables = 0, int key_bits = 0) {
   int64_t nnz = keys.numel();
   if (nnz == 0) return m_counter;
   auto stream = current_hip_stream();
-  k_dedup_pass_a<SKIP_PAD><<<n_blocks(nnz), kBlock, 0, stream>>>(
+  k_dedup_pass_a<SKIP_PAD, MATRIX><<<n_blocks(nnz), kBlock, 0, stream>>>(
       keys.data_ptr<int64_t>(), (int)nnz, ht_keys.data_ptr<int64_t>(),
       ht_epoch.data_ptr<int32_t>(), ht_compact.data_ptr<int32_t>(),
       ht_keys.numel() - 1, opt_ptr<int32_t>(epoch_dev), (int)epoch,
       entry_counter.data_ptr<int32_t>(), m_counter.data_ptr<int32_t>(),
       uniq_keys.data_ptr<int64_t>(), compact_entry.data_ptr<int64_t>(),
-      occ_entry.data_ptr<int64_t>(), error_flag.data_ptr<int32_t>());
+      occ_entry.data_ptr<int64_t>(), error_flag.data_ptr<int32_t>(), batch,
+      n_tables, key_bits);
   return m_counter;
 }
 
@@ -1103,6 +1202,31 @@
   return dedup_a_impl<true>(keys, ht_keys, ht_epoch, ht_compact, epoch_dev,
                             epoch, entry_counter, m_counter, uniq_keys,
                             compact_entry, occ_entry, error_flag);
+}
+
+torch::Tensor ht_dedup_a_matrix(
+    torch::Tensor ids, int64_t key_bits, torch::Tensor ht_keys,
+    torch::Tensor ht_epoch, torch::Tensor ht_compact,
+    c10::optional<torch::Tensor> epoch_dev, int64_t epoch,
+    torch::Tensor entry_counter, torch::Tensor m_counter,
+    torch::Tensor uniq_keys, torch::Tensor compact_entry,
+    torch::Tensor occ_entry, torch::Tensor error_flag) {
+  CHECK_DEV(ids);
+  TORCH_CHECK(ids.dim() == 2 && ids.is_contiguous() &&
+                  ids.scalar_type() == torch::kInt64,
+              "ht_dedup_a_matrix: ids must be contiguous int64 [batch, n]");
+  TORCH_CHECK(ids.numel() <= INT32_MAX, "ht_dedup_a_matrix: too many ids");
+  TORCH_CHECK(key_bits > 0 && key_bits < 63 &&
+                  ids.size(1) <= ((int64_t)1 << (63 - key_bits)),
+              "ht_dedup_a_matrix: table tag does not fit above key_bits");
+  TORCH_CHECK(uniq_keys.numel() >= ids.numel() &&
+                  compact_entry.numel() >= ids.numel() &&
+                  occ_entry.numel() >= ids.numel(),
+              "ht_dedup_a_matrix: output buffers are smaller than ids");
+  return dedup_a_impl<false, true>(
+      ids, ht_keys, ht_epoch, ht_compact, epoch_dev, epoch, entry_counter,
+      m_counter, uniq_keys, compact_entry, occ_entry, error_flag,
+      (int)ids.size(0), (int)ids.size(1), (int)key_bits);
 }
 
 torch::Tensor ht_dedup_b(torch::Tensor compact_entry, torch::Tensor uniq_keys,
@@ -1143,6 +1267,25 @@
       epoch_dev.data_ptr<int32_t>());
 }
 
+void dedup_begin(torch::Tensor epoch_dev,
+                 c10::optional<torch::Tensor> step_dev,
+                 torch::Tensor m_counter, torch::Tensor counts) {
+  CHECK_DEV(counts);
+  TORCH_CHECK(counts.scalar_type() == torch::kInt32 &&
+                  counts.is_contiguous() &&
+                  m_counter.scalar_type() == torch::kInt32 &&
+                  m_counter.numel() == 1,
+              "dedup_begin: counts int32 contiguous, m_counter int32 [1]");
+  TORCH_CHECK(reinterpret_cast<uintptr_t>(counts.data_ptr()) % 16 == 0,
+              "dedup_begin: counts must be 16-byte aligned");
+  const int64_t n = counts.numel();
+  k_dedup_begin<<<std::max(1, n_blocks((n + 3) / 4)), kBlock, 0,
+                  current_hip_stream()>>>(
+      epoch_dev.data_ptr<int32_t>(),
+      step_dev.has_value() ? step_dev->data_ptr<int64_t>() : nullptr,
+      m_counter.data_ptr<int32_t>(), counts.data_ptr<int32_t>(), n);
+}
+
 std::tuple<torch::Tensor, torch::Tensor, torch::Tensor> route_pad(
     torch::Tensor uniq_keys, torch::Tensor counts, torch::Tensor m_dev,
     int64_t world, int64_t cap, int64_t key_bits,
@@ -1255,19 +1398,49 @@
 
 std::tuple<torch::Tensor, torch::Tensor, torch::Tensor> ht_dedup_c(
     c10::optional<torch::Tensor> keys, torch::Tensor occ_entry,
-    torch::Tensor ht_compact, int64_t m) {
+    torch::Tensor ht_compact, int64_t m,
+    c10::optional<torch::Tensor> counts_in) {
   int64_t nnz = occ_entry.numel();
   auto inverse = torch::empty({nnz}, ht_compact.options());
   auto rank = torch::empty({nnz}, ht_compact.options());
-  auto counts = torch::empty({m}, ht_compact.options());
+  if (counts_in.has_value())
+    TORCH_CHECK(counts_in->numel() == m && counts_in->is_contiguous() &&
+                    counts_in->scalar_type() == torch::kInt32 &&
+                    counts_in->is_cuda(),
+                "ht_dedup_c: counts must be int32 [m] on GPU");
+  auto counts = counts_in.has_value()
+                    ? *counts_in
+                    : torch::empty({m}, ht_compact.options());
   if (nnz == 0) return {inverse, counts, rank};
   auto stream = current_hip_stream();
-  zero_fill(counts.data_ptr<int32_t>(), m, stream);
+  if (!counts_in.has_value()) zero_fill(counts.data_ptr<int32_t>(), m, stream);
   k_dedup_pass_c<<<n_blocks(nnz), kBlock, 0, stream>>>(
       opt_ptr<int64_t>(keys), occ_entry.data_ptr<int64_t>(), (int)nnz,
       ht_compact.data_ptr<int32_t>(), inverse.data_ptr<int32_t>(),
       counts.data_ptr<int32_t>(), rank.data_ptr<int32_t>());
   return {inverse, counts, rank};
+}
+
+torch::Tensor csr_bounds(torch::Tensor counts) {
+  CHECK_DEV(counts);
+  TORCH_CHECK(counts.scalar_type() == torch::kInt32 && counts.dim() == 1 &&
+                  counts.is_contiguous(),
+              "csr_bounds: counts must be contiguous int32 [m]");
+  const int64_t m = counts.numel();
+  if (m == 0) return torch::zeros({1}, counts.options());
+  auto bounds = torch::empty({m + 1}, counts.options());
+  const int64_t n_tiles = (m + kScanTile - 1) / kScanTile;
+  TORCH_CHECK(n_tiles <= INT32_MAX, "csr_bounds: too many counts");
+  auto tile_sums = torch::empty({n_tiles}, counts.options());
+  const int grid = (int)std::min<int64_t>(n_tiles, kScanMaxBlocks);
+  auto stream = current_hip_stream();
+  k_tile_sums<<<grid, kBlock, 0, stream>>>(
+      counts.data_ptr<int32_t>(), m, (int)n_tiles,
+      tile_sums.data_ptr<int32_t>());
+  k_csr_bounds<<<grid, kBlock, 0, stream>>>(
+      counts.data_ptr<int32_t>(), m, (int)n_tiles,
+      tile_sums.data_ptr<int32_t>(), bounds.data_ptr<int32_t>());
+  return bounds;
 }
 
 torch::Tensor csr_scatter(torch::Tensor inverse, torch::Tensor rank,
@@ -1815,6 +1988,7 @@
 void register_attention(pybind11::module_& mod);
 void register_fp8(pybind11::module_& mod);
 void register_quant_ev(pybind11::module_& mod);
+void register_loss(pybind11::module_& mod);
 
 PYBIND11_MODULE(TORCH_EXTENSION_NAME, mod) {
   register_dense(mod);
@@ -1822,12 +1996,15 @@
   register_attention(mod);
   register_fp8(mod);
   register_quant_ev(mod);
+  register_loss(mod);
   mod.def("ht_lookup_insert", &ht_lookup_insert);
   mod.def("ht_dedup_a", &ht_dedup_a);
   mod.def("ht_dedup_a_pad", &ht_dedup_a_pad);
+  mod.def("ht_dedup_a_matrix", &ht_dedup_a_matrix);
   mod.def("ht_dedup_b", &ht_dedup_b);
   mod.def("bump_epoch", &bump_epoch);
   mod.def("bump_epoch_only", &bump_epoch_only);
+  mod.def("dedup_begin", &dedup_begin);
   mod.def("route_pad", &route_pad);
   mod.def("rows_to_padded", &rows_to_padded);
   mod.def("slots_gather_pad", &slots_gather_pad);
@@ -1836,7 +2013,12 @@
   mod.def("compose_i32", &compose_i32);
   mod.def("gather_host_rows", &gather_host_rows);
   mod.def("scatter_host_rows", &scatter_host_rows);
-  mod.def("ht_dedup_c", &ht_dedup_c);
+  mod.def("ht_dedup_c", &ht_dedup_c, pybind11::arg("keys"),
+          pybind11::arg("occ_entry"), pybind11::arg("ht_compact"),
+          pybind11::arg("m"), pybind11::arg("counts") = pybind11::none());
+  mod.def("csr_bounds", &csr_bounds);
+  mod.attr("CSR_SCAN_TILE") = kScanTile;
+  mod.attr("CSR_SCAN_MAX_BLOCKS") = kScanMaxBlocks;
   mod.def("csr_order", &csr_order);
   mod.def("csr_scatter", &csr_scatter);
   mod.def("csr_scatter_pad", &csr_scatter_pad);
diff --git a/deeprec_amd/ops/hip/loss_kernels.hip b/deeprec_amd/ops/hip/loss_kernels.hip
--- /dev/null
+++ b/deeprec_amd/ops/hip/loss_kernels.hip
@@ -0,0 +1,89 @@
+
+#include "hip_common.h"
+
+namespace {
+
+constexpr int kLossBlock = 1024;
+constexpr int64_t kLossMaxB = 1 << 20;
+
+__global__ __launch_bounds__(kLossBlock) void k_bce_logits_mean_fwd(
+    const float* __restrict__ x, const float* __restrict__ y, int n,
+    float* __restrict__ loss) {
+  __shared__ float part[kLossBlock];
+  float acc = 0.0f;
+  for (int i = threadIdx.x; i < n; i += kLossBlock) {
+    const float xi = x[i];
+    acc += (fmaxf(xi, 0.0f) - xi * y[i]) + log1pf(expf(-fabsf(xi)));
+  }
+  part[threadIdx.x] = acc;
+  __syncthreads();
+  for (int s = kLossBlock / 2; s > 0; s >>= 1) {
+    if ((int)threadIdx.x < s) part[threadIdx.x] += part[threadIdx.x + s];
+    __syncthreads();
+  }
+  if (threadIdx.x == 0) loss[0] = part[0] / (float)n;
+}
+
+__global__ void k_bce_logits_mean_bwd(const float* __restrict__ x,
+                                      const float* __restrict__ y,
+                                      const float* __restrict__ grad_out,
+                                      int n, float* __restrict__ gx) {
+  const float scale = grad_out[0] / (float)n;
+  int i = blockIdx.x * blockDim.x + threadIdx.x;
+  const int stride = gridDim.x * blockDim.x;
+  for (; i < n; i += stride) {
+    const float xi = x[i], yi = y[i];
+    const float e = expf(-fabsf(xi));
+    const float omy = 1.0f - yi;
+    const float num = xi >= 0.0f ? fmaf(-yi, e, omy) : fmaf(e, omy, -yi);
+    gx[i] = (num / (1.0f + e)) * scale;
+  }
+}
+
+void check_loss_inputs(const torch::Tensor& logits,
+                       const torch::Tensor& labels) {
+  TORCH_CHECK(logits.is_cuda() && labels.is_cuda(),
+              "bce_logits_mean: inputs must be on GPU");
+  TORCH_CHECK(logits.scalar_type() == torch::kFloat32 &&
+                  labels.scalar_type() == torch::kFloat32,
+              "bce_logits_mean: inputs must be fp32");
+  TORCH_CHECK(logits.dim() == 1 && labels.dim() == 1 &&
+                  logits.numel() == labels.numel(),
+              "bce_logits_mean: logits and labels must be [B]");
+  TORCH_CHECK(logits.is_contiguous() && labels.is_contiguous(),
+              "bce_logits_mean: inputs must be contiguous");
+  TORCH_CHECK(logits.numel() >= 1 && logits.numel() <= kLossMaxB,
+              "bce_logits_mean: B must be in [1, ", kLossMaxB, "]");
+}
+
+}
+
+torch::Tensor bce_logits_mean_fwd(torch::Tensor logits,
+                                  torch::Tensor labels) {
+  check_loss_inputs(logits, labels);
+  auto loss = torch::empty({}, logits.options());
+  k_bce_logits_mean_fwd<<<1, kLossBlock, 0, current_hip_stream()>>>(
+      logits.data_ptr<float>(), labels.data_ptr<float>(),
+      (int)logits.numel(), loss.data_ptr<float>());
+  return loss;
+}
+
+torch::Tensor bce_logits_mean_bwd(torch::Tensor logits, torch::Tensor labels,
+                                  torch::Tensor grad_out) {
+  check_loss_inputs(logits, labels);
+  TORCH_CHECK(grad_out.is_cuda() && grad_out.numel() == 1 &&
+                  grad_out.scalar_type() == torch::kFloat32,
+              "bce_logits_mean: grad_out must be one fp32 value on GPU");
+  auto gx = torch::empty_like(logits);
+  const int n = (int)logits.numel();
+  k_bce_logits_mean_bwd<<<n_blocks(n), 256, 0, current_hip_stream()>>>(
+      logits.data_ptr<float>(), labels.data_ptr<float>(),
+      grad_out.data_ptr<float>(), n, gx.data_ptr<float>());
+  return gx;
+}
+
+void register_loss(py::module_& mod) {
+  mod.def("bce_logits_mean_fwd", &bce_logits_mean_fwd);
+  mod.def("bce_logits_mean_bwd", &bce_logits_mean_bwd);
+  mod.attr("BCE_LOGITS_MEAN_MAX_B") = kLossMaxB;
+}
diff --git a/deeprec_amd/ops/hip_backend.py b/deeprec_amd/ops/hip_backend.py
--- a/deeprec_amd/ops/hip_backend.py
+++ b/deeprec_amd/ops/hip_backend.py
@@ -206,20 +206,38 @@
         self._step_dev = torch.tensor([get_global_step()],
                                       dtype=torch.int64, device=self.device)
 
-    def _dedup_claim(self, keys: torch.Tensor, epoch_dev=None, pad=False):
+    def _dedup_begin(self, nnz: int, bump_step: bool = True):
+        m_counter = torch.empty(1, dtype=torch.int32, device=self.device)
+        counts = torch.empty(nnz, dtype=torch.int32, device=self.device)
+        self.ext.dedup_begin(self._epoch_dev,
+                             self._step_dev if bump_step else None,
+                             m_counter, counts)
+        return m_counter, counts
+
+    def _dedup_claim(self, keys: torch.Tensor, epoch_dev=None, pad=False,
+                     m_counter=None, matrix=False):
         nnz = keys.numel()
         uniq_buf = torch.empty(nnz, dtype=torch.int64, device=self.device)
         centry_buf = torch.empty(nnz, dtype=torch.int64, device=self.device)
         occ_entry = torch.empty(nnz, dtype=torch.int64, device=self.device)
-        m_counter = torch.zeros(1, dtype=torch.int32, device=self.device)
-        pass_a = self.ext.ht_dedup_a_pad if pad else self.ext.ht_dedup_a
-        pass_a(keys, self.ht_keys, self.ht_epoch, self.ht_compact,
-               epoch_dev, self._epoch, self.entry_counter, m_counter,
-               uniq_buf, centry_buf, occ_entry, self.error_flag)
+        if m_counter is None:
+            m_counter = torch.zeros(1, dtype=torch.int32, device=self.device)
+        rest = (self.ht_keys, self.ht_epoch, self.ht_compact, epoch_dev,
+                self._epoch, self.entry_counter, m_counter, uniq_buf,
+                centry_buf, occ_entry, self.error_flag)
+        if matrix:
+            assert not pad, "the id matrix holds no pads"
+            self.ext.ht_dedup_a_matrix(keys, self.key_bits, *rest)
+        elif pad:
+            self.ext.ht_dedup_a_pad(keys, *rest)
+        else:
+            self.ext.ht_dedup_a(keys, *rest)
         return uniq_buf, centry_buf, occ_entry, m_counter
 
-    def _dedup_count(self, occ_entry: torch.Tensor, m: int, pad_keys=None):
-        return self.ext.ht_dedup_c(pad_keys, occ_entry, self.ht_compact, m)
+    def _dedup_count(self, occ_entry: torch.Tensor, m: int, pad_keys=None,
+                     counts=None):
+        return self.ext.ht_dedup_c(pad_keys, occ_entry, self.ht_compact, m,
+                                   counts)
 
     def _dedup_admit(self, centry, uniq, counts, step=0, m_dev=None):
         return self.ext.ht_dedup_b(
@@ -231,19 +249,22 @@
             self._init_limit(), self.filter_freq, self.error_flag)
 
     def dedup_lookup_capture(self, values_cat: torch.Tensor, pad=False,
-                             bump_step=True) -> DedupResult:
-        if bump_step:
-            self.ext.bump_epoch(self._epoch_dev, self._step_dev)
-        else:
-            self.ext.bump_epoch_only(self._epoch_dev)
+                             bump_step=True, matrix=False) -> DedupResult:
+        nnz = values_cat.numel()
+        m_counter, counts = self._dedup_begin(nnz, bump_step)
         uniq_buf, centry_buf, occ_entry, m_counter = self._dedup_claim(
-            values_cat, self._epoch_dev, pad)
+            values_cat, self._epoch_dev, pad, m_counter, matrix)
         inverse, counts, rank = self._dedup_count(
-            occ_entry, values_cat.numel(),
-            pad_keys=values_cat if pad else None)
+            occ_entry, nnz, pad_keys=values_cat if pad else None,
+            counts=counts)
         slots = self._dedup_admit(centry_buf, uniq_buf, counts,
                                   m_dev=m_counter)
         return DedupResult(uniq_buf, inverse, counts, slots, rank, m_counter)
+
+    def dedup_lookup_capture_matrix(self, ids: torch.Tensor,
+                                    bump_step=True) -> DedupResult:
+        return self.dedup_lookup_capture(ids, bump_step=bump_step,
+                                         matrix=True)
 
     def dedup_only_capture(self, values_cat: torch.Tensor) -> DedupResult:
         self.ext.bump_epoch(self._epoch_dev, self._step_dev)
diff --git a/deeprec_amd/parallel/sharded_collection.py b/deeprec_amd/parallel/sharded_collection.py
--- a/deeprec_amd/parallel/sharded_collection.py
+++ b/deeprec_amd/parallel/sharded_collection.py
@@ -284,7 +284,7 @@
             grad_own.index_add_(0, ex.own_inv, grad_recv)
             grad_own = grad_own[:n_own]
         coll.accumulate_grad(ex.own_slots, ex.own_keys, grad_own)
-        return (torch.zeros_like(coll._anchor),) + (None,) * 11
+        return (None,) * 12
 
 
 def _a2a(sev: ShardedEmbeddingCollection, tensor, in_sp, out_sp):
@@ -367,4 +367,4 @@
                             device=grad_recv.device, dtype=grad_recv.dtype)
         grad2.index_add_(0, inv2.long(), grad_recv)
         coll.accumulate_grad(slots2, uniq2, grad2)
-        return (torch.zeros_like(coll._anchor),) + (None,) * 12
+        return (None,) * 13
diff --git a/deeprec_amd/parallel/sharded_embedding.py b/deeprec_amd/parallel/sharded_embedding.py
--- a/deeprec_amd/parallel/sharded_embedding.py
+++ b/deeprec_amd/parallel/sharded_embedding.py
@@ -130,7 +130,7 @@
                             device=grad_recv.device, dtype=grad_recv.dtype)
         grad2.index_add_(0, inv2, grad_recv)
         sev.local_ev.accumulate_grad(slots2, uniq2, grad2)
-        return (torch.zeros_like(sev.local_ev._anchor),) + (None,) * 9
+        return (None,) * 10
 
 
 def _sharded_lookup_infer(sev: ShardedEmbeddingVariable, uniq, inverse,
```

After: 16.80 million samples/sec (median of 6 runs). +7.9%, better.
